# edavalosanaya/FastPoseCNN

Measured on AMD Instinct MI355X. Metric: img/s end-to-end 640x480 inference; hough-vote kernel HBM GB/s vs roofline, higher is better.
Workload: dtype f32

## Files before the change

fastposecnn_amd/_native.py:

```python
import ctypes
import os

import torch

_HERE = os.path.dirname(os.path.abspath(__file__))
LIB_PATH = os.path.join(_HERE, "libfpc_hip.so")

_lib = None

_vp = ctypes.c_void_p
_i = ctypes.c_int
_i64 = ctypes.c_int64
_u64 = ctypes.c_uint64
_f = ctypes.c_float
_d = ctypes.c_double
_sz = ctypes.c_size_t

_SIGNATURES = {
    "fpc_abi_version": (ctypes.c_int, []),
    "fpc_error_string": (ctypes.c_char_p, [_i]),
    "fpc_last_hip_error": (ctypes.c_char_p, []),
    "fpc_generate_hypothesis": (_i, [_vp, _vp, _vp, _vp, _i, _i, _i, _vp]),
    "fpc_voting_for_hypothesis": (_i, [_vp, _vp, _vp, _vp, _i, _i, _i, _f, _vp]),
    "fpc_ransac_workspace_bytes": (_sz, [_i, _i, _i, _i]),
    "fpc_ransac_voting_v3": (_i, [_vp, _vp, _i64, _i64, _i64, _i64, _i, _vp, _i, _i, _i, _vp, _vp, _u64, _f, _i, _i,
                                  _vp, _vp, _vp, _vp, _vp, _vp, _vp, _vp, _vp, _sz, _vp]),
    "fpc_ransac_voting_v3_bits": (_i, [_vp, _vp, _vp, _i64, _i64, _i64, _i64, _i, _vp, _i, _i, _i, _vp, _vp, _u64, _f, _i, _i, _vp, _vp, _vp, _vp, _vp, _vp, _vp, _vp, _vp, _sz, _vp]),
    "fpc_ransac_voting_v3_pose": (_i, [_vp, _vp, _vp, _i64, _i64, _i64, _i64, _i, _vp, _i, _i, _i, _vp, _vp, _u64, _f, _i, _i, _vp, _vp, _vp, _vp, _vp, _vp, _vp, _vp,
                                       _vp, _vp, _vp, _vp, _vp, _vp, _vp, _sz, _vp]),
    "fpc_vote_set_prune": (_i, [_i, _i, ctypes.POINTER(ctypes.c_int32)]),
    "fpc_vote_prune_info": (_i, [_vp, _sz, _i, _i, _i, _i, _vp, _vp]),
    "fpc_class_compress": (_i, [_vp, _vp, _vp, _vp, _vp, _vp, _i, _i, _i, _vp, _vp, _vp, _vp, _vp, _vp]),
    "fpc_class_compress_bits": (_i, [_vp, _vp, _vp, _vp, _vp, _vp, _i, _i, _i, _vp, _vp, _vp, _vp, _vp, _vp, _vp]),
    "fpc_cc_workspace_bytes": (_sz, [_i, _i, _i]),
    "fpc_cc_bits_supported": (_i, [_i, _i, _i]),
    "fpc_fg_bits": (_i, [_vp, _i, _i, _i, _vp, _vp]),
    "fpc_cc_label_bits": (_i, [_vp, _i, _i, _i, _vp, _vp, _vp, _i, _vp, _sz, _vp]),
    "fpc_cc_label": (_i, [_vp, _i, _i, _i, _vp, _vp, _vp, _i, _vp, _sz, _vp]),
    "fpc_aggregate_workspace_bytes": (_sz, [_i]),
    "fpc_aggregate": (_i, [_vp, _vp, _vp, _vp, _vp, _vp, _i, _i, _i, _i, _vp, _vp, _vp, _vp, _vp, _vp, _vp, _vp, _vp, _vp, _sz,
                           _vp]),
    "fpc_aggregate_bits": (_i, [_vp, _vp, _vp, _vp, _vp, _vp, _i, _i, _i, _i, _vp, _vp, _vp, _vp, _vp, _vp, _vp, _vp, _vp, _vp, _vp, _vp, _sz, _vp]),
    "fpc_mask_bits_words": (_sz, [_i, _i]),
    "fpc_pose_errors": (_i, [_vp, _vp, _vp, _vp, _i, _vp, _vp, _vp, _vp, _vp, _vp, _i, _vp, _vp, _vp, _vp]),
    "fpc_pose_metrics_state_words": (_sz, [_i, _i, _i, _i, _i]),
    "fpc_pose_metrics_update": (_i, [_vp, _vp, _vp, _i, _i] + [_vp] * 11 + [_i, _vp, _i, _vp, _i, _vp, _i, _vp, _i, _vp, _i] + [_vp] * 5 + [_i, _vp]),
    "fpc_confusion_update": (_i, [_vp, _vp, _i64, _i, _vp, _vp]),
    "fpc_post_network_backward": (_i, [_vp, _vp, _i, _i, _i, _i, _vp, _vp, _f, _i, _u64, _vp, _vp, _vp, _vp, _vp, _vp]),
    "fpc_vote_refine_backward": (_i, [_vp, _vp, _i64, _i64, _i64, _i64, _i, _i, _i, _vp, _f, _i, _u64, _vp, _vp, _vp]),
    "fpc_class_compress_backward": (_i, [_vp, _vp, _vp, _vp, _vp, _vp, _vp, _i, _i, _i, _vp, _vp, _vp, _vp, _vp]),
    "fpc_mask_losses": (_i, [_vp, _vp, _i, _i, _i, _i64, _i64, _f, _f, _vp, _vp, _vp, _vp]),
    "fpc_match_assign": (_i, [_vp, _vp, _vp, _i, _i, _vp, _vp, _vp, _vp]),
    "fpc_matched_losses": (_i, [_vp, _vp, _vp, _i, _i] + [_vp] * 10 + [_i, _d, _i, _i, _i, ctypes.POINTER(_d)] + [_vp] * 5),
    "fpc_matched_losses_backward": (_i, [_vp, _vp, _vp, _i, _i] + [_vp] * 10 + [_i, _d, _i, _i, _i, ctypes.POINTER(_d)] + [_vp] * 8),
    "fpc_grad_sumsq": (_i, [_vp, _sz, _vp, _vp]),
    "fpc_lookahead_radam_step": (_i, [_vp, _vp, _vp, _vp, _vp, _sz, _f, _f, _f, _f, _f, _i64, _i, _f, _vp, _vp]),
    "fpc_pose_rt": (_i, [_vp, _vp, _vp, _vp, _i, _vp, _vp, _vp, _vp]),
    "fpc_pack_pose_records": (_i, [_vp] * 9 + [_i, _i, _i, _vp, _vp]),
    "fpc_mask_iou_workspace_bytes": (_sz, [_i, _i, _i64]),
    "fpc_mask_iou": (_i, [_vp, _i, _vp, _i, _i64, _i, _vp, _vp, _vp, _vp, _sz, _vp]),
    "fpc_preprocess_workspace_bytes": (_sz, [_i]),
    "fpc_preprocess_u8": (_i, [_vp, _i, _i, _i, ctypes.POINTER(ctypes.c_double), ctypes.POINTER(ctypes.c_double), _i, _vp, _vp,
                               _sz, _vp]),
    "fpc_png_info": (_i, [_vp, _sz, ctypes.POINTER(ctypes.c_int32)]),
    "fpc_png_decode": (_i, [_vp, _sz, _vp, _sz, _i]),
    "fpc_png_decode_batch": (_i, [ctypes.POINTER(_vp), ctypes.POINTER(_sz), _i, _vp, _i, _i, _i]),
    "fpc_inflate_host": (_i, [_vp, _sz, _vp, _sz, ctypes.POINTER(_sz)]),
    "fpc_png_pack_bytes": (_sz, [_i, _i, _i]),
    "fpc_png_pack_batch": (_i, [ctypes.POINTER(_vp), ctypes.POINTER(_sz), _i, _i, _i, _i, _vp, _sz, _vp, ctypes.POINTER(_sz)]),
    "fpc_png_decode_device_workspace_bytes": (_sz, [_i, _i, _i, _i]),
    "fpc_png_decode_device": (_i, [_vp, _sz, _vp, _i, _i, _i, _i, _i, _vp, _sz, _vp, _vp, _sz, _vp]),
    "fpc_gt_build": (_i, [_vp, _i64, _i64, _i, _i, _i, _vp, _vp, _vp, _i, _vp, _vp, _i, _vp, _vp]),
    "fpc_depth_decode": (_i, [_vp, _i, _i, _i, _i, _i, _vp, _vp]),
    "fpc_net_create": (_i, [ctypes.c_char_p, _i, _i, _i, _i, ctypes.POINTER(_vp)]),
    "fpc_net_create_encoder": (_i, [_i, ctypes.POINTER(_i), _i, _i, _i, _i, ctypes.POINTER(_vp)]),
    "fpc_net_create_encoder_ex": (_i, [_i, ctypes.POINTER(_i), _i, _i, _i, _i, _i, _i, ctypes.POINTER(_vp)]),
    "fpc_net_create_encoder_se": (_i, [ctypes.POINTER(_i), _i, _i, _i, _i, _i, ctypes.POINTER(_vp)]),
    "fpc_net_destroy": (None, [_vp]),
    "fpc_net_set_graph": (_i, [_vp, _i]),
    "fpc_net_set_split_precision": (_i, [_vp, _i]),
    "fpc_net_param_count": (_i, [_vp]),
    "fpc_net_param_name": (ctypes.c_char_p, [_vp, _i]),
    "fpc_net_param_numel": (_i64, [_vp, _i]),
    "fpc_net_workspace_bytes": (_sz, [_vp]),
    "fpc_net_load_params": (_i, [_vp, _vp, _i, _vp, _sz, _vp]),
    "fpc_net_forward": (_i, [_vp, _vp, _vp, _vp, _vp, _vp, _vp, _vp, _vp, _vp, _vp, _vp, _vp]),
    "fpc_net_forward_bits": (_i, [_vp, _vp, _vp, _vp, _vp, _vp, _vp, _vp, _vp, _vp, _vp, _vp, _vp, _vp]),
    "fpc_net_autotune_next": (_i, [_vp, _i]),
    "fpc_net_conv_count": (_i, [_vp]),
    "fpc_net_conv_plan": (_i, [_vp, _i, ctypes.POINTER(_i)]),
    "fpc_net_copy_plans": (_i, [_vp, _vp]),
    "fpc_net_force_winograd": (_i, [_vp, _i]),
    "fpc_net_force_pointwise": (_i, [_vp, _i]),
    "fpc_net_force_fold": (_i, [_vp, _i]),
    "fpc_net_force_direct_h3": (_i, [_vp, _i]),
    "fpc_net_force_stem_pool": (_i, [_vp, _i]),
    "fpc_act_range": (_i, [_vp, ctypes.c_longlong, _vp, _vp]),
    "fpc_net_survey_next": (_i, [_vp, _vp, _i]),
    "fpc_net_guard_ranges": (_i, [_vp, ctypes.POINTER(ctypes.c_uint32), _i, _f, _f]),
    "fpc_net_guarded": (_i, [_vp, _i]),
    "fpc_stem_pool_tasks": (_i, [_i, _i, ctypes.POINTER(_i64)]),
    "fpc_wino_pack_geometry": (_i, [_i, _i, _i, _i, _i, ctypes.POINTER(_i64)]),
    "fpc_net_set_wino_pack": (_i, [_vp, _i]),
    "fpc_net_set_wino_orient": (_i, [_vp, _i]),
    "fpc_wino_orient_geometry": (_i, [_i, _i, _i, _i, _i, _i, ctypes.POINTER(_i64)]),
    "fpc_wino_recip": (_i, [ctypes.c_uint32, ctypes.POINTER(_i64)]),
    "fpc_wino_decode": (_i, [_i, _i, _i, _i, _i, _i, _i, ctypes.POINTER(_i64)]),
    "fpc_net_wino_blocks": (_i64, [_vp]),
    "fpc_net_graph_recorded": (_i, [_vp]),
    "fpc_net_flops": (_i, [_vp, ctypes.POINTER(ctypes.c_double)]),
    "fpc_net_tensor": (_i, [_vp, ctypes.c_char_p, ctypes.POINTER(_vp), ctypes.POINTER(_i), ctypes.POINTER(_i),
                            ctypes.POINTER(_i)]),
    "fpc_conv2d_workspace_bytes": (_sz, [_i, _i, _i, _i, _i, _i, _i]),
    "fpc_conv2d_workspace_bytes_for": (_sz, [_i, _i, _i, _i, _i, _i, _i, _i, _i, _i]),
    "fpc_conv2d_plan": (_i, [_i, _i, _i, _i, _i, _i, _i, _i, _i, _i, ctypes.POINTER(_i)]),
    "fpc_conv2d": (_i, [_vp, _i64, _i64, _i64, _i64, _vp, _vp, _vp, _vp, _vp, _vp, _vp, _i, _i, _i, _i, _i, _i, _i, _i,
                        _i, _i, _i, _i, _i, _vp, _sz, _vp]),
    "fpc_conv2d_grouped_workspace_bytes": (_sz, [_i, _i]),
    "fpc_conv2d_grouped": (_i, [_vp, _i64, _i64, _i64, _i64, _vp, _vp, _vp, _vp, _i, _i, _i, _i, _i, _i, _i, _i, _vp, _sz, _vp]),
    "fpc_conv2d_grouped_dgrad_workspace_bytes": (_sz, [_i, _i]),
    "fpc_conv2d_grouped_dgrad": (_i, [_vp, _vp, _vp, _i, _i, _i, _i, _i, _i, _vp, _sz, _vp]),
    "fpc_conv2d_grouped_wgrad_workspace_bytes": (_sz, [_i, _i, _i, _i, _i]),
    "fpc_conv2d_grouped_wgrad": (_i, [_vp, _i64, _i64, _i64, _vp, _vp, _i, _i, _i, _i, _i, _i, _vp, _sz, _vp]),
    "fpc_image_nhwc4": (_i, [_vp, _vp, _i, _i, _i, _vp]),
    "fpc_stem_wgrad_workspace_bytes": (_sz, [_i, _i, _i]),
    "fpc_stem_wgrad_slices": (_i, [_i, _i, _i]),
    "fpc_stem_wgrad": (_i, [_vp, _vp, _vp, _i, _i, _i, _vp, _sz, _vp]),
    "fpc_maxpool3x3s2_fwd": (_i, [_vp, _vp, _i, _i, _i, _i, _vp]),
    "fpc_maxpool3x3s2_bwd": (_i, [_vp, _vp, _vp, _i, _i, _i, _i, _vp]),
    "fpc_se_pool_slabs": (_i, [_i, _i, _i]),
    "fpc_se_scratch_floats": (_sz, [_i, _i, _i, _i]),
    "fpc_se_gate": (_i, [_vp, _vp, _vp, _vp, _vp, _vp, _vp, _i, _i, _i, _i, _i, _vp]),
    "fpc_se_scale_add_relu": (_i, [_vp, _vp, _vp, _vp, _i, _i, _i, _i, _vp]),
    "fpc_maxpool3x3s2_ceil_fwd": (_i, [_vp, _vp, _i, _i, _i, _i, _vp]),
    "fpc_conv2d_wgrad_workspace_bytes": (_sz, [_i, _i, _i, _i, _i, _i, _i]),
    "fpc_upsample_bilinear_fwd": (_i, [_vp, _i64, _i64, _i64, _i64, _vp, _i, _i, _i, _i, _i, _i, _vp]),
    "fpc_upsample_bilinear_bwd_scratch_floats": (_sz, [_i, _i, _i, _i, _i]),
    "fpc_upsample_bilinear_bwd": (_i, [_vp, _i64, _i64, _i64, _i64, _vp, _vp, _i, _i, _i, _i, _i, _i, _vp]),
    "fpc_groupnorm4_relu_scratch_floats": (_sz, [_i, _i, _i]),
    "fpc_groupnorm4_relu_fwd": (_i, [_vp, _vp, _vp, _vp, _vp, _vp, _i, _i, _i, _i, ctypes.c_float, _vp]),
    "fpc_groupnorm4_relu_bwd": (_i, [_vp, _vp, _vp, _vp, _vp, _vp, _vp, _i, _i, _i, _i, _vp]),
    "fpc_batchnorm_scratch_floats": (_sz, [_i, _i]),
    "fpc_batchnorm_fwd": (_i, [_vp, _vp, _vp, _vp, _vp, _vp, _vp, _vp, _vp, _i, _i, _f, _f, _i, _vp]),
    "fpc_batchnorm_bwd": (_i, [_vp, _vp, _vp, _vp, _vp, _vp, _vp, _vp, _vp, _vp, _i, _i, _i, _vp]),
    "fpc_conv2d_wgrad": (_i, [_vp, _i64, _i64, _i64, _vp, _vp, _i, _i, _i, _i, _i, _i, _i, _i, _i, _vp, _sz, _vp]),
    "fpc_conv2d_wgrad_split": (_i, [_vp, _i64, _i64, _i64, _vp, _vp, _i, _i, _i, _i, _i, _i, _i, _i, _i, _vp, _sz, _vp]),
}

EXPORTED = tuple(_SIGNATURES)


def lib():
    global _lib
    if _lib is None:
        if not os.path.exists(LIB_PATH):
            raise RuntimeError(
                f"fastposecnn_amd: {LIB_PATH} is missing — build it with `python -m fastposecnn_amd.build` "
                "(hipcc --offload-arch=gfx950). There is no CPU fallback for the HIP hot path.")
        L = ctypes.CDLL(LIB_PATH)
        for name, (res, args) in _SIGNATURES.items():
            fn = getattr(L, name)
            fn.restype = res
            fn.argtypes = args
        if L.fpc_abi_version() != 11:
            raise RuntimeError("fastposecnn_amd: libfpc_hip.so ABI version mismatch")
        _lib = L
    return _lib


def check(rc, what):
    if rc != 0:
        L = lib()
        msg = L.fpc_error_string(rc).decode()
        hip = L.fpc_last_hip_error().decode() if rc == -3 else ""
        raise RuntimeError(f"fastposecnn_amd: {what} failed: {msg} (code {rc}){' — HIP: ' + hip if hip else ''}")


def ptr(t):
    return None if t is None else t.data_ptr()


_raw_stream = getattr(torch._C, "_cuda_getCurrentRawStream", None)
_cur_device = getattr(torch._C, "_cuda_getDevice", None)


def stream():
    if _raw_stream is not None and _cur_device is not None:
        return _raw_stream(_cur_device())
    return torch.cuda.current_stream().cuda_stream


def require_gpu(*tensors, what="this op"):
    for t in tensors:
        if t is not None and not t.is_cuda:
            raise RuntimeError(f"fastposecnn_amd: {what} runs only on GPU tensors (HIP kernels, no CPU fallback)")


_workspaces = {}


def workspace(tag, device, nbytes):
    key = (tag, device.index, stream())
    ws = _workspaces.get(key)
    if ws is None or ws.numel() < nbytes:
        ws = torch.empty(max(int(nbytes), 256), dtype=torch.uint8, device=device)
        assert ws.data_ptr() % 256 == 0
        _workspaces[key] = ws
    return ws
```

fastposecnn_amd/csrc/net.hip:

```cpp
#include <math.h>
#include <stdio.h>
#include <stdlib.h>
#include <string.h>

#include <initializer_list>
#include <string>
#include <utility>
#include <vector>

#include "net_kernels.hpp"

namespace fpc {

struct PackedConv {
    int Cin = 0, Cinp = 0, Cout = 0, Kh = 1, Kw = 1, stride = 1, pad = 0;
    int Kwp = 1;
    int K = 0, Kpad = 0, Npad = 0;
    int p_w = -1;
    int p_bn = -1;
    int p_bias = -1;
    size_t w_off = 0, scale_off = 0, shift_off = 0;
    size_t wino_off = 0;
    bool wino_ok = false;
    size_t h3_off = 0;
// ... 94 lines not shown
    return out;
}

static size_t splitk_floats_for(const ConvPlan& p, int groups, int B, int Npad) {
    return p.nsplit > 1 ? (size_t)groups * p.nsplit * B * p.mtiles * p.bm * Npad : 0;
}

enum WinoImage { kImgF32, kImgBf3, kImgC128, kImgH2, kImgH3, kWinoImageCount };
struct WinoImageDesc { int units, tail; int (*pack)(const float* w_oihw, float* packed, int Cout, int Cin, hipStream_t s); };
static int pack_h3_plain(const float* w_oihw, float* packed, int Cout, int Cin, hipStream_t s) { return launch_wino_pack_h3(w_oihw, packed, Cout, Cin, false, s); }
constexpr WinoImageDesc kWinoImages[kWinoImageCount] = {
    {16, 0, launch_wino_pack},
    {24, 0, launch_wino_pack_bf3},
    {24, 0, launch_wino_pack_c128},
    {16, 8, launch_wino_pack_h2},
    {16, 8, pack_h3_plain},
};
constexpr size_t kWinoSlack = 128;

constexpr int kWinoFormCount = 10;
constexpr int kWinoBf3 = 5, kWinoW4 = 7;
constexpr int kWinoH2 = 8, kWinoH3 = 9;
struct WinoForm {
    int waves;
    int bn, ck;
    int variant;
    WinoImage image;
    int wg_per_cu;
    int min_split;
    bool zeros;
    bool range_limited;
    int (*launch)(const WinoArgs& a, int groups, hipStream_t s);
};
constexpr WinoForm kWinoForms[kWinoFormCount] = {
    {},
    {4, 64, 8, 0, kImgF32, 2, 0, false, false, launch_conv_wino},
    {8, 64, 8, 0, kImgF32, 1, 0, false, false, launch_conv_wino},
    {4, 64, 8, 1, kImgF32, 2, 0, false, false, launch_conv_wino},
    {8, 64, 8, 2, kImgF32, 1, 0, true, false, launch_conv_wino},
    {8, 64, 8, 3, kImgBf3, 1, 1, true, false, launch_conv_wino},
    {4, 128, 8, 0, kImgC128, 1, 1, false, false, launch_conv_wino_c128},
    {8, 64, 8, 0, kImgBf3, 1, 1, false, false, launch_conv_wino_w4},
    {8, 64, 8, 0, kImgH2, 1, 2, false, true, launch_conv_wino_h2},
    {8, 64, 16, 0, kImgH3, 1, 3, false, true, launch_conv_wino_h3},
};
static bool wino_form_ok(int form, int Cin, int Cout) {
    return form >= 1 && form < kWinoFormCount && Cout % kWinoForms[form].bn == 0 && Cin % kWinoForms[form].ck == 0;
}
struct WinoSpan { size_t units, tails; };
static WinoSpan wino_span(int end, bool c128) {
    WinoSpan sp{0, 0};
    for (int i = 0; i < end; ++i)
        if (i != kImgC128 || c128) { sp.units += kWinoImages[i].units; sp.tails += kWinoImages[i].tail; }
    return sp;
}
static_assert(kWinoImages[kImgH2].tail + kWinoImages[kImgH3].tail <= 64, "kWinoSlack keeps one 64-float line for all tails");
static size_t wino_image_offset(WinoImage img, int Cout, int Cin) {
    const WinoSpan sp = wino_span(img, Cout % 128 == 0);
    return sp.units * Cout * Cin + sp.tails;
}
static size_t wino_region_floats(WinoImage last, int Cout, int Cin, bool c128) { return (wino_span(last, c128).units + kWinoImages[last].units) * Cout * Cin + kWinoSlack; }
static bool plan_range_limited(const ConvPlan& p) {
    return p.h3 || p.fold || p.pool || (p.wino && kWinoForms[p.wino].range_limited);
}
struct WinoGrid { int tbx, tby; int patches() const { return tbx * tby; } };
static WinoGrid wino_grid(int form, int H, int W) { return {cdiv(cdiv(W, 2), 8), cdiv(cdiv(H, 2), kWinoForms[form].waves)}; }

struct Conv2dRequest { int nsplit; bool bf3, two_launch; int wino, lat; bool stem; int pw; bool h3, pool, pack, orient; int grp; };
static Conv2dRequest decode_plan(int code) {
    Conv2dRequest r{code, false, false, 0, 0, false, 0, false, false, false, false, 0};
    if (code >= FPC_PLAN_GROUPED && code < FPC_PLAN_GROUPED + 1000) { r.grp = code - FPC_PLAN_GROUPED + 1; r.nsplit = 1; return r; }
    if (code == FPC_PLAN_WINO_ORIENT) { r.orient = true; r.nsplit = -kWinoH3; }
    if (code == FPC_PLAN_WINO_PACKED) { r.pack = true; r.nsplit = -kWinoH3; }
    if (r.nsplit >= FPC_PLAN_LATERAL_H3 && r.nsplit < FPC_PLAN_LATERAL_H3 + 1000) { r.lat = r.nsplit - FPC_PLAN_LATERAL_H3; r.h3 = true; r.nsplit = 1; return r; }
    if (r.nsplit >= FPC_PLAN_H3 && r.nsplit < FPC_PLAN_H3 + 200) { r.h3 = true; r.nsplit -= FPC_PLAN_H3; }
    if (r.nsplit >= FPC_PLAN_POINTWISE) { r.pw = r.nsplit - FPC_PLAN_POINTWISE + 1; r.bf3 = true; r.nsplit = 1; return r; }
    if (r.nsplit == FPC_PLAN_STEM_POOL) { r.stem = true; r.pool = true; r.h3 = true; r.nsplit = 1; return r; }
    if (r.nsplit == FPC_PLAN_STEM) { r.stem = true; r.bf3 = true; r.nsplit = 1; return r; }
    if (r.nsplit >= FPC_PLAN_LATERAL) { r.lat = r.nsplit - FPC_PLAN_LATERAL; r.bf3 = true; r.nsplit = 1; return r; }
    if (r.nsplit >= FPC_PLAN_BF3) { r.bf3 = true; r.nsplit -= FPC_PLAN_BF3; }
    if (r.nsplit >= FPC_PLAN_TWO_LAUNCH) { r.two_launch = true; r.nsplit -= FPC_PLAN_TWO_LAUNCH; }
    if (r.nsplit <= -1 && r.nsplit > -kWinoFormCount) r.wino = -r.nsplit;
    return r;
}
static int encode_plan(const ConvPlan& p, bool folded_away) {
    if (folded_away) return FPC_PLAN_FOLDED;
    if (p.grp) return FPC_PLAN_GROUPED + p.grp - 1;
    if (p.h3) return p.lat ? FPC_PLAN_LATERAL_H3 + p.lat : FPC_PLAN_H3 + p.nsplit;
    if (p.pw) return FPC_PLAN_POINTWISE + p.pw - 1;
    if (p.stem) return p.pool ? FPC_PLAN_STEM_POOL : FPC_PLAN_STEM;
    if (p.lat) return FPC_PLAN_LATERAL + p.lat;
    return p.wino ? -p.wino : p.nsplit;
}

}

using namespace fpc;

struct fpc_net {
    int layers[4];
    int classes, B, H, W;
    int expansion = 1;
    int groups = 1, width = 64;
    int se = 0;
    std::vector<std::string> pnames;
    std::vector<int64_t> pnumel;
    std::vector<const float*> pptr;
    std::vector<PackedConv> convs;
    size_t packed_floats = 0;
    size_t total_floats = 0;
    float* ws = nullptr;
    bool loaded = false;
    bool tuning = false;
    bool tuned = false;
    int tune_mode = 0;

    int c_stem = -1;
    struct Block { int conv1, conv2, ds, conv3 = -1; int p_se = -1; };
    std::vector<Block> blocks[4];
    struct Dec {
        int lat[4];
        int seg[7];
        int p_gn[7];
        int p_head_w, p_head_b;
        int head_ch, head_chp;
    } dec[4];

    Act a_img4, a_stem, a_pool;
    std::vector<Act> a_blk_t[4], a_blk_y[4], a_blk_d[4];
    std::vector<Act> a_blk_t2[4];
    Act a_p[4][4];
    Act a_seg[4][7];
    Act a_up[4][3];
    size_t gn_part_off[4][7], gn_aff_off[4][7];
    int gn_P[7];
    Act a_low[4];
    Act a_lsum[4];
    int merge_split = -1;
    size_t splitk_off = 0, splitk_floats = 0;
    size_t se_gate_off = 0, se_part_off = 0;
    int use_graph = 0;
    long long wino_blocks = 0;
    int wino_pack = 1;
    int wino_orient = 1;
    std::vector<char> c_tr;
    int split_precision = 0;
    hipGraphExec_t graph_exec = nullptr;
    size_t zeros_off = 0;
    size_t tickets_off = 0;

    bool h3_packed = false;
    hipStream_t load_stream = nullptr;
    size_t stem_h3_off = 0;
    bool fold_ok = false;
    size_t fold_wc_off[4] = {}, fold_img1_off[4] = {}, fold_img2_off[4] = {}, fold_tab_off[4] = {};

    std::vector<ConvPlan> cplan;
    std::vector<float> tune_score;
    unsigned* survey = nullptr;
    std::vector<ConvPlan> free_plan;
    std::vector<char> has_free;
    std::vector<char> guarded;
    std::vector<int> c_howo, c_groups;

    size_t bump = 0;
    size_t alloc(size_t n) { size_t o = bump; bump += (n + 63) / 64 * 64; return o; }
    Act alloc_act(int h, int w, int c) { Act a; a.H = h; a.W = w; a.C = c; a.off = alloc((size_t)B * h * w * c); return a; }
    int add_param(const std::string& n, int64_t numel) { pnames.push_back(n); pnumel.push_back(numel); return (int)pnames.size() - 1; }

    int add_conv(const std::string& wname, int Cin, int Cout, int k, int stride, int pad, const char* bn_prefix,
                 const char* bias_name, int Cinp = 0, int Kwp = 0) {
        PackedConv c;
        c.Cin = Cin; c.Cinp = Cinp ? Cinp : Cin; c.Cout = Cout; c.Kh = c.Kw = k; c.stride = stride; c.pad = pad;
        c.Kwp = Kwp ? Kwp : k;
        c.K = c.Cinp * k * c.Kwp; c.Kpad = cdiv(c.K, kConvBK) * kConvBK; c.Npad = cdiv(Cout, kConvNAlign) * kConvNAlign;
        c.p_w = add_param(wname, (int64_t)Cout * Cin * k * k);
        if (bn_prefix) {
            std::string p(bn_prefix);
            c.p_bn = add_param(p + ".weight", Cout);
            add_param(p + ".bias", Cout);
            add_param(p + ".running_mean", Cout);
            add_param(p + ".running_var", Cout);
        }
        if (bias_name) c.p_bias = add_param(bias_name, Cout);
        c.w_off = alloc(conv_packed_floats(c.Npad, c.Kpad));
        if (bn_prefix) { c.scale_off = alloc(Cout); c.shift_off = alloc(Cout); }
        c.wino_ok = (k == 3 && stride == 1 && pad == 1 && c.Cinp == Cin && Cin % 8 == 0 && Cout % 64 == 0);
        if (c.wino_ok) c.wino_off = alloc(wino_region_floats(kImgH3, Cout, Cin, Cout % 128 == 0));
        convs.push_back(c);
        return (int)convs.size() - 1;
    }
    int add_grouped_conv(const std::string& wname, int C, int cg, int stride, const char* bn_prefix) {
        PackedConv c;
        c.Cin = c.Cinp = c.Cout = C; c.Kh = c.Kw = c.Kwp = 3; c.stride = stride; c.pad = 1; c.cg = cg;
        c.K = cg * 9; c.Kpad = cdiv(c.K, kConvBK) * kConvBK; c.Npad = cdiv(C, kConvNAlign) * kConvNAlign;
        c.p_w = add_param(wname, (int64_t)C * cg * 9);
        std::string p(bn_prefix);
        c.p_bn = add_param(p + ".weight", C);
        add_param(p + ".bias", C);
        add_param(p + ".running_mean", C);
        add_param(p + ".running_var", C);
        c.grp_off = alloc((size_t)C * cg * 9);
        c.scale_off = alloc(C); c.shift_off = alloc(C);
        convs.push_back(c);
        return (int)convs.size() - 1;
    }
};

static void drop_graph(fpc_net* n) {
    if (n->graph_exec) { (void)hipGraphExecDestroy(n->graph_exec); n->graph_exec = nullptr; }
}

static const char* kDecNames[4] = {"mask_decoder", "rotation_decoder", "translation_decoder", "scales_decoder"};
static const char* kHeadNames[4] = {"segmentation_head", "rotation_head", "translation_head", "scales_head"};

static int conv_out(int x, int k, int s, int p) { return (x + 2 * p - k) / s + 1; }

static int net_build(fpc_net* n, int classes, int B, int H, int W, fpc_net_t** out);

extern "C" int fpc_net_create(const char* encoder, int classes, int B, int H, int W, fpc_net_t** out) {
    const int r18[4] = {2, 2, 2, 2}, r34[4] = {3, 4, 6, 3}, r101[4] = {3, 4, 23, 3};
    if (!encoder) return FPC_EINVAL;
    if (!strcmp(encoder, "resnext50_32x4d")) return fpc_net_create_encoder_ex(4, r34, 32, 4, classes, B, H, W, out);
    if (!strcmp(encoder, "resnext101_32x4d")) return fpc_net_create_encoder_ex(4, r101, 32, 4, classes, B, H, W, out);
    if (!strcmp(encoder, "resnext101_32x8d")) return fpc_net_create_encoder_ex(4, r101, 32, 8, classes, B, H, W, out);
    const int r152[4] = {3, 8, 36, 3};
    if (!strcmp(encoder, "se_resnet50")) return fpc_net_create_encoder_se(r34, 16, classes, B, H, W, out);
    if (!strcmp(encoder, "se_resnet101")) return fpc_net_create_encoder_se(r101, 16, classes, B, H, W, out);
    if (!strcmp(encoder, "se_resnet152")) return fpc_net_create_encoder_se(r152, 16, classes, B, H, W, out);
    if (strcmp(encoder, "resnet18") && strcmp(encoder, "resnet34")) return FPC_EINVAL;
    return fpc_net_create_encoder(1, strcmp(encoder, "resnet18") ? r34 : r18, classes, B, H, W, out);
}

extern "C" int fpc_net_create_encoder(int block, const int* layers4, int classes, int B, int H, int W, fpc_net_t** out) {
    return fpc_net_create_encoder_ex(block, layers4, 1, 64, classes, B, H, W, out);
}

extern "C" int fpc_net_create_encoder_ex(int block, const int* layers4, int groups, int width_per_group, int classes, int B, int H,
                                         int W, fpc_net_t** out) {
    if (!layers4 || !out || (block != 1 && block != 4) || classes < 2 || classes > 8 || B < 1 || H < 32 || W < 32 || H % 32 ||
        W % 32)
        return FPC_EINVAL;
    for (int L = 0; L < 4; ++L)
        if (layers4[L] < 1 || layers4[L] > 64) return FPC_EINVAL;
    if (groups < 1 || width_per_group < 1 || (groups == 1 && width_per_group != 64) || (groups > 1 && block != 4)) return FPC_EINVAL;
    if (groups > 1)
        for (int planes = 64; planes <= 512; planes *= 2) {
            const int cg = planes * width_per_group / 64;
            if (!grouped_cg_ok(cg) || (long long)cg * groups > 8192 || (cg * groups) % 64) return FPC_EINVAL;
        }
    fpc_net* n = new fpc_net();
    memcpy(n->layers, layers4, sizeof(n->layers));
    n->expansion = block;
    n->groups = groups; n->width = width_per_group;
    return net_build(n, classes, B, H, W, out);
}

extern "C" int fpc_net_create_encoder_se(const int* layers4, int reduction, int classes, int B, int H, int W, fpc_net_t** out) {
    if (!layers4 || !out || classes < 2 || classes > 8 || B < 1 || H < 32 || W < 32 || H % 32 || W % 32) return FPC_EINVAL;
    for (int L = 0; L < 4; ++L)
        if (layers4[L] < 1 || layers4[L] > 64) return FPC_EINVAL;
    if (reduction < 1 || 256 % reduction) return FPC_EINVAL;
    fpc_net* n = new fpc_net();
    memcpy(n->layers, layers4, sizeof(n->layers));
    n->expansion = 4;
    n->se = reduction;
    return net_build(n, classes, B, H, W, out);
}

static int net_build(fpc_net* n, int classes, int B, int H, int W, fpc_net_t** out) {
    n->classes = classes; n->B = B; n->H = H; n->W = W;
    {
        const char* e = getenv("FPC_MERGE_SPLIT");
        n->merge_split = e ? (atoi(e) != 0) : 1;
    }
    char buf[256];

    n->c_stem = n->se ? n->add_conv("encoder.layer0.conv1.weight", 3, 64, 7, 2, 3, "encoder.layer0.bn1", nullptr, 4, 8)
                      : n->add_conv("encoder.conv1.weight", 3, 64, 7, 2, 3, "encoder.bn1", nullptr, 4, 8);
    const int planes[4] = {64, 128, 256, 512};
    const int e = n->expansion;
    int inpl = 64;
    for (int L = 0; L < 4; ++L)
        for (int bi = 0; bi < n->layers[L]; ++bi) {
            int stride = (bi == 0 && L > 0) ? 2 : 1;
            fpc_net::Block blk;
            snprintf(buf, sizeof(buf), "encoder.layer%d.%d", L + 1, bi);
            std::string p(buf);
            if (n->se) {
                const int C = 4 * planes[L], Cr = C / n->se;
                blk.conv1 = n->add_conv(p + ".conv1.weight", inpl, planes[L], 1, stride, 0, (p + ".bn1").c_str(), nullptr);
                blk.conv2 = n->add_conv(p + ".conv2.weight", planes[L], planes[L], 3, 1, 1, (p + ".bn2").c_str(), nullptr);
                blk.conv3 = n->add_conv(p + ".conv3.weight", planes[L], C, 1, 1, 0, (p + ".bn3").c_str(), nullptr);
                blk.p_se = n->add_param(p + ".se_module.fc1.weight", (int64_t)Cr * C);
                n->add_param(p + ".se_module.fc1.bias", Cr);
                n->add_param(p + ".se_module.fc2.weight", (int64_t)C * Cr);
                n->add_param(p + ".se_module.fc2.bias", C);
                blk.ds = -1;
                if (stride != 1 || inpl != C)
                    blk.ds = n->add_conv(p + ".downsample.0.weight", inpl, C, 1, stride, 0, (p + ".downsample.1").c_str(), nullptr);
                inpl = C;
                n->blocks[L].push_back(blk);
                continue;
            }
            if (e == 4) {
                const int C = 4 * planes[L];
// ... 36 lines not shown
                snprintf(buf, sizeof(buf), "%s.seg_blocks.%d.block.%d.block", kDecNames[d], sb, j);
                std::string p(buf);
                dc.seg[si] = n->add_conv(p + ".0.weight", j == 0 ? 256 : 128, 128, 3, 1, 1, nullptr, nullptr);
                dc.p_gn[si] = n->add_param(p + ".1.weight", 128);
                n->add_param(p + ".1.bias", 128);
                ++si;
            }
    }
    for (int d = 0; d < 4; ++d) {
        fpc_net::Dec& dc = n->dec[d];
        dc.head_ch = head_ch[d];
        dc.head_chp = (head_ch[d] + 3) / 4 * 4;
        dc.p_head_w = n->add_param(std::string(kHeadNames[d]) + ".0.weight", (int64_t)head_ch[d] * 128);
        dc.p_head_b = n->add_param(std::string(kHeadNames[d]) + ".0.bias", head_ch[d]);
    }
    n->fold_ok = e == 1;
    if (n->fold_ok)
        for (int d = 0; d < 4; ++d) {
            n->fold_wc_off[d] = n->alloc((size_t)128 * 64 * 9);
            n->fold_img1_off[d] = n->alloc((size_t)16 * 128 * 64 + 2);
            n->fold_img2_off[d] = n->alloc((size_t)16 * 128 * 256 + 2);
            n->fold_tab_off[d] = n->alloc((size_t)16 * 128);
        }
    if (e == 1) {
        std::vector<int> sites;
        for (int L = 1; L < 4; ++L) { sites.push_back(n->blocks[L][0].conv1); if (n->blocks[L][0].ds >= 0) sites.push_back(n->blocks[L][0].ds); }
        for (int d = 0; d < 4; ++d)
            for (int i = 0; i < 3; ++i) sites.push_back(n->dec[d].lat[i]);
        for (int ci : sites) {
            PackedConv& c = n->convs[ci];
            if (c.wino_ok || c.Cin % kConvBK != 0 || c.Cinp != c.Cin || c.Kh * c.Kw > 32) continue;
            c.h3_ok = true;
            c.h3_off = n->alloc(h3_packed_floats(c.Npad, c.Kpad));
        }
    }
    n->stem_h3_off = n->alloc(h3_packed_floats(n->convs[n->c_stem].Npad, n->convs[n->c_stem].Kpad));
    n->zeros_off = n->alloc(64);
    n->tickets_off = n->alloc(kConvTickets);
    n->packed_floats = n->bump;

    int h1 = conv_out(H, 7, 2, 3), w1 = conv_out(W, 7, 2, 3);
    n->a_img4 = n->alloc_act(H, W, 4);
    n->a_stem = n->alloc_act(h1, w1, 64);
    int hp = n->se ? h1 / 2 : conv_out(h1, 3, 2, 1), wp = n->se ? w1 / 2 : conv_out(w1, 3, 2, 1);
    n->a_pool = n->alloc_act(hp, wp, 64);
    int fh[4], fw[4];
    {
        int h = hp, w = wp;
        for (int L = 0; L < 4; ++L) {
            const int hin = h, win = w;
            if (L > 0) { h = conv_out(h, 3, 2, 1); w = conv_out(w, 3, 2, 1); }
            fh[L] = h; fw[L] = w;
            if (e == 4) {
                const int C = 4 * planes[L];
                const int mid = planes[L] * n->width / 64 * n->groups;
                const Act t1 = n->se ? n->alloc_act(h, w, mid) : n->alloc_act(hin, win, mid), t2 = n->alloc_act(h, w, mid);
                const Act y[2] = {n->alloc_act(h, w, C), n->alloc_act(h, w, C)};
                const Act dd = n->alloc_act(h, w, C);
                for (int bi = 0; bi < n->layers[L]; ++bi) {
                    Act t = t1;
                    if (bi > 0) { t.H = h; t.W = w; }
                    n->a_blk_t[L].push_back(t);
                    n->a_blk_t2[L].push_back(t2);
                    n->a_blk_y[L].push_back(y[bi & 1]);
                    n->a_blk_d[L].push_back(n->blocks[L][bi].ds >= 0 ? dd : Act());
                }
                continue;
            }
            for (int bi = 0; bi < n->layers[L]; ++bi) {
                n->a_blk_t[L].push_back(n->alloc_act(h, w, planes[L]));
                n->a_blk_y[L].push_back(n->alloc_act(h, w, planes[L]));
                n->a_blk_d[L].push_back(n->blocks[L][bi].ds >= 0 ? n->alloc_act(h, w, planes[L]) : Act());
            }
        }
    }
    if (n->se) {
        size_t part = 0;
        for (int L = 0; L < 4; ++L) part = std::max(part, (size_t)se_pool_slabs(fh[L], fw[L], 4 * planes[L]) * 4 * planes[L]);
        n->se_gate_off = n->alloc((size_t)B * 4 * planes[3]);
        n->se_part_off = n->alloc((size_t)B * part);
    }
    for (int L = 1; L < 4; ++L)
        if (fh[L - 1] != 2 * fh[L] || fw[L - 1] != 2 * fw[L]) { delete n; return FPC_EINVAL; }
    const int seg_level[7] = {3, 2, 1, 2, 1, 1, 0};
    for (int d = 0; d < 4; ++d) {
        for (int i = 0; i < 4; ++i) n->a_p[d][i] = n->alloc_act(fh[3 - i], fw[3 - i], 256);
        for (int i = 0; i < 7; ++i) n->a_seg[d][i] = n->alloc_act(fh[seg_level[i]], fw[seg_level[i]], 128);
        n->a_up[d][0] = n->alloc_act(fh[2], fw[2], 128);
        n->a_up[d][1] = n->alloc_act(fh[1], fw[1], 128);
        n->a_up[d][2] = n->alloc_act(fh[1], fw[1], 128);
        n->a_low[d] = n->alloc_act(fh[0], fw[0], n->dec[d].head_chp);
        n->a_lsum[d] = n->alloc_act(fh[1], fw[1], n->dec[d].head_chp);
    }

    n->cplan.resize(n->convs.size());
    n->tune_score.assign(n->convs.size(), 0.f);
    n->free_plan.assign(n->convs.size(), ConvPlan());
    n->has_free.assign(n->convs.size(), 0);
    n->guarded.assign(n->convs.size(), 0);
    n->c_howo.assign(n->convs.size(), 0);
    n->c_groups.assign(n->convs.size(), 0);
    n->c_tr.assign(n->convs.size(), 0);
    auto oriented = [&](int ci, int h, int w) { if (ci >= 0 && n->convs[ci].wino_ok) n->c_tr[ci] = wino_orient_rule(h, w) ? 1 : 0; };
    for (int L = 0; L < 4; ++L)
        for (const fpc_net::Block& blk : n->blocks[L]) { oriented(blk.conv1, fh[L], fw[L]); oriented(blk.conv2, fh[L], fw[L]); }
    auto plan = [&](int ci, int HoWo, int groups) {
        const PackedConv& c = n->convs[ci];
        n->c_howo[ci] = HoWo; n->c_groups[ci] = groups;
        if (c.cg) { ConvPlan q; q.grp = 1; n->cplan[ci] = q; return; }
        n->cplan[ci] = plan_conv(HoWo, B, c.Cout, c.Kpad / kConvBK, groups);
        size_t need = splitk_floats_for(n->cplan[ci], groups, B, c.Npad);
        for (const ConvPlan& q : conv_candidates(HoWo, B, c.Cout, c.Kpad / kConvBK, groups)) {
            size_t f = splitk_floats_for(q, groups, B, c.Npad);
            if (f * sizeof(float) <= ((size_t)256 << 20) && f > need) need = f;
        }
        if (need > n->splitk_floats) n->splitk_floats = need;
    };
    plan(n->c_stem, h1 * w1, 1);
    for (int L = 0; L < 4; ++L)
        for (size_t bi = 0; bi < n->blocks[L].size(); ++bi) {
            const fpc_net::Block& blk = n->blocks[L][bi];
            plan(blk.conv1, n->a_blk_t[L][bi].H * n->a_blk_t[L][bi].W, 1);
            plan(blk.conv2, fh[L] * fw[L], 1);
            if (blk.conv3 >= 0) plan(blk.conv3, fh[L] * fw[L], 1);
            if (blk.ds >= 0) plan(blk.ds, fh[L] * fw[L], 1);
        }
    for (int i = 0; i < 4; ++i) plan(n->dec[0].lat[i], fh[3 - i] * fw[3 - i], 4);
    for (int i = 0; i < 7; ++i) {
        int HoWo = fh[seg_level[i]] * fw[seg_level[i]];
        plan(n->dec[0].seg[i], HoWo, 4);
        n->gn_P[i] = cdiv(HoWo, 128) * 4;
        n->gn_P[i] = std::max(n->gn_P[i], wino_pack_geometry(fh[seg_level[i]], fw[seg_level[i]], B, n->convs[n->dec[0].seg[i]].Cin, true).gn_rows);
        bool tr;
        if (wino_launch_geometry(fh[seg_level[i]], fw[seg_level[i]], B, n->convs[n->dec[0].seg[i]].Cin, true, true, &tr).gn_rows > n->gn_P[i]) { delete n; return FPC_EINVAL; }
        for (int d = 0; d < 4; ++d) oriented(n->dec[d].seg[i], fh[seg_level[i]], fw[seg_level[i]]);
        for (int d = 0; d < 4; ++d) {
            n->gn_part_off[d][i] = n->alloc((size_t)B * n->gn_P[i] * 128 * 2);
            n->gn_aff_off[d][i] = n->alloc((size_t)B * 128 * 2);
        }
    }
    n->splitk_off = n->alloc(n->splitk_floats);
    n->total_floats = n->bump;
    n->pptr.assign(n->pnames.size(), nullptr);
    *out = n;
    return FPC_OK;
}

extern "C" void fpc_net_destroy(fpc_net_t* n) {
    if (!n) return;
    if (n->graph_exec) (void)hipGraphExecDestroy(n->graph_exec);
    delete n;
}

static int pack_h3_images(fpc_net* n, hipStream_t s) {
    for (const PackedConv& c : n->convs)
        if (c.h3_ok) {
            int rc = launch_pack_weight_h3(n->pptr[c.p_w], n->ws + c.h3_off, c.Cout, c.Cin, c.Cinp, c.Kh, c.Kw, c.Kwp, c.Npad, c.Kpad, s);
            if (rc) return rc;
        }
    const PackedConv& st = n->convs[n->c_stem];
    int rc = launch_pack_weight_h3(n->pptr[st.p_w], n->ws + n->stem_h3_off, st.Cout, st.Cin, st.Cinp, st.Kh, st.Kw, st.Kwp, st.Npad, st.Kpad, s);
    if (rc) return rc;
    n->h3_packed = true;
    return FPC_OK;
}

extern "C" int fpc_net_set_split_precision(fpc_net_t* n, int on) {
    if (!n) return FPC_EINVAL;
    n->split_precision = on < 0 ? 0 : (on > 3 ? 3 : on);
    if (n->split_precision >= 3 && n->loaded && !n->h3_packed) return pack_h3_images(n, n->load_stream);
    return FPC_OK;
}

extern "C" int fpc_net_graph_recorded(const fpc_net_t* n) { return n && n->use_graph && n->graph_exec ? 1 : 0; }

extern "C" int fpc_net_set_wino_pack(fpc_net_t* n, int on) {
    if (!n || on < 0 || on > 1) return FPC_EINVAL;
    if (n->wino_pack != on) drop_graph(n);
    n->wino_pack = on;
    return FPC_OK;
}

static int pack_wino_h3_image(const fpc_net* n, int ci, hipStream_t s) {
    const PackedConv& c = n->convs[ci];
    return launch_wino_pack_h3(n->pptr[c.p_w], n->ws + c.wino_off + wino_image_offset(kImgH3, c.Cout, c.Cin), c.Cout, c.Cin,
                               n->wino_orient && n->c_tr[ci], s);
}
static int pack_fold_images(const fpc_net* n, int d, hipStream_t s) {
    const PackedConv &sc = n->convs[n->dec[d].seg[6]], &lc = n->convs[n->dec[d].lat[3]];
    const bool tr = n->wino_orient && n->c_tr[n->dec[d].seg[6]];
    int rc = launch_fold_compose(n->pptr[sc.p_w], n->pptr[lc.p_w], n->pptr[lc.p_bias], n->ws + n->fold_wc_off[d],
                                 n->ws + n->fold_tab_off[d], sc.Cout, sc.Cin, lc.Cin, tr, s);
    if (!rc) rc = launch_wino_pack_h3_pair(n->ws + n->fold_wc_off[d], n->ws + n->fold_img1_off[d], lc.Cin, n->pptr[sc.p_w],
                                           n->ws + n->fold_img2_off[d], sc.Cin, sc.Cout, tr, s);
    return rc;
}

extern "C" int fpc_net_set_wino_orient(fpc_net_t* n, int on) {
    if (!n || on < 0 || on > 1) return FPC_EINVAL;
    if (n->wino_orient == on) return FPC_OK;
    drop_graph(n);
    n->wino_orient = on;
    if (!n->loaded) return FPC_OK;
    if (hipDeviceSynchronize() != hipSuccess) return FPC_ELAUNCH;
    for (size_t ci = 0; ci < n->convs.size(); ++ci)
        if (n->c_tr[ci] && wino_form_ok(kWinoH3, n->convs[ci].Cin, n->convs[ci].Cout)) { const int rc = pack_wino_h3_image(n, (int)ci, n->load_stream); if (rc) return rc; }
    if (n->fold_ok && n->c_tr[n->dec[0].seg[6]])
        for (int d = 0; d < 4; ++d) { const int rc = pack_fold_images(n, d, n->load_stream); if (rc) return rc; }
    return hipStreamSynchronize(n->load_stream) == hipSuccess ? FPC_OK : FPC_ELAUNCH;
}

extern "C" int64_t fpc_net_wino_blocks(const fpc_net_t* n) { return n ? (int64_t)n->wino_blocks : -1; }

extern "C" int fpc_net_set_graph(fpc_net_t* n, int on) {
    if (!n) return FPC_EINVAL;
    n->use_graph = on ? 1 : 0;
    if (!on) drop_graph(n);
    return FPC_OK;
}
extern "C" int fpc_net_param_count(const fpc_net_t* n) { return n ? (int)n->pnames.size() : 0; }
extern "C" const char* fpc_net_param_name(const fpc_net_t* n, int i) {
    return (n && i >= 0 && i < (int)n->pnames.size()) ? n->pnames[i].c_str() : nullptr;
}
extern "C" int64_t fpc_net_param_numel(const fpc_net_t* n, int i) {
    return (n && i >= 0 && i < (int)n->pnumel.size()) ? n->pnumel[i] : -1;
}
extern "C" size_t fpc_net_workspace_bytes(const fpc_net_t* n) { return n ? n->total_floats * sizeof(float) : 0; }

extern "C" int fpc_net_load_params(fpc_net_t* n, const float* const* params, int count, void* ws, size_t ws_bytes,
                                   fpc_stream_t stream) {
    if (!n || !params || count != (int)n->pnames.size() || !ws) return FPC_EINVAL;
    if (((uintptr_t)ws & 255) != 0 || ws_bytes < n->total_floats * sizeof(float)) return FPC_EWORKSPACE;
    drop_graph(n);
    for (int i = 0; i < count; ++i)
        if (!params[i] || ((uintptr_t)params[i] & 15)) return FPC_EINVAL;
    hipStream_t s = (hipStream_t)stream;
    n->ws = (float*)ws;
    n->pptr.assign(params, params + count);
    n->load_stream = s;
    n->h3_packed = false;
    if (n->split_precision >= 3) { int rc = pack_h3_images(n, s); if (rc) return rc; }
    if (hipMemsetAsync(n->ws + n->zeros_off, 0, 64 * sizeof(float), s) != hipSuccess) return FPC_ELAUNCH;
    if (hipMemsetAsync(n->ws + n->tickets_off, 0, kConvTickets * sizeof(int), s) != hipSuccess) return FPC_ELAUNCH;
    for (size_t ci = 0; ci < n->convs.size(); ++ci) {
        const PackedConv& c = n->convs[ci];
        if (c.cg) {
            int rg = launch_pack_grouped(n->pptr[c.p_w], n->ws + c.grp_off, c.Cout, c.cg, s);
            if (!rg) rg = launch_fold_bn(n->pptr[c.p_bn], n->pptr[c.p_bn + 1], n->pptr[c.p_bn + 2], n->pptr[c.p_bn + 3], 1e-5f, c.Cout,
                                         n->ws + c.scale_off, n->ws + c.shift_off, s);
            if (rg) return rg;
            continue;
        }
        int rc = launch_pack_weight(n->pptr[c.p_w], n->ws + c.w_off, c.Cout, c.Cin, c.Cinp, c.Kh, c.Kw, c.Kwp, c.Npad, c.Kpad, s);
        if (rc) return rc;
        rc = launch_pack_weight_bf3(n->pptr[c.p_w], n->ws + c.w_off, c.Cout, c.Cin, c.Cinp, c.Kh, c.Kw, c.Kwp, c.Npad, c.Kpad, s);
        if (rc) return rc;
        if (c.wino_ok) {
            for (int f = 1, done = 0; f < kWinoFormCount; ++f) {
                const WinoImage img = kWinoForms[f].image;
                if (!wino_form_ok(f, c.Cin, c.Cout) || (done >> img & 1)) continue;
                done |= 1 << img;
                rc = img == kImgH3 ? pack_wino_h3_image(n, (int)ci, s)
                                   : kWinoImages[img].pack(n->pptr[c.p_w], n->ws + c.wino_off + wino_image_offset(img, c.Cout, c.Cin), c.Cout, c.Cin, s);
                if (rc) return rc;
            }
        }
        if (c.p_bn >= 0) {
            rc = launch_fold_bn(n->pptr[c.p_bn], n->pptr[c.p_bn + 1], n->pptr[c.p_bn + 2], n->pptr[c.p_bn + 3], 1e-5f,
                                c.Cout, n->ws + c.scale_off, n->ws + c.shift_off, s);
            if (rc) return rc;
        }
    }
    if (n->fold_ok)
        for (int d = 0; d < 4; ++d) {
            const int rc = pack_fold_images(n, d, s);
            if (rc) return rc;
        }
    n->loaded = true;
    return FPC_OK;
}

namespace {

struct ConvIO {
    const float* in; long long sb, sh, sw, sc; int Hi, Wi;
    float* out; int Ho, Wo;
    const float* res; const float* up; float* gn_part;
};

void fill_conv_args(const fpc_net* n, ConvArgs& a, const PackedConv& c, const ConvPlan& p, int Hi, int Wi, int Ho,
                    int Wo, long long sb, long long sh, long long sw, long long sc, bool relu, int mode) {
    memset(&a, 0, sizeof(a));
    a.B = n->B; a.Hi = Hi; a.Wi = Wi; a.Cin = c.Cin; a.Ho = Ho; a.Wo = Wo; a.Cout = c.Cout; a.Npad = c.Npad;
    a.Kh = c.Kh; a.Kw = c.Kw; a.stride = c.stride; a.pad = c.pad; a.K = c.K; a.Kpad = c.Kpad;
    a.in_sb = sb; a.in_sh = sh; a.in_sw = sw; a.in_sc = sc;
    a.relu = relu ? 1 : 0; a.nsplit = p.nsplit; a.mtiles = p.mtiles; a.ntiles = p.ntiles; a.ksteps = c.Kpad / kConvBK;
    a.bm = p.bm; a.bn = p.bn; a.generic = mode;
    a.splitk_ws = n->ws + n->splitk_off;
    a.zeros = n->ws + n->zeros_off;
    a.tickets = (int*)(n->ws + n->tickets_off);
    a.fused = p.fused;
    a.wino_pack = n->wino_pack;
    a.wino_orient = n->wino_orient;
}

int launch_conv_plan(ConvArgs& a, const ConvPlan& p, int groups, hipStream_t s) {
    if (p.grp || a.cg) {
        if (!p.grp || p.grp > kGroupedForms || !a.cg || !a.grp_w || groups != 1 || a.in_sc != 1 || a.Kh != 3 || a.pad != 1 ||
            a.Cin != a.Cout || a.p[0].res || a.p[0].up || a.p[0].gn_part)
            return FPC_EINVAL;
        GroupedArgs g;
        memset(&g, 0, sizeof(g));
        g.in = a.p[0].in; g.w = a.grp_w; g.out = a.p[0].out; g.scale = a.p[0].scale; g.shift = a.p[0].shift;
        g.in_sb = a.in_sb; g.in_sh = a.in_sh; g.in_sw = a.in_sw;
        g.B = a.B; g.Hi = a.Hi; g.Wi = a.Wi; g.Ho = a.Ho; g.Wo = a.Wo; g.C = a.Cout; g.CG = a.cg; g.stride = a.stride; g.relu = a.relu;
        g.form = p.grp - 1;
        return launch_conv3x3_grouped(g, s);
// ... 95 lines not shown
    int rc = launch_conv(l, groups, s);
    if (!rc && l.nsplit > 1 && !l.fused) rc = launch_conv_splitk_epilogue(l, groups, s);
    return rc;
}

int plan_gn_rows(const ConvPlan& p, int Ho, int Wo, int B, int Cin, int pack, int orient) {
    bool tr;
    if (p.wino == kWinoH3) return wino_launch_geometry(Ho, Wo, B, Cin, orient, pack && !p.fold, &tr).gn_rows;
    return p.wino ? wino_grid(p.wino, Ho, Wo).patches() : p.mtiles * p.bm / 32;
}

template <class F> float min_ms(hipStream_t s, int reps, F run) {
    hipEvent_t e0 = nullptr, e1 = nullptr;
    float ms = 1e30f;
    if (hipEventCreate(&e0) == hipSuccess && hipEventCreate(&e1) == hipSuccess)
        for (int rep = 0; rep < reps; ++rep) {
            float t = 0.f;
            bool timed = hipEventRecord(e0, s) == hipSuccess && run() == FPC_OK && hipEventRecord(e1, s) == hipSuccess &&
                         hipEventSynchronize(e1) == hipSuccess && hipEventElapsedTime(&t, e0, e1) == hipSuccess;
            if (timed && t < ms) ms = t;
        }
    if (e0) (void)hipEventDestroy(e0);
    if (e1) (void)hipEventDestroy(e1);
    return ms;
}

std::vector<ConvPlan> tune_candidates(const ConvArgs& a, int groups, int split, int expansion) {
    if (a.cg) {
        std::vector<ConvPlan> gc;
        for (int f = 0; f < kGroupedForms; ++f) { ConvPlan q; q.grp = f + 1; gc.push_back(q); }
        return gc;
    }
    std::vector<ConvPlan> cands = conv_candidates(a.Ho * a.Wo, a.B, a.Cout, a.ksteps, groups);
    const size_t nf = cands.size();
    if (split && a.generic == 0) {
        for (size_t i = 0; i < nf; ++i) { ConvPlan q = cands[i]; q.bf3 = 1; cands.push_back(q); }
    }
    if (split >= 3 && a.generic == 0 && a.h3_w[0]) {
        for (size_t i = 0; i < nf; ++i) { ConvPlan q = cands[i]; q.h3 = 1; cands.push_back(q); }
    }
    if (split && groups == 1 && stem_ok(a)) {
        ConvPlan sq; sq.stem = 256; cands.push_back(sq);
    }
    if (split && lateral_ok(a, groups)) {
        const int tiles = groups * (a.Cout / 32);
        for (int parts = 1; parts <= tiles; parts *= 2)
            if (tiles % parts == 0) {
                ConvPlan lq; lq.lat = parts; cands.push_back(lq);
                if (split >= 3 && a.h3_w[0]) { lq.h3 = 1; cands.push_back(lq); }
            }
    }
    if (split && expansion == 4 && pw_ok(a, groups)) {
        ConvPlan pq;
        pq.pw = 1; cands.push_back(pq);
        pq.pw = 2; cands.push_back(pq);
    }
    if (a.wino_w[0] && !a.p[0].up) {
        auto offered = [&](int f) { return split >= kWinoForms[f].min_split && wino_form_ok(f, a.Cin, a.Cout) && (a.zeros || !kWinoForms[f].zeros); };
        for (int f = 1; f < kWinoFormCount; ++f) {
            if (!offered(f) || (f == kWinoH2 && offered(kWinoH3))) continue;
            ConvPlan wq; wq.wino = f; cands.push_back(wq);
        }
    }
    return cands;
}

struct PlanFootprint { double nblk, share; };
PlanFootprint plan_footprint(const ConvPlan& q, const ConvArgs& a, int groups) {
    bool tr;
    double nblk = q.grp ? (double)cdiv(a.Ho, 8) * cdiv(a.Wo, grouped_tile_cols(a.stride)) * (a.Cout / 32) * a.B
                  : q.stem ? 512.0
                  : q.lat ? (double)cdiv(a.Ho * a.Wo, 128) * a.B * q.lat
                  : q.pw ? (double)cdiv(a.B * a.Ho * a.Wo, pw_tile_pixels(q.pw - 1)) * (a.Cout / 64) * groups * q.pw
                  : q.wino == kWinoH3 ? (double)wino_launch_geometry(a.Ho, a.Wo, a.B, a.Cin, a.wino_orient, a.wino_pack && !q.fold, &tr).patches * (a.Cout / 64) * groups
                  : q.wino ? (double)wino_grid(q.wino, a.Ho, a.Wo).patches() * a.B * (a.Cout / kWinoForms[q.wino].bn) * groups
                         : (double)q.mtiles * q.ntiles * q.nsplit * a.B * groups;
    double share = nblk / (256.0 * (q.wino ? kWinoForms[q.wino].wg_per_cu : 2));
    if (share > 1.0) share = 1.0;
    if (share < 0.125) share = 0.125;
    return {nblk, share};
}

int survey_site(const fpc_net* n, const ConvArgs& a, const ConvPlan& p, int groups, int ci, hipStream_t s) {
    unsigned* rec = n->survey + 4 * (size_t)ci;
    if (p.fold) {
        unsigned* rec_up = n->survey + 4 * (size_t)n->dec[0].lat[3];
        int rc = launch_act_range(a.fold_in, (long long)a.B * a.Ho * a.Wo * a.fold_cin, rec, s);
        for (int g = 0; g < groups && !rc; ++g) rc = launch_act_range(a.fold_up[g], (long long)a.B * (a.Ho / 2) * (a.Wo / 2) * a.Cin, rec_up, s);
        return rc;
    }
    for (int g = 0; g < groups; ++g) {
        bool seen = false;
        for (int h = 0; h < g; ++h) seen = seen || a.p[h].in == a.p[g].in;
        if (seen) continue;
        const int rc = launch_act_range(a.p[g].in, (long long)a.B * a.in_sb, rec, s);
        if (rc) return rc;
    }
    return FPC_OK;
}

int run_conv(fpc_net* n, ConvArgs& a, int groups, int ci, hipStream_t s) {
    if (n && n->tuning) {
        float best_ms = 1e30f, free_ms = 1e30f;
        ConvPlan best = n->cplan[ci];
        n->has_free[ci] = 0;
        for (const ConvPlan& q : tune_candidates(a, groups, n->split_precision, n->expansion)) {
            if (splitk_floats_for(q, groups, a.B, a.Npad) > n->splitk_floats) continue;
            if (n->guarded[ci] && plan_range_limited(q)) continue;
            int rc = launch_conv_plan(a, q, groups, s);
            if (rc == FPC_EINVAL) continue;
            if (rc) return rc;
            const float ms = min_ms(s, 3, [&] { return launch_conv_plan(a, q, groups, s); });
            float score = ms;
            if (n->tune_mode >= 1) {
                const double share = plan_footprint(q, a, groups).share;
                score = ms * (float)(n->tune_mode == 2 ? share : sqrt(share));
            }
            if (score < best_ms) { best_ms = score; best = q; }
            if (score < free_ms && !plan_range_limited(q)) { free_ms = score; n->free_plan[ci] = q; n->has_free[ci] = 1; }
        }
        n->tune_score[ci] = best_ms;
        if (n->split_precision >= 3 && a.fold_in && a.fold_lat_ms > 0.f && !n->guarded[ci]) {
            ConvPlan fq;
            fq.wino = kWinoH3; fq.fold = 1;
            int rc = launch_conv_plan(a, fq, groups, s);
            if (rc && rc != FPC_EINVAL) return rc;
            const float ms = rc ? 1e30f : min_ms(s, 3, [&] { return launch_conv_plan(a, fq, groups, s); });
            if (ms < best_ms + a.fold_lat_ms) best = fq;
        }
        n->cplan[ci] = best;
    }
    ConvPlan p = n ? n->cplan[ci] : ConvPlan{a.bm, a.bn, a.nsplit, a.mtiles, a.ntiles, 0, a.bf3, a.fused};
    if (n && n->survey) { const int rs = survey_site(n, a, p, groups, ci, s); if (rs) return rs; }
    const int rc = launch_conv_plan(a, p, groups, s);
    if (n && !rc && p.wino == kWinoH3) n->wino_blocks += a.wino_blocks;
    return rc;
}

}

#define FPC_TRY(x) do { int rc__ = (x); if (rc__) return rc__; } while (0)

static int launch_stem_pool(const ConvArgs& a, const float* h3_image, float* pool, int Hp, int Wp, hipStream_t s) {
    if (!h3_image || !stem_ok(a)) return FPC_EINVAL;
    StemPoolArgs t;
    memset(&t, 0, sizeof(t));
    t.in = a.p[0].in; t.wpl = reinterpret_cast<const unsigned short*>(h3_image); t.out = pool;
    t.scale = a.p[0].scale; t.shift = a.p[0].shift;
    t.B = a.B; t.Hi = a.Hi; t.Wi = a.Wi; t.Ho = a.Ho; t.Wo = a.Wo; t.Hp = Hp; t.Wp = Wp; t.Npad = a.Npad; t.Kpad = a.Kpad; t.relu = a.relu;
    t.band = kStemPoolBand; t.grid = 256;
    return launch_stem_pool_h3(t, s);
}

static int forward_middle(fpc_net* n, hipStream_t s) {
    float* ws = n->ws;
    n->wino_blocks = 0;
    const int B = n->B, H = n->H, W = n->W;
    ConvArgs a;
    auto nhwc = [&](const Act& t, long long& sb, long long& sh, long long& sw, long long& sc) {
        sc = 1; sw = t.C; sh = (long long)t.W * t.C; sb = (long long)t.H * sh;
    };
    {
        const PackedConv& c = n->convs[n->c_stem];
        fill_conv_args(n, a, c, n->cplan[n->c_stem], H, W, n->a_stem.H, n->a_stem.W, (long long)4 * H * W, (long long)4 * W, 4,
                       1, true, 0);
        a.Cin = 8 * c.Cinp; a.Kw = 1; a.K = c.K; a.lanepx = 1;
        a.p[0] = ConvPtrs{ws + n->a_img4.off, ws + c.w_off, ws + n->a_stem.off, ws + c.scale_off, ws + c.shift_off, nullptr, nullptr, nullptr};
        const float* h3img = n->h3_packed ? ws + n->stem_h3_off : nullptr;
        auto pool_launch = [&]() {
            return launch_maxpool3x3s2(ws + n->a_stem.off, ws + n->a_pool.off, B, n->a_stem.H, n->a_stem.W, 64, n->a_pool.H, n->a_pool.W, s);
        };
        if (n->se) {
            n->cplan[n->c_stem].pool = 0;
            FPC_TRY(run_conv(n, a, 1, n->c_stem, s));
            FPC_TRY(launch_maxpool3x3s2_ceil(ws + n->a_stem.off, ws + n->a_pool.off, B, n->a_stem.H, n->a_stem.W, 64, s));
        } else if (n->cplan[n->c_stem].pool && !n->tuning) {
            if (n->survey) FPC_TRY(survey_site(n, a, n->cplan[n->c_stem], 1, n->c_stem, s));
            FPC_TRY(launch_stem_pool(a, h3img, ws + n->a_pool.off, n->a_pool.H, n->a_pool.W, s));
        } else {
            n->cplan[n->c_stem].pool = 0;
            FPC_TRY(run_conv(n, a, 1, n->c_stem, s));
            FPC_TRY(pool_launch());
            if (n->tuning && n->split_precision >= 3 && !n->guarded[n->c_stem] && launch_stem_pool(a, h3img, ws + n->a_pool.off, n->a_pool.H, n->a_pool.W, s) == FPC_OK) {
                const ConvPlan cur = n->cplan[n->c_stem];
                float ms_pair = 1e30f, ms_fused = 1e30f;
                for (int rep = 0; rep < 3; ++rep) {
                    ms_pair = std::min(ms_pair, min_ms(s, 1, [&] { int rc = launch_conv_plan(a, cur, 1, s); return rc ? rc : pool_launch(); }));
                    ms_fused = std::min(ms_fused, min_ms(s, 1, [&] { return launch_stem_pool(a, h3img, ws + n->a_pool.off, n->a_pool.H, n->a_pool.W, s); }));
                }
                if (ms_fused < ms_pair) { ConvPlan q; q.stem = 256; q.pool = 1; n->cplan[n->c_stem] = q; }
            }
        }
    }
    auto enc_conv = [&](int ci, const Act& in, const Act& out, bool relu, const float* res) -> int {
        long long sb, sh, sw, sc;
        nhwc(in, sb, sh, sw, sc);
        const PackedConv& c = n->convs[ci];
        fill_conv_args(n, a, c, n->cplan[ci], in.H, in.W, out.H, out.W, sb, sh, sw, sc, relu, 0);
        a.p[0] = ConvPtrs{ws + in.off, ws + c.w_off, ws + out.off, ws + c.scale_off, ws + c.shift_off, res, nullptr, nullptr};
        if (c.wino_ok) a.wino_w[0] = ws + c.wino_off;
        if (c.h3_ok && n->h3_packed) a.h3_w[0] = ws + c.h3_off;
        if (c.cg) { a.cg = c.cg; a.grp_w = ws + c.grp_off; }
        return run_conv(n, a, 1, ci, s);
    };
    Act cur = n->a_pool;
    Act feat[4];
    for (int L = 0; L < 4; ++L) {
        for (size_t bi = 0; bi < n->blocks[L].size(); ++bi) {
            const fpc_net::Block& blk = n->blocks[L][bi];
            const Act& T = n->a_blk_t[L][bi];
            const Act& Y = n->a_blk_y[L][bi];
            const float* res = ws + cur.off;
            if (n->se) {
                const Act& T2 = n->a_blk_t2[L][bi];
                FPC_TRY(enc_conv(blk.conv1, cur, T, true, nullptr));
                FPC_TRY(enc_conv(blk.conv2, T, T2, true, nullptr));
                if (blk.ds >= 0) {
                    FPC_TRY(enc_conv(blk.ds, cur, n->a_blk_d[L][bi], false, nullptr));
                    res = ws + n->a_blk_d[L][bi].off;
                }
                FPC_TRY(enc_conv(blk.conv3, T2, Y, false, nullptr));
                FPC_TRY(launch_se_pool(ws + Y.off, ws + n->se_part_off, B, Y.H, Y.W, Y.C, s));
                FPC_TRY(launch_se_excite(ws + n->se_part_off, n->pptr[blk.p_se], n->pptr[blk.p_se + 1], n->pptr[blk.p_se + 2],
                                         n->pptr[blk.p_se + 3], ws + n->se_gate_off, B, Y.H, Y.W, Y.C, n->se, s));
                FPC_TRY(launch_se_scale_add_relu(ws + Y.off, ws + n->se_gate_off, res, ws + Y.off, B, Y.H, Y.W, Y.C, s));
                cur = Y;
                continue;
            }
            if (n->expansion == 4) {
                const Act& T2 = n->a_blk_t2[L][bi];
                FPC_TRY(enc_conv(blk.conv1, cur, T, true, nullptr));
                FPC_TRY(enc_conv(blk.conv2, T, T2, true, nullptr));
                if (blk.ds >= 0) {
                    FPC_TRY(enc_conv(blk.ds, cur, n->a_blk_d[L][bi], false, nullptr));
                    res = ws + n->a_blk_d[L][bi].off;
                }
                FPC_TRY(enc_conv(blk.conv3, T2, Y, true, res));
                cur = Y;
                continue;
            }
            FPC_TRY(enc_conv(blk.conv1, cur, T, true, nullptr));
            if (blk.ds >= 0) {
                FPC_TRY(enc_conv(blk.ds, cur, n->a_blk_d[L][bi], false, nullptr));
                res = ws + n->a_blk_d[L][bi].off;
            }
            FPC_TRY(enc_conv(blk.conv2, T, Y, true, res));
            cur = Y;
        }
        feat[L] = cur;
    }

    const bool fold = n->cplan[n->dec[0].seg[6]].fold && !n->tuning;
    for (int i = 0; i < 4; ++i) {
        if (i == 3 && fold) continue;
        const Act& src = feat[3 - i];
        long long sb, sh, sw, sc;
        nhwc(src, sb, sh, sw, sc);
        int ci0 = n->dec[0].lat[i];
        fill_conv_args(n, a, n->convs[ci0], n->cplan[ci0], src.H, src.W, src.H, src.W, sb, sh, sw, sc, false, 0);
        for (int d = 0; d < 4; ++d) {
            const PackedConv& c = n->convs[n->dec[d].lat[i]];
            a.p[d] = ConvPtrs{ws + src.off, ws + c.w_off, ws + n->a_p[d][i].off, nullptr, n->pptr[c.p_bias], nullptr,
                              i > 0 ? ws + n->a_p[d][i - 1].off : nullptr, nullptr};
            if (c.h3_ok && n->h3_packed) a.h3_w[d] = ws + c.h3_off;
        }
        FPC_TRY(run_conv(n, a, 4, ci0, s));
    }
    auto seg_conv = [&](int si, int which) -> int {
        int ci0 = n->dec[0].seg[si];
        const Act& in0 = which < 0 ? n->a_p[0][-which - 1] : n->a_up[0][which];
        long long sb, sh, sw, sc;
        nhwc(in0, sb, sh, sw, sc);
        const Act& o0 = n->a_seg[0][si];
        fill_conv_args(n, a, n->convs[ci0], n->cplan[ci0], in0.H, in0.W, o0.H, o0.W, sb, sh, sw, sc, false, 0);
        for (int d = 0; d < 4; ++d) {
            const PackedConv& c = n->convs[n->dec[d].seg[si]];
            const Act& in = which < 0 ? n->a_p[d][-which - 1] : n->a_up[d][which];
            a.p[d] = ConvPtrs{ws + in.off, ws + c.w_off, ws + n->a_seg[d][si].off, nullptr, nullptr, nullptr, nullptr,
                              ws + n->gn_part_off[d][si]};
            if (c.wino_ok) a.wino_w[d] = ws + c.wino_off;
        }
        if (si == 6 && n->fold_ok) {
            a.fold_in = ws + feat[0].off;
            a.fold_cin = feat[0].C;
            for (int d = 0; d < 4; ++d) {
                a.fold_w[d] = ws + n->fold_img1_off[d];
                a.fold_w2[d] = ws + n->fold_img2_off[d];
                a.fold_up[d] = ws + n->a_p[d][2].off;
                a.fold_tab[d] = ws + n->fold_tab_off[d];
            }
            a.fold_lat_ms = n->tune_score[n->dec[0].lat[3]];
        }
        return run_conv(n, a, 4, ci0, s);
    };
    auto gn_finish = [&](std::initializer_list<int> sites) -> int {
        GnFinArgs g;
        memset(&g, 0, sizeof(g));
        int k = 0;
        for (int si : sites) {
            const Act& o0 = n->a_seg[0][si];
            for (int d = 0; d < 4; ++d) {
                g.gn_part[k * kMaxGroup + d] = ws + n->gn_part_off[d][si];
                g.gamma[k * kMaxGroup + d] = n->pptr[n->dec[d].p_gn[si]];
                g.beta[k * kMaxGroup + d] = n->pptr[n->dec[d].p_gn[si] + 1];
                g.affine[k * kMaxGroup + d] = ws + n->gn_aff_off[d][si];
            }
            g.P[k] = plan_gn_rows(n->cplan[n->dec[0].seg[si]], o0.H, o0.W, B, n->convs[n->dec[0].seg[si]].Cin, n->wino_pack, n->wino_orient);
            g.count[k] = (long long)o0.H * o0.W * 4;
            ++k;
        }
        g.B = B; g.C = 128; g.groups = 32; g.sites = k; g.eps = 1e-5f;
        return launch_gn_finalize(g, 4, s);
    };
    auto gn_up = [&](std::initializer_list<std::pair<int, int>> jobs) -> int {
        GnUpArgs u;
        memset(&u, 0, sizeof(u));
        int k = 0;
        for (const auto& job : jobs) {
            const int si = job.first, ui = job.second;
            for (int d = 0; d < 4; ++d) {
                u.in[k * kMaxGroup + d] = ws + n->a_seg[d][si].off;
                u.affine[k * kMaxGroup + d] = ws + n->gn_aff_off[d][si];
                u.out[k * kMaxGroup + d] = ws + n->a_up[d][ui].off;
            }
            u.h[k] = n->a_seg[0][si].H; u.w[k] = n->a_seg[0][si].W;
            ++k;
        }
        u.B = B; u.C = 128; u.jobs = k;
        return launch_gn_relu_up2(u, 4, s);
    };
    FPC_TRY(seg_conv(0, -1));
    FPC_TRY(seg_conv(3, -2));
    FPC_TRY(seg_conv(5, -3));
    FPC_TRY(seg_conv(6, -4));
    FPC_TRY(gn_finish({0, 3, 5, 6}));
    FPC_TRY(gn_up({{0, 0}, {3, 2}}));
    FPC_TRY(seg_conv(1, 0));
    FPC_TRY(seg_conv(4, 2));
    FPC_TRY(gn_finish({1, 4}));
    FPC_TRY(gn_up({{1, 1}}));
    FPC_TRY(seg_conv(2, 1));
    FPC_TRY(gn_finish({2}));

    const int lo[3] = {2, 4, 5};
    const int split = n->merge_split;
    if (split) {
        HeadPartArgs hl, hh;
        memset(&hl, 0, sizeof(hl));
        memset(&hh, 0, sizeof(hh));
        for (int d = 0; d < 4; ++d) {
            for (int k = 0; k < 3; ++k) {
                hl.t[d][k] = ws + n->a_seg[d][lo[k]].off;
                hl.aff[d][k] = ws + n->gn_aff_off[d][lo[k]];
            }
            hh.t[d][0] = ws + n->a_seg[d][6].off;
            hh.aff[d][0] = ws + n->gn_aff_off[d][6];
            hl.hw[d] = hh.hw[d] = n->pptr[n->dec[d].p_head_w];
            hl.hb[d] = hh.hb[d] = n->pptr[n->dec[d].p_head_b];
            hl.out[d] = ws + n->a_lsum[d].off;
            hh.lsum[d] = ws + n->a_lsum[d].off;
            hh.out[d] = ws + n->a_low[d].off;
            hl.ch[d] = hh.ch[d] = n->dec[d].head_ch;
            hl.chp[d] = hh.chp[d] = n->dec[d].head_chp;
        }
        hl.B = hh.B = B; hl.C = hh.C = 128;
        hl.H = n->a_seg[0][2].H; hl.W = n->a_seg[0][2].W; hl.hl = hl.H; hl.wl = hl.W;
        hh.H = n->a_seg[0][6].H; hh.W = n->a_seg[0][6].W; hh.hl = hl.H; hh.wl = hl.W;
        FPC_TRY(launch_head_part(hl, false, 4, s));
        FPC_TRY(launch_head_part(hh, true, 4, s));
    } else {
        MergeHeadArgs m;
        memset(&m, 0, sizeof(m));
        for (int d = 0; d < 4; ++d) {
            for (int k = 0; k < 3; ++k) {
                m.t_lo[d][k] = ws + n->a_seg[d][lo[k]].off;
                m.a_lo[d][k] = ws + n->gn_aff_off[d][lo[k]];
            }
            m.t_hi[d] = ws + n->a_seg[d][6].off;
            m.a_hi[d] = ws + n->gn_aff_off[d][6];
            m.hw[d] = n->pptr[n->dec[d].p_head_w];
            m.hb[d] = n->pptr[n->dec[d].p_head_b];
            m.out[d] = ws + n->a_low[d].off;
            m.ch[d] = n->dec[d].head_ch;
            m.chp[d] = n->dec[d].head_chp;
        }
        m.B = B; m.h = n->a_seg[0][2].H; m.w = n->a_seg[0][2].W; m.C = 128;
        FPC_TRY(launch_merge_head(m, 4, s));
    }
    return FPC_OK;
}

extern "C" int fpc_net_forward(fpc_net_t* n, const float* x, float* logits_mask, float* logits_quat,
                               float* logits_scales, float* logits_xy, float* logits_z, int64_t* cat_mask, float* cq,
                               float* cs, float* cxy, float* cz, fpc_stream_t stream) {
    return fpc_net_forward_bits(n, x, logits_mask, logits_quat, logits_scales, logits_xy, logits_z, cat_mask, cq, cs, cxy, cz, nullptr, stream);
}

static int forward_bits(fpc_net_t* n, const float* x, float* logits_mask, float* logits_quat, float* logits_scales,
                        float* logits_xy, float* logits_z, int64_t* cat_mask, float* cq, float* cs, float* cxy, float* cz,
                        uint64_t* fg_bits, fpc_stream_t stream);

extern "C" int fpc_net_forward_bits(fpc_net_t* n, const float* x, float* logits_mask, float* logits_quat,
                                    float* logits_scales, float* logits_xy, float* logits_z, int64_t* cat_mask, float* cq,
                                    float* cs, float* cxy, float* cz, uint64_t* fg_bits, fpc_stream_t stream) {
    const int rc = forward_bits(n, x, logits_mask, logits_quat, logits_scales, logits_xy, logits_z, cat_mask, cq, cs, cxy, cz, fg_bits, stream);
    if (n) n->survey = nullptr;
    return rc;
}

static int forward_bits(fpc_net_t* n, const float* x, float* logits_mask, float* logits_quat, float* logits_scales,
                        float* logits_xy, float* logits_z, int64_t* cat_mask, float* cq, float* cs, float* cxy, float* cz,
                        uint64_t* fg_bits, fpc_stream_t stream) {
    if (!n || !n->loaded || !x || !cat_mask || !cq || !cs || !cxy || !cz) return FPC_EINVAL;
    if (fg_bits && (n->W % 64 != 0 || ((uintptr_t)fg_bits & 7))) return FPC_EINVAL;
    bool any = logits_mask || logits_quat || logits_scales || logits_xy || logits_z;
    bool all = logits_mask && logits_quat && logits_scales && logits_xy && logits_z;
    if (any && !all) return FPC_EINVAL;
    hipStream_t s = (hipStream_t)stream;
    float* ws = n->ws;
    const int B = n->B, H = n->H, W = n->W;

    FPC_TRY(launch_nchw3_to_nhwc4(x, ws + n->a_img4.off, B, H * W, s));
    const bool plain = n->tuning || n->survey;
    if (n->use_graph && !plain && s != nullptr && !n->graph_exec) {
        hipGraph_t g = nullptr;
        if (hipStreamBeginCapture(s, hipStreamCaptureModeThreadLocal) == hipSuccess) {
            int rc = forward_middle(n, s);
            hipError_t e = hipStreamEndCapture(s, &g);
            if (rc) { if (g) (void)hipGraphDestroy(g); return rc; }
            if (e == hipSuccess && g) e = hipGraphInstantiate(&n->graph_exec, g, nullptr, nullptr, 0);
            if (g) (void)hipGraphDestroy(g);
            if (e != hipSuccess) n->graph_exec = nullptr;
        }
        if (!n->graph_exec) { (void)hipGetLastError(); n->use_graph = 0; }
    }
    if (n->use_graph && !plain && s != nullptr && n->graph_exec) {
        if (hipGraphLaunch(n->graph_exec, s) != hipSuccess) return FPC_ELAUNCH;
    } else {
        FPC_TRY(forward_middle(n, s));
    }
    {
        Up4Args u;
        memset(&u, 0, sizeof(u));
        u.lm = ws + n->a_low[0].off; u.lq = ws + n->a_low[1].off; u.lt = ws + n->a_low[2].off; u.ls = ws + n->a_low[3].off;
        u.pm = n->dec[0].head_chp; u.pq = n->dec[1].head_chp; u.pt = n->dec[2].head_chp; u.ps = n->dec[3].head_chp;
        u.o_mask = logits_mask; u.o_quat = logits_quat; u.o_scales = logits_scales; u.o_xy = logits_xy; u.o_z = logits_z;
        u.cat_mask = (long long*)cat_mask; u.cq = cq; u.cs = cs; u.cxy = cxy; u.cz = cz;
        u.B = B; u.hl = n->a_low[0].H; u.wl = n->a_low[0].W; u.H = H; u.W = W; u.C = n->classes;
        u.fg_bits = reinterpret_cast<unsigned long long*>(fg_bits); u.fg_stride = (size_t)((H * W + 4095) / 4096) * 64;
        if (u.hl * 4 != H || u.wl * 4 != W) return FPC_EINVAL;
        FPC_TRY(launch_up4_compress(u, s));
    }
    if (n->tuning) { n->tuning = false; n->tuned = true; }
    return FPC_OK;
}

extern "C" int fpc_net_autotune_next(fpc_net_t* n, int mode) {
    if (!n || !n->loaded || mode < 0 || mode > 2) return FPC_EINVAL;
    n->tuning = true;
    n->tune_mode = mode;
    drop_graph(n);
    return FPC_OK;
}

extern "C" int fpc_net_survey_next(fpc_net_t* n, unsigned* records_dev, int sites) {
    if (n && !records_dev) { n->survey = nullptr; return FPC_OK; }
    if (!n || !n->loaded || ((uintptr_t)records_dev & 3) || sites != (int)n->convs.size()) return FPC_EINVAL;
    n->survey = records_dev;
    return FPC_OK;
}

static ConvPlan range_free_plan(const fpc_net* n, int i) {
    if (n->has_free[i]) return n->free_plan[i];
    const PackedConv& c = n->convs[i];
    ConvPlan q = n->cplan[i];
    if (q.pool) { ConvPlan st; st.stem = 256; return st; }
    if (q.wino) {
        q.wino = wino_form_ok(kWinoW4, c.Cin, c.Cout) ? kWinoW4 : kWinoBf3;
        q.fold = 0;
        return q;
    }
    q.h3 = 0; q.bf3 = 1;
    return q;
}

extern "C" int fpc_net_guard_ranges(fpc_net_t* n, const unsigned* records_host, int sites, float lo, float hi) {
    if (!n || !records_host || sites != (int)n->convs.size() || !(lo >= 0.f) || !(hi > lo)) return FPC_EINVAL;
    auto outside = [&](int site) {
        const unsigned* rec = records_host + 4 * (size_t)site;
        float mx;
        memcpy(&mx, &rec[0], sizeof(mx));
        return rec[2] != 0 && (rec[1] > 0 || mx >= hi || (mx > 0.f && mx < lo));
    };
    int demoted = 0;
    for (int i = 0; i < sites; ++i) {
        if (!n->c_groups[i] || !plan_range_limited(n->cplan[i]) || records_host[4 * (size_t)i + 2] == 0) continue;
        if (!(outside(i) || (n->cplan[i].fold && outside(n->dec[0].lat[3])))) continue;
        n->cplan[i] = range_free_plan(n, i);
        n->guarded[i] = 1;
        ++demoted;
    }
    if (demoted) drop_graph(n);
    return demoted;
}

extern "C" int fpc_net_guarded(const fpc_net_t* n, int i) {
    return n && i >= 0 && i < (int)n->guarded.size() && n->guarded[i] ? 1 : 0;
}

extern "C" int fpc_net_conv_count(const fpc_net_t* n) { return n ? (int)n->convs.size() : 0; }
extern "C" int fpc_net_conv_plan(const fpc_net_t* n, int i, int* out5) {
    if (!n || !out5 || i < 0 || i >= (int)n->convs.size()) return FPC_EINVAL;
    const ConvPlan& p = n->cplan[i];
    out5[0] = p.bm; out5[1] = p.bn;
    if (p.lat) { out5[0] = 128; out5[1] = 32; }
    if (p.stem) { out5[0] = 64; out5[1] = 64; }
    if (p.pw) { out5[0] = pw_tile_pixels(p.pw - 1); out5[1] = 64; }
    if (p.grp) { out5[0] = 8 * grouped_tile_cols(n->convs[i].stride); out5[1] = 32; }
    out5[2] = encode_plan(p, n->fold_ok && i == n->dec[0].lat[3] && n->cplan[n->dec[0].seg[6]].fold);
    out5[3] = n->convs[i].Cout; out5[4] = n->convs[i].K;
    return FPC_OK;
}

extern "C" int fpc_net_force_winograd(fpc_net_t* n, int form) {
    if (!n || form < 1 || form >= kWinoFormCount) return FPC_EINVAL;
    int changed = 0;
    for (size_t i = 0; i < n->convs.size(); ++i) {
        const PackedConv& c = n->convs[i];
        if (!c.wino_ok || !n->c_groups[i] || !wino_form_ok(form, c.Cin, c.Cout)) continue;
        ConvPlan q = n->cplan[i];
        q.wino = form; q.lat = 0; q.stem = 0;
        if (form != kWinoH3) q.fold = 0;
        n->cplan[i] = q;
        n->guarded[i] = 0;
        ++changed;
    }
    drop_graph(n);
    return changed;
}

extern "C" int fpc_net_force_fold(fpc_net_t* n, int on) {
    if (!n || on < 0 || on > 1 || (on && !n->fold_ok)) return FPC_EINVAL;
    ConvPlan& p = n->cplan[n->dec[0].seg[6]];
    if (p.fold == on) return 0;
    ConvPlan q;
    q.wino = kWinoH3; q.fold = on;
    p = q;
    n->guarded[n->dec[0].seg[6]] = 0;
    drop_graph(n);
    return 1;
}

extern "C" int fpc_net_force_pointwise(fpc_net_t* n, int on) {
    if (!n || on < 0 || on > 1) return FPC_EINVAL;
    int changed = 0;
    for (size_t i = 0; i < n->convs.size(); ++i) {
        const PackedConv& c = n->convs[i];
        if (!n->c_groups[i] || c.Kh != 1 || c.pad != 0 || c.Cinp != c.Cin || c.Cin % 64 || c.Kpad != c.Cin || c.Cout % 64) continue;
        if (on) {
            if (n->cplan[i].pw) continue;
            ConvPlan q;
            q.pw = 1;
            n->cplan[i] = q;
        } else {
            if (!n->cplan[i].pw) continue;
            n->cplan[i] = plan_conv(n->c_howo[i], n->B, c.Cout, c.Kpad / kConvBK, n->c_groups[i]);
        }
        ++changed;
    }
    drop_graph(n);
    return changed;
}

extern "C" int fpc_net_force_direct_h3(fpc_net_t* n, int on) {
    if (!n || on < 0 || on > 1 || (on && !n->h3_packed)) return FPC_EINVAL;
    int changed = 0;
    for (size_t i = 0; i < n->convs.size(); ++i) {
        const PackedConv& c = n->convs[i];
        if (!c.h3_ok || !n->c_groups[i] || on == n->cplan[i].h3) continue;
        const ConvPlan& p = n->cplan[i];
        ConvPlan q = plan_conv(n->c_howo[i], n->B, c.Cout, c.Kpad / kConvBK, n->c_groups[i]);
        if (on && !p.wino && !p.stem && !p.pw) q = p;
        q.bf3 = 0;
        q.h3 = on;
        n->cplan[i] = q;
        n->guarded[i] = 0;
        ++changed;
    }
    drop_graph(n);
    return changed;
}

extern "C" int fpc_net_force_stem_pool(fpc_net_t* n, int on) {
    if (!n || on < 0 || on > 1 || (on && !n->h3_packed)) return FPC_EINVAL;
    if (on && n->se) return FPC_EINVAL;
    if (on && ((n->a_stem.H & 1) || (n->a_stem.W & 63) || (long long)n->H * n->W * 16 >= (1LL << 31))) return FPC_EINVAL;
    ConvPlan& p = n->cplan[n->c_stem];
    if (p.pool == on) return 0;
    ConvPlan q;
    q.stem = 256; q.pool = on;
    p = q;
    n->guarded[n->c_stem] = 0;
    drop_graph(n);
    return 1;
}

extern "C" int fpc_net_copy_plans(fpc_net_t* dst, const fpc_net_t* src) {
    if (!dst || !src || dst->convs.size() != src->convs.size() || dst->H != src->H || dst->W != src->W) return FPC_EINVAL;
    for (size_t i = 0; i < dst->convs.size(); ++i) {
        const PackedConv &a = dst->convs[i], &b = src->convs[i];
        if (a.Cin != b.Cin || a.Cout != b.Cout || a.Kh != b.Kh || a.Kw != b.Kw || a.stride != b.stride || a.Npad != b.Npad ||
            a.Kpad != b.Kpad || a.cg != b.cg || dst->c_groups[i] != src->c_groups[i])
            return FPC_EINVAL;
    }
    for (size_t i = 0; i < dst->convs.size(); ++i) {
        const ConvPlan& q = src->cplan[i];
        if (splitk_floats_for(q, dst->c_groups[i] ? dst->c_groups[i] : 1, dst->B, dst->convs[i].Npad) > dst->splitk_floats) continue;
        if (q.nsplit > 1 && q.fused && !can_fuse(q, dst->c_groups[i] ? dst->c_groups[i] : 1, dst->B)) continue;
        if ((q.h3 || q.pool) && !dst->h3_packed) continue;
        dst->cplan[i] = q;
    }
    for (size_t i = 0; i < dst->convs.size(); ++i) {
        const ConvPlan& q = src->free_plan[i];
        const int groups = dst->c_groups[i] ? dst->c_groups[i] : 1;
        dst->has_free[i] = src->has_free[i] && splitk_floats_for(q, groups, dst->B, dst->convs[i].Npad) <= dst->splitk_floats &&
                           !(q.nsplit > 1 && q.fused && !can_fuse(q, groups, dst->B));
        if (dst->has_free[i]) dst->free_plan[i] = q;
        dst->guarded[i] = dst->guarded[i] || src->guarded[i];
        if (dst->guarded[i] && plan_range_limited(dst->cplan[i])) dst->cplan[i] = range_free_plan(dst, (int)i);
    }
    dst->tuned = true;
    drop_graph(dst);
    return FPC_OK;
}

extern "C" int fpc_net_flops(const fpc_net_t* n, double* out3) {
    if (!n || !out3) return FPC_EINVAL;
    double direct = 0.0, executed = 0.0, wino = 0.0;
    for (size_t i = 0; i < n->convs.size(); ++i) {
        if (!n->c_groups[i]) continue;
        const PackedConv& c = n->convs[i];
        const double f = 2.0 * n->B * (double)n->c_howo[i] * c.Cout * (c.cg ? c.cg : c.Cin) * c.Kh * c.Kw * n->c_groups[i];
        direct += f;
        if (n->cplan[i].wino) { executed += f / 2.25; wino += f; } else executed += f;
    }
    for (int d = 0; d < 4; ++d)
        direct += 2.0 * n->B * (double)n->a_low[d].H * n->a_low[d].W * 128.0 * n->dec[d].head_ch,
        executed += 2.0 * n->B * (double)n->a_low[d].H * n->a_low[d].W * 128.0 * n->dec[d].head_ch;
    out3[0] = direct; out3[1] = executed; out3[2] = direct > 0.0 ? wino / direct : 0.0;
    return FPC_OK;
}

extern "C" int fpc_net_tensor(const fpc_net_t* n, const char* name, const float** ptr, int* H, int* W, int* C) {
    if (!n || !n->ws || !name || !ptr || !H || !W || !C) return FPC_EINVAL;
    Act t;
    bool ok = false;
    if (!strcmp(name, "stem")) {
        if (n->cplan[n->c_stem].pool) return FPC_EINVAL;
        t = n->a_stem; ok = true;
    }
    else if (!strcmp(name, "pool")) { t = n->a_pool; ok = true; }
    else if (name[0] == 'c' && name[1] >= '2' && name[1] <= '5' && !name[2]) { t = n->a_blk_y[name[1] - '2'].back(); ok = true; }
    else if (name[0] == 'd' && name[1] >= '0' && name[1] <= '3' && name[2] == '.') {
        int d = name[1] - '0';
        const char* r = name + 3;
        if (r[0] == 'p' && r[1] >= '2' && r[1] <= '5' && !r[2]) {
            if (r[1] == '2' && n->cplan[n->dec[0].seg[6]].fold) return FPC_EINVAL;
            t = n->a_p[d]['5' - r[1]]; ok = true;
        }
        else if (!strncmp(r, "seg", 3) && r[3] >= '0' && r[3] <= '6' && !r[4]) { t = n->a_seg[d][r[3] - '0']; ok = true; }
        else if (!strcmp(r, "low")) { t = n->a_low[d]; ok = true; }
    }
    if (!ok) return FPC_EINVAL;
    *ptr = n->ws + t.off; *H = t.H; *W = t.W; *C = t.C;
    return FPC_OK;
}

extern "C" int fpc_stem_pool_tasks(int Ho, int Wo, int64_t* out4) {
    if (!out4 || Ho < 2 || (Ho & 1) || Wo < 64 || (Wo & 63)) return FPC_EINVAL;
    long long o[4];
    stem_pool_tasks(Ho, Wo, kStemPoolBand, o);
    for (int i = 0; i < 4; ++i) out4[i] = o[i];
    return FPC_OK;
}

extern "C" int fpc_wino_pack_geometry(int H, int W, int B, int Cin, int fold, int64_t* out8) {
    if (!out8 || H < 1 || W < 1 || B < 1 || Cin < 1) return FPC_EINVAL;
    const WinoPackGeom q = wino_pack_geometry(H, W, B, Cin, !fold);
    out8[0] = q.G; out8[1] = q.tbx; out8[2] = q.tby; out8[3] = q.patches; out8[4] = q.slots; out8[5] = q.tiles; out8[6] = q.gn_rows;
    out8[7] = q.rx;
    return FPC_OK;
}

extern "C" int fpc_wino_orient_geometry(int H, int W, int B, int Cin, int fold, int pack, int64_t* out9) {
    if (!out9 || H < 1 || W < 1 || B < 1 || Cin < 1) return FPC_EINVAL;
    bool tr;
    const WinoPackGeom q = wino_launch_geometry(H, W, B, Cin, true, pack && !fold, &tr);
    out9[0] = tr ? 1 : 0;
    out9[1] = q.G; out9[2] = q.tbx; out9[3] = q.tby; out9[4] = q.patches; out9[5] = q.slots; out9[6] = q.tiles; out9[7] = q.gn_rows;
    out9[8] = q.rx;
    return FPC_OK;
}

extern "C" int fpc_wino_recip(uint32_t d, int64_t* out2) {
    if (!out2 || d < 1 || d > (1u << 31)) return FPC_EINVAL;
    const WinoRecip r = wino_recip(d);
    out2[0] = r.m; out2[1] = r.sh;
    return FPC_OK;
}
extern "C" int fpc_wino_decode(int Cout, int groups, int tbx, int tby, int W, int B, int pack, int64_t* out14) {
    if (!out14 || Cout < 64 || groups < 1 || tbx < 1 || tby < 1 || W < 1 || B < 1 || pack < 0) return FPC_EINVAL;
    const WinoDecode d = wino_decode(Cout, groups, tbx, tby, W, B, pack);
    const WinoRecip r[7] = {d.nnb, d.groups, d.tbx, d.tby, d.per, d.tbxl, d.tcw};
    for (int i = 0; i < 7; ++i) { out14[2 * i] = r[i].m; out14[2 * i + 1] = r[i].sh; }
    return FPC_OK;
}

extern "C" size_t fpc_conv2d_workspace_bytes(int B, int Ho, int Wo, int Cin, int Cout, int Kh, int Kw) {
    int K = Cin * Kh * Kw, Kpad = cdiv(K, kConvBK) * kConvBK, Npad = cdiv(Cout, kConvNAlign) * kConvNAlign;
    size_t packed = conv_packed_floats(Npad, Kpad);
    size_t splitk = (size_t)32 * B * (cdiv(Ho * Wo, 128) * 128) * Npad;
    size_t wino = wino_region_floats(kImgH3, Cout, Cin, true);
    return (packed + splitk + wino + kConvTickets) * sizeof(float);
}

namespace {
struct Conv2dLayout { size_t packed, splitk, wino, tickets, total; };
Conv2dLayout conv2d_layout(int B, int Cin, int Cout, int Kh, int Kw, const ConvPlan& p, const Conv2dRequest& r) {
    const int K = Cin * Kh * Kw, Kpad = cdiv(K, kConvBK) * kConvBK, Npad = cdiv(Cout, kConvNAlign) * kConvNAlign;
    Conv2dLayout L;
    L.packed = r.wino ? 0 : conv_packed_floats(Npad, Kpad);
    L.splitk = r.wino ? 0 : (splitk_floats_for(p, 1, B, Npad) + 63) / 64 * 64;
    L.wino = r.wino ? wino_region_floats(kWinoForms[r.wino].image, Cout, Cin, Cout % 128 == 0) : 0;
    L.tickets = (!r.wino && p.fused && p.nsplit > 1) ? kConvTickets : 0;
    L.total = L.packed + L.splitk + L.wino + L.tickets;
    return L;
}
ConvPlan conv2d_plan_for(int B, int Ho, int Wo, int Cin, int Cout, int Kh, int Kw, int bm, int bn, const Conv2dRequest& r) {
    const int Kpad = cdiv(Cin * Kh * Kw, kConvBK) * kConvBK;
    ConvPlan p = plan_conv(Ho * Wo, B, Cout, Kpad / kConvBK, 1, r.wino ? 0 : bm, bn, r.wino ? 1 : r.nsplit);
    p.bf3 = r.bf3 ? 1 : 0;
    p.h3 = r.h3 ? 1 : 0;
    if (r.two_launch) p.fused = 0;
    p.lat = r.lat;
    p.stem = r.stem ? 256 : 0;
    p.pool = r.pool ? 1 : 0;
    p.pw = r.pw;
    p.wino = r.wino;
    return p;
}
}

extern "C" int fpc_conv2d_plan(int B, int Ho, int Wo, int Cin, int Cout, int Kh, int Kw, int bm, int bn, int nsplit,
                               int* out4) {
    if (!out4) return FPC_EINVAL;
    const int Kpad = cdiv(Cin * Kh * Kw, kConvBK) * kConvBK;
    const Conv2dRequest r = decode_plan(nsplit);
    ConvPlan p = plan_conv(Ho * Wo, B, Cout, Kpad / kConvBK, 1, bm, bn, r.nsplit);
    p.wino = r.wino;
    out4[0] = p.bm; out4[1] = p.bn; out4[2] = r.wino ? nsplit : p.nsplit; out4[3] = plan_gn_rows(p, Ho, Wo, B, Cin, r.pack, r.orient);
    return FPC_OK;
}

extern "C" size_t fpc_conv2d_workspace_bytes_for(int B, int Ho, int Wo, int Cin, int Cout, int Kh, int Kw, int bm, int bn,
                                                 int nsplit) {
    if (B < 1 || Ho < 1 || Wo < 1 || Cin < 1 || Cout < 1 || Kh < 1 || Kw < 1) return 0;
    const Conv2dRequest r = decode_plan(nsplit);
    const ConvPlan p = conv2d_plan_for(B, Ho, Wo, Cin, Cout, Kh, Kw, bm, bn, r);
    return std::max<size_t>(conv2d_layout(B, Cin, Cout, Kh, Kw, p, r).total * sizeof(float), 256);
}

extern "C" int fpc_conv2d(const float* in, int64_t sb, int64_t sh, int64_t sw, int64_t sc, const float* w_oihw,
                          const float* scale, const float* shift, const float* res, const float* up, float* out,
                          float* gn_part, int B, int Hi, int Wi, int Cin, int Cout, int Kh, int Kw, int stride, int pad,
                          int relu, int bm, int bn, int nsplit, void* ws, size_t ws_bytes, fpc_stream_t stream) {
    if (!in || !w_oihw || !out || !ws || B < 1 || Kh != Kw) return FPC_EINVAL;
    int Ho = conv_out(Hi, Kh, stride, pad), Wo = conv_out(Wi, Kw, stride, pad);
    if (Ho < 1 || Wo < 1) return FPC_EINVAL;
    const Conv2dRequest rq = decode_plan(nsplit);
    if (rq.grp) return FPC_EINVAL;
    const int wino = rq.wino;
    ConvPlan p = conv2d_plan_for(B, Ho, Wo, Cin, Cout, Kh, Kw, bm, bn, rq);
    const Conv2dLayout lay = conv2d_layout(B, Cin, Cout, Kh, Kw, p, rq);
    if (ws_bytes < lay.total * sizeof(float) || ((uintptr_t)ws & 255)) return FPC_EWORKSPACE;
    PackedConv c;
    c.Cin = c.Cinp = Cin; c.Cout = Cout; c.Kh = Kh; c.Kw = Kw; c.stride = stride; c.pad = pad;
    c.K = Cin * Kh * Kw; c.Kpad = cdiv(c.K, kConvBK) * kConvBK; c.Npad = cdiv(Cout, kConvNAlign) * kConvNAlign;
    hipStream_t s = (hipStream_t)stream;
    float* packed = (float*)ws;
    if (rq.stem) {
        if (Cin != 4 || Kh != 7 || stride != 2 || pad != 3 || Cout != 64 || sc != 1 || sw != 4 || sh != (int64_t)4 * Wi ||
            sb != (int64_t)4 * Hi * Wi || res || up || gn_part)
            return FPC_EINVAL;
        c.Kwp = 8; c.K = 4 * 7 * 8; c.Kpad = 224;
        FPC_TRY((rq.pool ? launch_pack_weight_h3 : launch_pack_weight_bf3)(w_oihw, packed, Cout, Cin, Cin, Kh, Kw, c.Kwp, c.Npad, c.Kpad, s));
        fpc_net tmp0;
        tmp0.B = B; tmp0.ws = packed; tmp0.splitk_off = lay.packed;
        ConvArgs a0;
        fill_conv_args(&tmp0, a0, c, p, Hi, Wi, Ho, Wo, sb, sh, sw, sc, relu != 0, 0);
        a0.Cin = 8 * c.Cinp; a0.Kw = 1; a0.K = c.K; a0.lanepx = 1;
        a0.p[0] = ConvPtrs{in, packed, out, scale, shift, nullptr, nullptr, nullptr};
        return rq.pool ? launch_stem_pool(a0, packed, out, Ho / 2, Wo / 2, s) : launch_conv_plan(a0, p, 1, s);
    }
    static_assert(FPC_IGEMM_DMA_B, "the split-precision direct form stages its B rows from the bf16 planes by LDS-DMA; a build that loads "
                                   "them from the f32 image must pack that image here as well");
    if (!wino) FPC_TRY((p.h3 ? launch_pack_weight_h3 : p.bf3 ? launch_pack_weight_bf3 : launch_pack_weight)(w_oihw, packed, Cout, Cin, Cin, Kh, Kw, Kw, c.Npad, c.Kpad, s));
    int mode = (sc == 1 && Cin % kConvBK == 0 && Kh * Kw <= 32 && ((int64_t)Hi + 2 * pad) * sh * 4 < ((int64_t)1 << 31)) ? 0
               : (sc == 1 && Cin % 4 == 0 && sw % 4 == 0 && sh % 4 == 0 && sb % 4 == 0 && ((uintptr_t)in & 15) == 0) ? 2 : 1;
    fpc_net tmp;
    tmp.B = B;
    tmp.wino_pack = rq.pack ? 1 : 0;
    tmp.wino_orient = rq.orient ? 1 : 0;
    tmp.ws = packed;
    tmp.splitk_off = lay.packed;
    ConvArgs a;
    fill_conv_args(&tmp, a, c, p, Hi, Wi, Ho, Wo, sb, sh, sw, sc, relu != 0, mode);
    a.p[0] = ConvPtrs{in, packed, out, scale, shift, res, up, gn_part};
    a.zeros = nullptr;
    a.tickets = nullptr;
    if (lay.tickets) {
        float* tk = packed + lay.packed + lay.splitk + lay.wino;
        a.tickets = (int*)tk;
        if (hipMemsetAsync(tk, 0, kConvTickets * sizeof(int), s) != hipSuccess) return FPC_ELAUNCH;
    }
#ifdef FPC_STAMP_WINO
    if (wino && relu == 77) { a.dbg = gn_part; a.p[0].gn_part = nullptr; a.relu = 0; }
#endif
#ifdef FPC_STAMP_IGEMM
    if (!wino && relu == 77) { a.dbg = gn_part; a.p[0].gn_part = nullptr; a.relu = 0; }
#endif
    if (wino) {
        if (Kh != 3 || stride != 1 || pad != 1 || Cin % 8 || Cout % 64 || sc != 1 || up || sw != Cin ||
            sh != (int64_t)Wi * Cin || sb != (int64_t)Hi * Wi * Cin)
            return FPC_EINVAL;
        float* wp = packed + lay.packed + lay.splitk;
        if (!wino_form_ok(wino, Cin, Cout)) return FPC_EINVAL;
        const WinoImage img = kWinoForms[wino].image;
        if (rq.orient && wino_orient_rule(Ho, Wo)) FPC_TRY(launch_wino_pack_h3(w_oihw, wp + wino_image_offset(img, Cout, Cin), Cout, Cin, true, s));
        else FPC_TRY(kWinoImages[img].pack(w_oihw, wp + wino_image_offset(img, Cout, Cin), Cout, Cin, s));
        a.wino_w[0] = wp;
        a.zeros = zero_page();
        if (!a.zeros) {
            float* zp = wp + lay.wino - 64;
            if (hipMemsetAsync(zp, 0, 64 * sizeof(float), s) != hipSuccess) return FPC_ELAUNCH;
            a.zeros = zp;
        }
        return launch_conv_plan(a, p, 1, s);
    }
    if (p.h3) {
        if (mode != 0) return FPC_EINVAL;
        a.h3_w[0] = packed;
        return launch_conv_plan(a, p, 1, s);
    }
    a.bf3 = (p.bf3 && mode == 0) ? 1 : 0;
    if (p.bf3 && mode != 0) return FPC_EINVAL;
    if (p.lat || p.pw) return launch_conv_plan(a, p, 1, s);
    return run_conv(nullptr, a, 1, 0, s);
}

extern "C" size_t fpc_conv2d_grouped_workspace_bytes(int C, int groups) {
    if (C < 32 || C % 32 || groups < 1 || C % groups || !grouped_cg_ok(C / groups)) return 0;
    return std::max<size_t>(align_up((size_t)C * (C / groups) * 9 * sizeof(float), 256), 256);
}

extern "C" int fpc_conv2d_grouped(const float* in, int64_t sb, int64_t sh, int64_t sw, int64_t sc, const float* w_oihw,
                                  const float* scale, const float* shift, float* out, int B, int Hi, int Wi, int C, int groups,
                                  int stride, int relu, int form, void* ws, size_t ws_bytes, fpc_stream_t stream) {
    if (!in || !w_oihw || !out || !ws || B < 1 || Hi < 1 || Wi < 1 || C < 32 || C % 32 || groups < 1 || C % groups ||
        !grouped_cg_ok(C / groups) || (stride != 1 && stride != 2) || sc != 1 || form < 0 || form >= 1000)
        return FPC_EINVAL;
    const Conv2dRequest rq = decode_plan(FPC_PLAN_GROUPED + form);
    if (!rq.grp || rq.grp > kGroupedForms) return FPC_EINVAL;
    if (ws_bytes < fpc_conv2d_grouped_workspace_bytes(C, groups) || ((uintptr_t)ws & 255)) return FPC_EWORKSPACE;
    hipStream_t s = (hipStream_t)stream;
    GroupedArgs g;
    memset(&g, 0, sizeof(g));
    g.in = in; g.w = (const float*)ws; g.out = out; g.scale = scale; g.shift = shift;
    g.in_sb = sb; g.in_sh = sh; g.in_sw = sw;
    g.B = B; g.Hi = Hi; g.Wi = Wi; g.Ho = conv_out(Hi, 3, stride, 1); g.Wo = conv_out(Wi, 3, stride, 1);
    g.C = C; g.CG = C / groups; g.stride = stride; g.relu = relu ? 1 : 0; g.form = rq.grp - 1;
    if (((uintptr_t)in | (uintptr_t)out | (uintptr_t)scale | (uintptr_t)shift | (uintptr_t)w_oihw) & 15) return FPC_EINVAL;
    if ((sb | sh | sw) % 4 || sw < C) return FPC_EINVAL;
    FPC_TRY(launch_pack_grouped(w_oihw, (float*)ws, C, g.CG, s));
    return launch_conv3x3_grouped(g, s);
}
```

fastposecnn_amd/csrc/net_kernels.hpp:

```cpp
#pragma once
#include "common.hpp"

namespace fpc {

#ifndef FPC_IGEMM_DMA_B
#define FPC_IGEMM_DMA_B 1
#endif

constexpr int kMaxGroup = 4;
constexpr int kConvBK = 32;
constexpr int kConvNAlign = 128;
constexpr int kConvTickets = 16384;

struct ConvPtrs {
    const float* in;
    const float* w;
    float* out;
    const float* scale;
    const float* shift;
    const float* res;
    const float* up;
    float* gn_part;
};

struct ConvArgs {
    ConvPtrs p[kMaxGroup];
    float* splitk_ws;
    int* tickets;
    int fused;
    int B, Hi, Wi, Cin, Ho, Wo, Cout, Npad, Kh, Kw, stride, pad, K, Kpad;
    long long in_sb, in_sh, in_sw, in_sc;
    int relu, nsplit, mtiles, ntiles, ksteps, bm, bn, generic, groups;
    int bf3;
    int h3;
    int lanepx;
    const float* wino_w[kMaxGroup];
    const float* h3_w[kMaxGroup];
    const float* zeros;
    const float* fold_in;
    const float* fold_w[kMaxGroup];
    const float* fold_w2[kMaxGroup];
    const float* fold_up[kMaxGroup];
    const float* fold_tab[kMaxGroup];
    int fold_cin;
    float fold_lat_ms;
    void* dbg;
    long long wino_blocks;
    int wino_pack;
    int wino_orient;
    int cg;
    const float* grp_w;
};

struct LatArgs {
    const float* in;
    const unsigned short* wpl[kMaxGroup];
    float* out[kMaxGroup];
    const float* shift[kMaxGroup];
    const float* up[kMaxGroup];
    int B, Ho, Wo, Cout, Npad, Kpad, groups, relu;
    unsigned bias_mask;
    int parts;
    int h3;
};
int launch_lateral1x1(const LatArgs& a, hipStream_t s);

struct PwArgs {
    const float* in;
    const unsigned short* wpl[kMaxGroup];
    float* out[kMaxGroup];
    const float* scale[kMaxGroup];
    const float* shift[kMaxGroup];
    const float* res[kMaxGroup];
    const float* up[kMaxGroup];
    long long in_sb, in_sh, in_sw;
    int B, Ho, Wo, Cin, Cout, Npad, Kpad, stride, groups, relu;
    int has_scale, has_shift, has_res, has_up;
    int variant;
};
int launch_conv1x1(const PwArgs& a, hipStream_t s);
inline int pw_tile_pixels(int variant) { return variant == 0 ? 64 : 128; }

struct GroupedArgs {
    const float* in;
    const float* w;
    float* out;
    const float* scale;
    const float* shift;
    long long in_sb, in_sh, in_sw;
    int B, Hi, Wi, Ho, Wo, C, CG, stride, relu;
    int form;
    int tx, ty;
};
constexpr int kGroupedForms = 1;
bool grouped_cg_ok(int cg);
int launch_pack_grouped(const float* w_oihw, float* packed, int C, int CG, hipStream_t s, int mode = 0);
int launch_conv3x3_grouped(const GroupedArgs& a, hipStream_t s);
inline int grouped_tile_cols(int stride) { return stride == 1 ? 16 : 8; }

struct StemArgs {
    const float* in;
    const unsigned short* wpl;
    float* out;
    const float* scale;
    const float* shift;
    int B, Hi, Wi, Ho, Wo, Cout, Npad, Kpad, relu;
    int grid;
};
int launch_stem7x7(const StemArgs& a, hipStream_t s);

struct StemPoolArgs {
    const float* in;
    const unsigned short* wpl;
    float* out;
    const float* scale;
    const float* shift;
    int B, Hi, Wi, Ho, Wo, Hp, Wp, Npad, Kpad, relu;
    int band;
    int grid;
};
constexpr int kStemPoolBand = 10;
int launch_stem_pool_h3(const StemPoolArgs& a, hipStream_t s);
void stem_pool_tasks(int Ho, int Wo, int band, long long out4[4]);

constexpr int kMaxGnSites = 4;
struct GnFinArgs {
    const float* gn_part[kMaxGnSites * kMaxGroup];
    const float* gamma[kMaxGnSites * kMaxGroup];
    const float* beta[kMaxGnSites * kMaxGroup];
    float* affine[kMaxGnSites * kMaxGroup];
    int P[kMaxGnSites];
    long long count[kMaxGnSites];
    int B, C, groups, sites;
    float eps;
};

constexpr int kMaxUpJobs = 2;
struct GnUpArgs {
    const float* in[kMaxUpJobs * kMaxGroup];
    const float* affine[kMaxUpJobs * kMaxGroup];
    float* out[kMaxUpJobs * kMaxGroup];
    int h[kMaxUpJobs], w[kMaxUpJobs];
    int B, C, jobs;
};

struct MergeHeadArgs {
    const float* t_lo[kMaxGroup][3];
    const float* a_lo[kMaxGroup][3];
    const float* t_hi[kMaxGroup];
    const float* a_hi[kMaxGroup];
    const float* hw[kMaxGroup];
    const float* hb[kMaxGroup];
    float* out[kMaxGroup];
    int ch[kMaxGroup];
    int chp[kMaxGroup];
    int B, h, w, C;
};

struct HeadPartArgs {
    const float* t[kMaxGroup][3];
    const float* aff[kMaxGroup][3];
    const float* hw[kMaxGroup];
    const float* hb[kMaxGroup];
    const float* lsum[kMaxGroup];
    float* out[kMaxGroup];
    int ch[kMaxGroup], chp[kMaxGroup];
    int B, H, W, C, hl, wl;
};
int launch_head_part(const HeadPartArgs& a, bool hi, int groups, hipStream_t s);

struct Up4Args {
    const float* lm; const float* lq; const float* lt; const float* ls;
    int pm, pq, pt, ps;
    float* o_mask; float* o_quat; float* o_scales; float* o_xy; float* o_z;
    long long* cat_mask; float* cq; float* cs; float* cxy; float* cz;
    int B, hl, wl, H, W, C;
    unsigned long long* fg_bits; size_t fg_stride;
};

#ifdef FPC_STAMP_WINO
constexpr bool kWinoStamp = true;
#else
constexpr bool kWinoStamp = false;
#endif
constexpr int kWinoSerialStamps = 16;

struct WinoRecip { unsigned m; int sh; };
inline WinoRecip wino_recip(unsigned d) {
    int l = 0;
    while ((1ull << l) < d) ++l;
    const int sh = 31 + l;
    return WinoRecip{(unsigned)(((1ull << sh) + d - 1) / d), sh};
}
struct WinoDecode { WinoRecip nnb, groups, tbx, tby, per, tbxl, tcw; };
inline WinoDecode wino_decode(int Cout, int groups, int tbx, int tby, int W, int B, int pack) {
    const int tcw = (W + 1) / 2, last = pack > 0 ? ((B % pack) * tcw + 7) / 8 : 0;
    return WinoDecode{wino_recip(Cout / 64), wino_recip(groups), wino_recip(tbx), wino_recip(tby), wino_recip(tbx * tby),
                      wino_recip(last ? last : tbx), wino_recip(tcw)};
}

struct WinoArgs {
    ConvPtrs p[kMaxGroup];
    long long* dbg;
    const float* zeros;
    int variant;
    int groups;
    int waves;
    int B, H, W, Cin, Cout, relu, tbx, tby;
    const float* in2[kMaxGroup];
    const float* w2[kMaxGroup];
    const float* btab[kMaxGroup];
    int fold, Cin2;
    int pack, pack_rx;
    int orient;
    WinoDecode dec;
};
int launch_conv_wino(const WinoArgs& a, int groups, hipStream_t s);
const float* zero_page();
int launch_wino_pack(const float* w_oihw, float* packed, int Cout, int Cin, hipStream_t s);
int launch_wino_pack_bf3(const float* w_oihw, float* packed, int Cout, int Cin, hipStream_t s);
int launch_conv_wino_c128(const WinoArgs& a, int groups, hipStream_t s);
int launch_wino_pack_c128(const float* w_oihw, float* packed, int Cout, int Cin, hipStream_t s);
int launch_conv_wino_w4(const WinoArgs& a, int groups, hipStream_t s);
int launch_conv_wino_h2(const WinoArgs& a, int groups, hipStream_t s);
int launch_wino_pack_h2(const float* w_oihw, float* packed, int Cout, int Cin, hipStream_t s);
int launch_absmax_bits(const float* w, long long n, unsigned* out_bits, hipStream_t s);
int launch_act_range(const float* x, long long n, unsigned* rec4, hipStream_t s);
int launch_conv_wino_h3(const WinoArgs& a, int groups, hipStream_t s);
struct WinoPackGeom { int G, tbx, tby, rx; long long patches, slots, tiles; int gn_rows; };
WinoPackGeom wino_pack_geometry(int H, int W, int B, int Cin, bool allow);
bool wino_orient_rule(int H, int W);
WinoPackGeom wino_launch_geometry(int H, int W, int B, int Cin, bool orient, bool pack_allow, bool* transposed);
int launch_wino_pack_h3(const float* w_oihw, float* packed, int Cout, int Cin, bool transpose, hipStream_t s);
int launch_wino_pack_h3_pair(const float* w1, float* packed1, int Cin1, const float* w2, float* packed2, int Cin2, int Cout, bool transpose,
                             hipStream_t s);
int launch_fold_compose(const float* W, const float* L, const float* bias, float* wc, float* btab, int Cout, int Cmid, int Cin,
                        bool transpose, hipStream_t s);
int launch_conv(const ConvArgs& a, int groups, hipStream_t s);
int launch_conv_splitk_epilogue(const ConvArgs& a, int groups, hipStream_t s);
int launch_maxpool3x3s2(const float* in, float* out, int B, int Hi, int Wi, int C, int Ho, int Wo, hipStream_t s);
int launch_maxpool3x3s2_ceil(const float* in, float* out, int B, int Hi, int Wi, int C, hipStream_t s);
int se_pool_slabs(int H, int W, int C);
int launch_se_pool(const float* x, float* partial, int B, int H, int W, int C, hipStream_t s);
int launch_se_excite(const float* partial, const float* w1, const float* b1, const float* w2, const float* b2, float* gate, int B, int H,
                     int W, int C, int R, hipStream_t s);
int launch_se_scale_add_relu(const float* x, const float* gate, const float* res, float* y, int B, int H, int W, int C, hipStream_t s);
int launch_gn_finalize(const GnFinArgs& a, int groups, hipStream_t s);
int launch_gn_relu_up2(const GnUpArgs& a, int groups, hipStream_t s);
int launch_merge_head(const MergeHeadArgs& a, int groups, hipStream_t s);
int launch_up4_compress(const Up4Args& a, hipStream_t s);
void launch_up4_compress7x4(const Up4Args& a, hipStream_t s);

struct Lerp { int i0, i1; float l0, l1; };
__device__ __forceinline__ Lerp lerp_coord(int dst, int in, int out) {
    float scale = out > 1 ? (float)(in - 1) / (float)(out - 1) : 0.f;
    float src = scale * (float)dst;
    Lerp L;
    L.i0 = (int)src;
    L.i1 = L.i0 + (L.i0 < in - 1 ? 1 : 0);
    L.l1 = src - (float)L.i0;
    L.l0 = 1.f - L.l1;
    return L;
}

__device__ __forceinline__ Lerp lerp_scaled(int dst, int in, float scale) {
    float src = scale * (float)dst;
    Lerp L;
    L.i0 = (int)src;
    L.i1 = L.i0 + (L.i0 < in - 1 ? 1 : 0);
    L.l1 = src - (float)L.i0;
    L.l0 = 1.f - L.l1;
    return L;
}

int launch_pack_weight(const float* w_oihw, float* packed, int Cout, int Cin, int Cinp, int Kh, int Kw, int Kwp, int Npad,
// ... 13 lines not shown
```

fastposecnn_amd/csrc/stem.hip:

```cpp
#include <algorithm>
#include <type_traits>

#include "net_kernels.hpp"

namespace fpc {

typedef float f32x16 __attribute__((ext_vector_type(16)));
typedef unsigned u32x4 __attribute__((ext_vector_type(4)));
typedef float f32x3 __attribute__((ext_vector_type(3)));
typedef __bf16 bf16x8 __attribute__((ext_vector_type(8)));
typedef _Float16 f16x8 __attribute__((ext_vector_type(8)));

constexpr int kStemKG = 14;
constexpr int kStemLds = kStemKG * 3 * 2 * 1024;

__global__ __launch_bounds__(512, 1) void k_stem7x7(const StemArgs a) {
    __shared__ __attribute__((aligned(16))) unsigned char s_w[kStemLds];
    const int tid = threadIdx.x, lane = tid & 63, wv = tid >> 6, col = lane & 31, h = lane >> 5;
    for (int c = tid; c < kStemKG * 3 * 2 * 64; c += 512) {
        const int l = c & 63, nt = (c >> 6) & 1, pk = c >> 7, plane = pk % 3, kg = pk / 3;
        const unsigned short* src = a.wpl + ((size_t)plane * a.Npad + nt * 32 + (l & 31)) * a.Kpad + 16 * kg + 8 * (l >> 5);
        *reinterpret_cast<u32x4*>(&s_w[(size_t)c * 16]) = *reinterpret_cast<const u32x4*>(src);
    }
    float sc[2], sh[2];
    sc[0] = a.scale ? a.scale[col] : 1.f; sc[1] = a.scale ? a.scale[32 + col] : 1.f;
    sh[0] = a.shift ? a.shift[col] : 0.f; sh[1] = a.shift ? a.shift[32 + col] : 0.f;
    __syncthreads();

    const int segs = a.Wo >> 6;
    const int ntile = a.B * a.Ho * segs;
    int t_first = blockIdx.x * 8 + wv, t_end = ntile, t_step = gridDim.x * 8;
    if ((gridDim.x & 7) == 0) {
        const int per = (ntile + 7) >> 3, lo = (blockIdx.x & 7) * per;
        t_first = lo + (blockIdx.x >> 3) * 8 + wv; t_end = min(lo + per, ntile); t_step = (gridDim.x >> 3) * 8;
    }
    for (int tile = t_first; tile < t_end; tile += t_step) {
        const int t2 = tile / segs, seg = tile - t2 * segs;
        const int b = t2 / a.Ho, oy = t2 - b * a.Ho;
        const int ox0 = seg * 64;
        const float* img = a.in + (size_t)b * a.Hi * a.Wi * 4;
        f32x16 acc[2][2];
#pragma unroll
        for (int s = 0; s < 2; ++s)
#pragma unroll
            for (int nt = 0; nt < 2; ++nt)
#pragma unroll
                for (int i = 0; i < 16; ++i) acc[s][nt][i] = 0.f;
        const int ixb = 2 * (ox0 + col) - 3 + 2 * h;
        constexpr int kPre = 4;
        f32x4 ring[kPre][4];
        unsigned keep[kPre][4];
        auto issue = [&](int j, f32x4 (&r)[4], unsigned (&m)[4]) {
            const int kh = j >> 1, g2 = j & 1;
            const int iy = 2 * oy - 3 + kh;
            const bool rowok = iy >= 0 && iy < a.Hi;
            const float* rowp = img + (size_t)min(max(iy, 0), a.Hi - 1) * a.Wi * 4;
#pragma unroll
            for (int q = 0; q < 4; ++q) {
                const int ix = ixb + 64 * (q >> 1) + 4 * g2 + (q & 1);
                m[q] = (rowok && ix >= 0 && ix < a.Wi) ? 0xFFFFFFFFu : 0u;
                r[q] = *reinterpret_cast<const f32x4*>(rowp + (size_t)min(max(ix, 0), a.Wi - 1) * 4);
            }
        };
        auto masked = [](f32x4 v, unsigned m) {
            f32x4 o;
#pragma unroll
            for (int e = 0; e < 4; ++e) { const float x = v[e]; o[e] = __builtin_bit_cast(float, __builtin_bit_cast(unsigned, x) & m); }
            return o;
        };
#pragma unroll
        for (int j = 0; j < kPre; ++j) issue(j, ring[j], keep[j]);
#pragma unroll
        for (int j = 0; j < kStemKG; ++j) {
            u32x4 A1[2], A2[2], A3[2];
#pragma unroll
            for (int s = 0; s < 2; ++s) {
                u32x2 p1, p2, p3, q1, q2, q3;
                split_bf3(masked(ring[j % kPre][2 * s], keep[j % kPre][2 * s]), p1, p2, p3);
                split_bf3(masked(ring[j % kPre][2 * s + 1], keep[j % kPre][2 * s + 1]), q1, q2, q3);
                A1[s] = u32x4{p1[0], p1[1], q1[0], q1[1]};
                A2[s] = u32x4{p2[0], p2[1], q2[0], q2[1]};
                A3[s] = u32x4{p3[0], p3[1], q3[0], q3[1]};
            }
            if (j + kPre < kStemKG) issue(j + kPre, ring[j % kPre], keep[j % kPre]);
            const unsigned char* wb = &s_w[(size_t)(j * 3 * 2) * 1024 + lane * 16];
#pragma unroll
            for (int nt = 0; nt < 2; ++nt) {
                const bf16x8 b1 = __builtin_bit_cast(bf16x8, *reinterpret_cast<const u32x4*>(wb + (0 * 2 + nt) * 1024));
                const bf16x8 b2 = __builtin_bit_cast(bf16x8, *reinterpret_cast<const u32x4*>(wb + (1 * 2 + nt) * 1024));
                const bf16x8 b3 = __builtin_bit_cast(bf16x8, *reinterpret_cast<const u32x4*>(wb + (2 * 2 + nt) * 1024));
#pragma unroll
                for (int s = 0; s < 2; ++s) {
                    f32x16 c = acc[s][nt];
                    c = __builtin_amdgcn_mfma_f32_32x32x16_bf16(__builtin_bit_cast(bf16x8, A3[s]), b1, c, 0, 0, 0);
                    c = __builtin_amdgcn_mfma_f32_32x32x16_bf16(__builtin_bit_cast(bf16x8, A1[s]), b3, c, 0, 0, 0);
                    c = __builtin_amdgcn_mfma_f32_32x32x16_bf16(__builtin_bit_cast(bf16x8, A2[s]), b2, c, 0, 0, 0);
                    c = __builtin_amdgcn_mfma_f32_32x32x16_bf16(__builtin_bit_cast(bf16x8, A2[s]), b1, c, 0, 0, 0);
                    c = __builtin_amdgcn_mfma_f32_32x32x16_bf16(__builtin_bit_cast(bf16x8, A1[s]), b2, c, 0, 0, 0);
                    c = __builtin_amdgcn_mfma_f32_32x32x16_bf16(__builtin_bit_cast(bf16x8, A1[s]), b1, c, 0, 0, 0);
                    acc[s][nt] = c;
                }
            }
            __builtin_amdgcn_sched_barrier(0);
        }
        float* orow = a.out + (((size_t)b * a.Ho + oy) * a.Wo + ox0 + 4 * h) * a.Cout + col;
#pragma unroll
        for (int s = 0; s < 2; ++s)
#pragma unroll
            for (int nt = 0; nt < 2; ++nt)
#pragma unroll
                for (int i = 0; i < 16; ++i) {
                    float v = acc[s][nt][i] * sc[nt] + sh[nt];
                    if (a.relu) v = fmaxf(v, 0.f);
                    orow[(size_t)(32 * s + 8 * (i >> 2) + (i & 3)) * a.Cout + 32 * nt] = v;
                }
    }
}

constexpr int kSpLdsW = kStemKG * 2 * 2 * 1024;
constexpr int kSpHaloRows = 32;

__device__ __attribute__((noinline)) void stem_pool_halo(const char* img, const unsigned char* s_w, float* halo, int y0, int ox0, int Hi,
                                                         unsigned rowB, float sc0, float sc1, float sh0, float sh1) {
    const int lane = threadIdx.x & 63, col = lane & 31, h = lane >> 5;
    const float sc[2] = {sc0, sc1}, sh[2] = {sh0, sh1};
    float m1 = -1.f;
    asm volatile("" : "+s"(m1));
    auto masked = [](f32x3 v, unsigned m) {
        f32x4 o;
#pragma unroll
        for (int e = 0; e < 3; ++e) { const float x = v[e]; o[e] = __builtin_bit_cast(float, __builtin_bit_cast(unsigned, x) & m); }
        o[3] = 0.f;
        return o;
    };
                const int iyb = 2 * (y0 + col) - 3;
                const int ixh = 2 * (ox0 - 1) - 3 + 2 * h;
                f32x16 hacc[2];
    #pragma unroll
                for (int nt = 0; nt < 2; ++nt)
    #pragma unroll
                    for (int i = 0; i < 16; ++i) hacc[nt][i] = 0.f;
                constexpr int kPreH = 4;
                f32x3 hr[kPreH][2];
                unsigned hk[kPreH];
                auto hissue = [&](int j, f32x3 (&r)[2], unsigned& m) {
                    const int kh = j >> 1, g2 = j & 1, iy = iyb + kh;
                    m = (iy >= 0 && iy < Hi) ? 0xFFFFFFFFu : 0u;
                    const unsigned off = (unsigned)min(max(iy, 0), Hi - 1) * rowB + (unsigned)(ixh + 4 * g2) * 16u;
                    r[0] = *reinterpret_cast<const f32x3*>(img + off);
                    r[1] = *reinterpret_cast<const f32x3*>(img + off + 16u);
                };
    #pragma unroll
                for (int j = 0; j < kPreH; ++j) hissue(j, hr[j], hk[j]);
    #pragma unroll
                for (int j = 0; j < kStemKG; ++j) {
                    u32x2 p1, p2, q1, q2;
                    split_h2(masked(hr[j % kPreH][0], hk[j % kPreH]), m1, p1, p2);
                    split_h2(masked(hr[j % kPreH][1], hk[j % kPreH]), m1, q1, q2);
                    const u32x4 A1 = u32x4{p1[0], p1[1], q1[0], q1[1]}, A2 = u32x4{p2[0], p2[1], q2[0], q2[1]};
                    if (j + kPreH < kStemKG) hissue(j + kPreH, hr[j % kPreH], hk[j % kPreH]);
                    const unsigned char* wb = &s_w[(size_t)(j * 2 * 2) * 1024 + lane * 16];
    #pragma unroll
                    for (int nt = 0; nt < 2; ++nt) {
                        const f16x8 b1 = __builtin_bit_cast(f16x8, *reinterpret_cast<const u32x4*>(wb + (0 * 2 + nt) * 1024));
                        const f16x8 b2 = __builtin_bit_cast(f16x8, *reinterpret_cast<const u32x4*>(wb + (1 * 2 + nt) * 1024));
                        f32x16 c = hacc[nt];
                        c = __builtin_amdgcn_mfma_f32_32x32x16_f16(__builtin_bit_cast(f16x8, A2), b1, c, 0, 0, 0);
                        c = __builtin_amdgcn_mfma_f32_32x32x16_f16(__builtin_bit_cast(f16x8, A1), b2, c, 0, 0, 0);
                        c = __builtin_amdgcn_mfma_f32_32x32x16_f16(__builtin_bit_cast(f16x8, A1), b1, c, 0, 0, 0);
                        hacc[nt] = c;
                    }
                    __builtin_amdgcn_sched_barrier(0);
                }
    #pragma unroll
                for (int nt = 0; nt < 2; ++nt)
    #pragma unroll
                    for (int i = 0; i < 16; ++i)
                        halo[(8 * (i >> 2) + (i & 3) + 4 * h) * 64 + 32 * nt + col] = fmaxf(hacc[nt][i] * sc[nt] + sh[nt], 0.f);
                __builtin_amdgcn_fence(__ATOMIC_RELEASE, "wavefront");
                __builtin_amdgcn_wave_barrier();
                __builtin_amdgcn_fence(__ATOMIC_ACQUIRE, "wavefront");
}

__global__ __launch_bounds__(512, 1) void k_stem_pool_h3(const StemPoolArgs a) {
    __shared__ __attribute__((aligned(16))) unsigned char s_w[kSpLdsW];
    __shared__ float s_halo[8][kSpHaloRows][64];
    const int tid = threadIdx.x, lane = tid & 63, col = lane & 31, h = lane >> 5;
    const int wv = __builtin_amdgcn_readfirstlane(tid >> 6);
    for (int c = tid; c < kStemKG * 2 * 2 * 64; c += 512) {
        const int l = c & 63, nt = (c >> 6) & 1, pk = c >> 7, plane = pk & 1, kg = pk >> 1;
        const unsigned short* src = a.wpl + ((size_t)plane * a.Npad + nt * 32 + (l & 31)) * a.Kpad + 16 * kg + 8 * (l >> 5);
        *reinterpret_cast<u32x4*>(&s_w[(size_t)c * 16]) = *reinterpret_cast<const u32x4*>(src);
    }
    const float isc = reinterpret_cast<const float*>(a.wpl)[(size_t)a.Npad * a.Kpad];
    float sc[2], sh[2];
    sc[0] = (a.scale ? a.scale[col] : 1.f) * isc; sc[1] = (a.scale ? a.scale[32 + col] : 1.f) * isc;
    sh[0] = a.shift ? a.shift[col] : 0.f; sh[1] = a.shift ? a.shift[32 + col] : 0.f;
    float m1 = -1.f;
    asm volatile("" : "+s"(m1));
    __syncthreads();

    const int strips = a.Wo >> 6, bands = (a.Hp + a.band - 1) / a.band;
    const int ntask = a.B * bands * strips;
    int t_first = blockIdx.x * 8 + wv, t_end = ntask, t_step = gridDim.x * 8;
    if ((gridDim.x & 7) == 0) {
        const int per = (ntask + 7) >> 3, lo = (blockIdx.x & 7) * per;
        t_first = lo + (blockIdx.x >> 3) * 8 + wv; t_end = min(lo + per, ntask); t_step = (gridDim.x >> 3) * 8;
    }
    const unsigned rowB = (unsigned)a.Wi * 16u;
    auto masked = [](f32x3 v, unsigned m) {
        f32x4 o;
#pragma unroll
        for (int e = 0; e < 3; ++e) { const float x = v[e]; o[e] = __builtin_bit_cast(float, __builtin_bit_cast(unsigned, x) & m); }
        o[3] = 0.f;
        return o;
    };
    float* halo = &s_halo[wv][0][0];
    for (int task = t_first; task < t_end; task += t_step) {
        const int t2 = task / strips, strip = task - t2 * strips;
        const int b = t2 / bands, band = t2 - b * bands;
        const int r0 = band * a.band, nr = min(a.band, a.Hp - r0);
        const int y0 = 2 * r0 - 1;
        const int ox0 = strip * 64;
        const char* img = reinterpret_cast<const char*>(a.in + (size_t)b * a.Hi * a.Wi * 4);
        if (strip > 0) stem_pool_halo(img, s_w, halo, y0, ox0, a.Hi, rowB, sc[0], sc[1], sh[0], sh[1]);
        else {
#pragma unroll
            for (int i = 0; i < kSpHaloRows * 64 / 256; ++i) *reinterpret_cast<f32x4*>(&halo[(i * 64 + lane) * 4]) = f32x4{0.f, 0.f, 0.f, 0.f};
        }
        __builtin_amdgcn_fence(__ATOMIC_RELEASE, "wavefront");
        __builtin_amdgcn_wave_barrier();
        __builtin_amdgcn_fence(__ATOMIC_ACQUIRE, "wavefront");
        unsigned xoff[8], xm[8];
#pragma unroll
        for (int k = 0; k < 8; ++k) {
            const int ix = 2 * (ox0 + col) - 3 + 2 * h + 64 * (k >> 2) + 4 * ((k >> 1) & 1) + (k & 1);
            xm[k] = (ix >= 0 && ix < a.Wi) ? 0xFFFFFFFFu : 0u;
            xoff[k] = (unsigned)min(max(ix, 0), a.Wi - 1) * 16u;
        }
        constexpr int kPre = 4;
        f32x3 ring[kPre][4];
        auto issue = [&](int y, int j, f32x3 (&r)[4]) {
            const int kh = j >> 1, g2 = j & 1;
            const unsigned ro = (unsigned)min(max(2 * y - 3 + kh, 0), a.Hi - 1) * rowB;
#pragma unroll
            for (int q = 0; q < 4; ++q) r[q] = *reinterpret_cast<const f32x3*>(img + (ro + xoff[4 * (q >> 1) + 2 * g2 + (q & 1)]));
        };
        const unsigned olane = (unsigned)(2 * h * 64 + col) * 4u;
        float run[2][16];
#pragma unroll
        for (int nt = 0; nt < 2; ++nt)
#pragma unroll
            for (int i = 0; i < 16; ++i) run[nt][i] = 0.f;
        auto conv_row = [&](auto Mc, int y, int yn, int prow) {
            constexpr int MODE = decltype(Mc)::value;
            constexpr int SL = MODE == 1 ? 2 : 0;
            float hlv[2];
#pragma unroll
            for (int nt = 0; nt < 2; ++nt) hlv[nt] = halo[(y - y0) * 64 + 32 * nt + col];
            __builtin_amdgcn_sched_barrier(0);
            f32x16 acc[2][2];
#pragma unroll
            for (int s = 0; s < 2; ++s)
#pragma unroll
                for (int nt = 0; nt < 2; ++nt)
#pragma unroll
                    for (int i = 0; i < 16; ++i) acc[s][nt][i] = 0.f;
#pragma unroll
            for (int j = 0; j < kStemKG; ++j) {
                const int slot = (j + SL) % kPre;
                const int kh = j >> 1, g2 = j & 1;
                const int iy = 2 * y - 3 + kh;
                const unsigned rm = (iy >= 0 && iy < a.Hi) ? 0xFFFFFFFFu : 0u;
                const unsigned char* wb = &s_w[(size_t)(j * 2 * 2) * 1024 + lane * 16];
                f16x8 bw[2][2];
#pragma unroll
                for (int nt = 0; nt < 2; ++nt) {
                    bw[0][nt] = __builtin_bit_cast(f16x8, *reinterpret_cast<const u32x4*>(wb + (0 * 2 + nt) * 1024));
                    bw[1][nt] = __builtin_bit_cast(f16x8, *reinterpret_cast<const u32x4*>(wb + (1 * 2 + nt) * 1024));
                }
#pragma unroll
                for (int s = 0; s < 2; ++s) {
                    u32x2 p1, p2, q1, q2;
                    split_h2(masked(ring[slot][2 * s], xm[4 * s + 2 * g2] & rm), m1, p1, p2);
                    split_h2(masked(ring[slot][2 * s + 1], xm[4 * s + 2 * g2 + 1] & rm), m1, q1, q2);
                    const u32x4 A1 = u32x4{p1[0], p1[1], q1[0], q1[1]}, A2 = u32x4{p2[0], p2[1], q2[0], q2[1]};
#pragma unroll
                    for (int nt = 0; nt < 2; ++nt) {
                        f32x16 c = acc[s][nt];
                        c = __builtin_amdgcn_mfma_f32_32x32x16_f16(__builtin_bit_cast(f16x8, A2), bw[0][nt], c, 0, 0, 0);
                        c = __builtin_amdgcn_mfma_f32_32x32x16_f16(__builtin_bit_cast(f16x8, A1), bw[1][nt], c, 0, 0, 0);
                        c = __builtin_amdgcn_mfma_f32_32x32x16_f16(__builtin_bit_cast(f16x8, A1), bw[0][nt], c, 0, 0, 0);
                        acc[s][nt] = c;
                    }
                }
                if (j + kPre < kStemKG) issue(y, j + kPre, ring[slot]);
                else issue(yn, j + kPre - kStemKG, ring[slot]);
                __builtin_amdgcn_sched_barrier(0);
            }
#pragma unroll
            for (int nt = 0; nt < 2; ++nt) {
                float recv[8];
#pragma unroll
                for (int G = 0; G < 8; ++G)
                    recv[G] = __shfl_xor(fmaxf(acc[G >> 2][nt][4 * (G & 3) + 3] * sc[nt] + sh[nt], 0.f), 32, 64);
                const float hl = hlv[nt];
#pragma unroll
                for (int G = 0; G < 8; ++G) {
                    float v[4];
#pragma unroll
                    for (int e = 0; e < 4; ++e) v[e] = fmaxf(acc[G >> 2][nt][4 * (G & 3) + e] * sc[nt] + sh[nt], 0.f);
                    const float left = h ? recv[G] : (G ? recv[G ? G - 1 : 0] : hl);
                    const float hm0 = fmaxf(fmaxf(v[0], v[1]), left), hm1 = fmaxf(fmaxf(v[1], v[2]), v[3]);
                    if (MODE == 2) {
                        char* ob = reinterpret_cast<char*>(a.out + (((size_t)b * a.Hp + prow) * a.Wp + 32 * strip) * 64) + olane;
                        float* o = reinterpret_cast<float*>(ob) + (4 * G) * 64 + 32 * nt;
                        o[0] = fmaxf(run[nt][2 * G], hm0);
                        o[64] = fmaxf(run[nt][2 * G + 1], hm1);
                    }
                    if (MODE == 0) {
                        run[nt][2 * G] = y >= 0 ? hm0 : 0.f;
                        run[nt][2 * G + 1] = y >= 0 ? hm1 : 0.f;
                    } else if (MODE == 2) {
                        run[nt][2 * G] = hm0;
                        run[nt][2 * G + 1] = hm1;
                    } else {
                        run[nt][2 * G] = fmaxf(run[nt][2 * G], hm0);
                        run[nt][2 * G + 1] = fmaxf(run[nt][2 * G + 1], hm1);
                    }
                    __builtin_amdgcn_sched_barrier(0);
                }
            }
        };
#pragma unroll
        for (int j = 0; j < kPre; ++j) issue(y0, j, ring[j]);
        conv_row(std::integral_constant<int, 0>{}, y0, y0 + 1, 0);
        for (int p = 0; p < nr; ++p) {
            conv_row(std::integral_constant<int, 1>{}, y0 + 2 * p + 1, y0 + 2 * p + 2, 0);
            conv_row(std::integral_constant<int, 2>{}, y0 + 2 * p + 2, y0 + 2 * p + 3, r0 + p);
        }
    }
}

void stem_pool_tasks(int Ho, int Wo, int band, long long out4[4]) {
    const int Hp = Ho / 2, strips = Wo / 64, bands = (Hp + band - 1) / band;
    long long rows = 0;
    for (int bd = 0; bd < bands; ++bd) {
        const int r0 = bd * band, nr = std::min(band, Hp - r0);
        rows += 2 * nr + 1 - (r0 == 0 ? 1 : 0);
    }
    out4[0] = bands; out4[1] = strips;
    out4[2] = rows * Wo + (long long)bands * (strips - 1) * 32;
    out4[3] = (long long)Ho * Wo;
}

int launch_stem_pool_h3(const StemPoolArgs& a, hipStream_t s) {
    if (!a.in || !a.wpl || !a.out || a.B < 1 || !a.relu || a.Npad < 64 || a.Kpad != 224 || (a.Wo & 63) != 0 || a.Ho < 2 || (a.Ho & 1) ||
        a.Ho != (a.Hi + 6 - 7) / 2 + 1 || a.Wo != (a.Wi + 6 - 7) / 2 + 1 || a.Hp != a.Ho / 2 || a.Wp != a.Wo / 2 ||
        a.band < 1 || 2 * a.band + 1 > kSpHaloRows || (long long)a.Hi * a.Wi * 16 >= (1LL << 31))
        return FPC_EINVAL;
    const long long tasks = (long long)a.B * ((a.Hp + a.band - 1) / a.band) * (a.Wo >> 6);
    if (tasks >= (1LL << 31) - 8 * 4096) return FPC_EINVAL;
    const int grid = (int)std::min<long long>(a.grid > 0 ? a.grid : 256, (tasks + 7) / 8);
    hipLaunchKernelGGL(k_stem_pool_h3, dim3(grid), dim3(512), 0, s, a);
    return check_launch();
}

int launch_stem7x7(const StemArgs& a, hipStream_t s) {
    if (!a.in || !a.wpl || !a.out || a.B < 1 || a.Cout != 64 || a.Npad < 64 || a.Kpad != 224 || (a.Wo & 63) != 0 || a.Ho < 1 ||
        a.Ho != (a.Hi + 6 - 7) / 2 + 1 || a.Wo != (a.Wi + 6 - 7) / 2 + 1 || (long long)a.Hi * a.Wi * 4 >= (1LL << 31))
        return FPC_EINVAL;
    const long long waves = (long long)a.B * a.Ho * (a.Wo >> 6);
    if (waves >= (1LL << 31) - 8 * 4096) return FPC_EINVAL;
    const int grid = (int)std::min<long long>(a.grid > 0 ? a.grid : 256, (waves + 7) / 8);
    hipLaunchKernelGGL(k_stem7x7, dim3(grid), dim3(512), 0, s, a);
    return check_launch();
}

}
```

fastposecnn_amd/engine.py:

```python
import ctypes
import operator

import torch

from fastposecnn_amd import _native as nat


_DATA_PTR = torch.Tensor.data_ptr
_VERSION = operator.attrgetter('_version')

class NetEngine:

    def __init__(self, model, B, H, W, device, autotune=True, tune_mode=0, graph=False, split_precision=False):
        L = nat.lib()
        self._lib = L
        self.B, self.H, self.W, self.device = B, H, W, device
        self.classes = model.classes
        h = ctypes.c_void_p()
        from fastposecnn_amd.lib import backbone
        block, layers = backbone.encoder_layout(model.encoder.name)
        groups, width = backbone.encoder_groups(model.encoder.name)
        reduction = backbone.encoder_reduction(model.encoder.name)
        if reduction:
            nat.check(L.fpc_net_create_encoder_se((ctypes.c_int * 4)(*layers), reduction, self.classes, B, H, W, ctypes.byref(h)),
                      "fpc_net_create_encoder_se")
        elif groups > 1:
            nat.check(L.fpc_net_create_encoder_ex(block, (ctypes.c_int * 4)(*layers), groups, width, self.classes, B, H, W,
                                                  ctypes.byref(h)), "fpc_net_create_encoder_ex")
        elif block == 1:
            nat.check(L.fpc_net_create(model.encoder.name.encode(), self.classes, B, H, W, ctypes.byref(h)), "fpc_net_create")
        else:
            nat.check(L.fpc_net_create_encoder(block, (ctypes.c_int * 4)(*layers), self.classes, B, H, W, ctypes.byref(h)),
                      "fpc_net_create_encoder")
        self._h = h
        self._names = [L.fpc_net_param_name(h, i).decode() for i in range(L.fpc_net_param_count(h))]
        nbytes = L.fpc_net_workspace_bytes(h)
        with torch.cuda.device(device):
            self._ws = torch.empty(nbytes, dtype=torch.uint8, device=device)
            assert self._ws.data_ptr() % 256 == 0
        self.reloads = 0
        self.generation = 0
        self.guard_forwards = 0
        self.bind(model)
        if split_precision:
            nat.check(L.fpc_net_set_split_precision(h, int(split_precision)), "fpc_net_set_split_precision")
        if autotune:
            nat.check(L.fpc_net_autotune_next(h, int(tune_mode)), "fpc_net_autotune_next")
            self.forward(torch.zeros((B, 3, H, W), dtype=torch.float32, device=device), want_logits=False)
        if graph:
            nat.check(L.fpc_net_set_graph(h, 1), "fpc_net_set_graph")

    def bind(self, model):
        L, h, device = self._lib, self._h, self.device
        tensors = dict(model.named_parameters())
        tensors.update(dict(model.named_buffers()))
        params = []
        for i, name in enumerate(self._names):
            if name not in tensors:
                raise RuntimeError(f"fastposecnn_amd: the model has no parameter {name!r} (smp naming expected)")
            t = tensors[name]
            if t.device != device or t.dtype != torch.float32 or not t.is_contiguous():
                raise RuntimeError(f"fastposecnn_amd: parameter {name!r} must be a contiguous f32 tensor on {device}")
            if t.numel() != L.fpc_net_param_numel(h, i):
                raise RuntimeError(f"fastposecnn_amd: parameter {name!r} has {t.numel()} elements, expected "
                                   f"{L.fpc_net_param_numel(h, i)}")
            params.append(t)
        self._params = params
        n = len(params)
        ptrs = (ctypes.c_void_p * n)(*[t.data_ptr() for t in params])
        with torch.cuda.device(device):
            nat.check(L.fpc_net_load_params(h, ptrs, n, self._ws.data_ptr(), self._ws.numel(), nat.stream()),
                      "fpc_net_load_params")
        self._stamp = self._fingerprint()
        self.reloads += 1

    def _fingerprint(self):
        return (tuple(map(_DATA_PTR, self._params)), tuple(map(_VERSION, self._params)))

    def stale(self):
        return self._fingerprint() != self._stamp

    def conv_plans(self):
        out = []
        buf = (ctypes.c_int * 5)()
        for i in range(self._lib.fpc_net_conv_count(self._h)):
            self._lib.fpc_net_conv_plan(self._h, i, buf)
            out.append(tuple(buf))
        return out

    def copy_plans_from(self, other):
        nat.check(self._lib.fpc_net_copy_plans(self._h, other._h), "fpc_net_copy_plans")

    def force_winograd(self, form):
        rc = self._lib.fpc_net_force_winograd(self._h, int(form))
        if rc < 0:
            nat.check(rc, "fpc_net_force_winograd")
        return rc

    def force_fold(self, on):
        rc = self._lib.fpc_net_force_fold(self._h, int(on))
        if rc < 0:
            nat.check(rc, "fpc_net_force_fold")
        return rc

    def force_direct_h3(self, on):
        rc = self._lib.fpc_net_force_direct_h3(self._h, int(on))
        if rc < 0:
            nat.check(rc, "fpc_net_force_direct_h3")
        return rc

    def force_stem_pool(self, on):
        rc = self._lib.fpc_net_force_stem_pool(self._h, int(on))
        if rc < 0:
            nat.check(rc, "fpc_net_force_stem_pool")
        return rc

    def survey(self, x, want_logits=True):
        if tuple(x.shape) != (self.B, 3, self.H, self.W) or x.device != self.device:
            raise RuntimeError("NetEngine.survey: input shape / device does not match the plan")
        sites = self._lib.fpc_net_conv_count(self._h)
        with torch.cuda.device(self.device):
            rec = torch.zeros((sites, 4), dtype=torch.int32, device=self.device)
            nat.check(self._lib.fpc_net_survey_next(self._h, rec.data_ptr(), sites), "fpc_net_survey_next")
        try:
            logits, cat = self.forward(x, want_logits=want_logits)
        finally:
            self._lib.fpc_net_survey_next(self._h, None, sites)
        return logits, cat, rec.cpu().to(torch.int64) & 0xFFFFFFFF

    @staticmethod
    def record_max(records):
        return (records[:, 0] & 0xFFFFFFFF).to(torch.int32).view(torch.float32) if records.dtype == torch.int64 \
            else records[:, 0].contiguous().view(torch.float32)

    def guard_ranges(self, records, lo=2.0 ** -2, hi=2.0 ** 14):
        sites = self._lib.fpc_net_conv_count(self._h)
        flat = [int(v) & 0xFFFFFFFF for v in records.reshape(-1).tolist()]
        if len(flat) != 4 * sites:
            raise RuntimeError("NetEngine.guard_ranges: records must be [sites, 4]")
        before = set(self.guarded())
        rc = self._lib.fpc_net_guard_ranges(self._h, (ctypes.c_uint32 * len(flat))(*flat), sites, float(lo), float(hi))
        if rc < 0:
            nat.check(rc, "fpc_net_guard_ranges")
        return [i for i in self.guarded() if i not in before]

    def guarded(self):
        return [i for i in range(self._lib.fpc_net_conv_count(self._h)) if self._lib.fpc_net_guarded(self._h, i)]

    def graph_recorded(self):
        return bool(self._lib.fpc_net_graph_recorded(self._h))

    def set_wino_pack(self, on):
        nat.check(self._lib.fpc_net_set_wino_pack(self._h, int(on)), "fpc_net_set_wino_pack")

    def set_wino_orient(self, on):
        nat.check(self._lib.fpc_net_set_wino_orient(self._h, int(on)), "fpc_net_set_wino_orient")

    def wino_blocks(self):
        return int(self._lib.fpc_net_wino_blocks(self._h))

    def force_pointwise(self, on):
        rc = self._lib.fpc_net_force_pointwise(self._h, int(on))
        if rc < 0:
            nat.check(rc, "fpc_net_force_pointwise")
        return rc

    def flops(self):
        buf = (ctypes.c_double * 3)()
        nat.check(self._lib.fpc_net_flops(self._h, buf), "fpc_net_flops")
        return tuple(buf)

    def __del__(self):
        h = getattr(self, "_h", None)
        if h:
            self._lib.fpc_net_destroy(h)
            self._h = None

    def forward(self, x, want_logits=True):
        B, H, W, C, dev = self.B, self.H, self.W, self.classes, self.device
        G = C - 1
        if tuple(x.shape) != (B, 3, H, W) or x.device != dev:
            raise RuntimeError("NetEngine.forward: input shape / device does not match the plan")
        if x.dtype != torch.float32 or not x.is_contiguous():
            x = x.float().contiguous()
        f32 = dict(dtype=torch.float32, device=dev)
        logits = None
        lp = [None] * 5
        if want_logits:
            logits = {'mask': torch.empty((B, C, H, W), **f32), 'quaternion': torch.empty((B, 4 * G, H, W), **f32),
                      'scales': torch.empty((B, 3 * G, H, W), **f32), 'xy': torch.empty((B, 2 * G, H, W), **f32),
                      'z': torch.empty((B, G, H, W), **f32)}
            lp = [logits[k].data_ptr() for k in ('mask', 'quaternion', 'scales', 'xy', 'z')]
        cat = {'mask': torch.empty((B, H, W), dtype=torch.int64, device=dev),
               'quaternion': torch.empty((B, 4, H, W), **f32), 'scales': torch.empty((B, 3, H, W), **f32),
               'xy': torch.empty((B, 2, H, W), **f32), 'z': torch.empty((B, H, W), **f32)}
        bits = None
        if W % 64 == 0 and self._lib.fpc_cc_bits_supported(B, H, W):
            bits = torch.empty((B, self._lib.fpc_mask_bits_words(H, W)), dtype=torch.int64, device=dev)
        with torch.cuda.device(dev):
            nat.check(self._lib.fpc_net_forward_bits(self._h, x.data_ptr(), *lp, cat['mask'].data_ptr(),
                                                     cat['quaternion'].data_ptr(), cat['scales'].data_ptr(),
                                                     cat['xy'].data_ptr(), cat['z'].data_ptr(), nat.ptr(bits), nat.stream()),
                      "fpc_net_forward_bits")
        if bits is not None:
            cat['mask']._fpc_fg_bits = (bits, cat['mask']._version)
        return logits, cat

    def tensor(self, name):
        p = ctypes.c_void_p()
        H, W, C = ctypes.c_int(), ctypes.c_int(), ctypes.c_int()
        nat.check(self._lib.fpc_net_tensor(self._h, name.encode(), ctypes.byref(p), ctypes.byref(H), ctypes.byref(W),
                                           ctypes.byref(C)), "fpc_net_tensor")
        off = p.value - self._ws.data_ptr()
        n = self.B * H.value * W.value * C.value
        return self._ws[off:off + 4 * n].view(torch.float32).view(self.B, H.value, W.value, C.value)
```

include/fpc.h:

```cpp
#ifndef FPC_H_
#define FPC_H_

#include <stddef.h>
#include <stdint.h>

#ifdef __cplusplus
extern "C" {
#endif

#define FPC_ABI_VERSION 11

#define FPC_OK 0
#define FPC_EINVAL (-1)
#define FPC_EWORKSPACE (-2)
#define FPC_ELAUNCH (-3)
#define FPC_EDEVICE (-4)
#define FPC_EFORMAT (-5)

typedef void* fpc_stream_t;

int fpc_abi_version(void);
const char* fpc_error_string(int code);
const char* fpc_last_hip_error(void);

// ... 65 lines not shown
int fpc_aggregate(const int32_t* labels, const int64_t* cat_mask,
                  const float* quat, const float* scales, const float* xy, const float* z,
                  int B, int H, int W, int N, const int32_t* n_dev,
                  int64_t* class_ids, int64_t* sample_ids, float* inst_masks,
                  float* oq, float* os, float* oz, float* oxy, float* out_stats,
                  void* ws, size_t ws_bytes, fpc_stream_t stream);
size_t fpc_mask_bits_words(int H, int W);
int fpc_aggregate_bits(const int32_t* labels, const int64_t* cat_mask,
                       const float* quat, const float* scales, const float* xy, const float* z,
                       int B, int H, int W, int N, const int32_t* n_dev,
                       int64_t* class_ids, int64_t* sample_ids, float* inst_masks,
                       float* oq, float* os, float* oz, float* oxy, float* out_stats, uint64_t* inst_bits,
                       const int32_t* root_pix, void* ws, size_t ws_bytes, fpc_stream_t stream);

int fpc_pose_rt(const float* q, const float* xy, const float* z, const float* kinv, int n,
                float* R, float* T, float* RT, fpc_stream_t stream);

int fpc_pack_pose_records(const int64_t* sample_ids, const int64_t* class_ids, const float* q, const float* scales,
                          const float* xy, const float* z, const float* R, const float* T, const float* RT, int n,
                          int sample_offset, int capacity, float* out, fpc_stream_t stream);

size_t fpc_mask_iou_workspace_bytes(int n1, int n2, int64_t hw);
int fpc_mask_iou(const void* masks1, int n1, const void* masks2, int n2, int64_t hw, int elem_size,
                 float* iou, int32_t* inter, int32_t* uni, void* ws, size_t ws_bytes, fpc_stream_t stream);

size_t fpc_preprocess_workspace_bytes(int B);
int fpc_preprocess_u8(const uint8_t* img_hwc, int B, int H, int W, const double* mean3, const double* std3,
                      int input_range_01, float* out_nchw, void* ws, size_t ws_bytes, fpc_stream_t stream);

int fpc_png_info(const uint8_t* data, size_t nbytes, int32_t* out5);
int fpc_png_decode(const uint8_t* data, size_t nbytes, void* out, size_t out_bytes, int mode);
int fpc_png_decode_batch(const uint8_t* const* datas, const size_t* sizes, int n, uint8_t* out, int H, int W, int threads);

#define FPC_PNG_DESC_WORDS 8
#define FPC_INF_ETRUNCATED 1
#define FPC_INF_EBLOCK_TYPE 2
#define FPC_INF_ESTORED_LEN 3
#define FPC_INF_EOVERSUBSCRIBED 4
#define FPC_INF_EINCOMPLETE 5
#define FPC_INF_EREPEAT_FIRST 6
#define FPC_INF_ELITLEN_SYMBOL 7
#define FPC_INF_EDIST_SYMBOL 8
#define FPC_INF_EDIST_TOO_FAR 9
#define FPC_INF_EOUT_OVERFLOW 10
#define FPC_INF_EOUT_SHORT 11
#define FPC_INF_EADLER 12
#define FPC_INF_EFDICT 13
#define FPC_INF_EMETHOD 14
#define FPC_INF_EFCHECK 15
#define FPC_INF_ELENGTHS_OVERRUN 16
#define FPC_INF_ENO_END_CODE 17
#define FPC_INF_EBAD_CODE 18
#define FPC_PNG_EDESC 20
#define FPC_PNG_EFILTER 21
int fpc_inflate_host(const uint8_t* in, size_t zbytes, uint8_t* out, size_t cap, size_t* out_len);
size_t fpc_png_pack_bytes(int n, int H, int W);
int fpc_png_pack_batch(const uint8_t* const* datas, const size_t* sizes, int n, int H, int W, int mode, uint8_t* staging,
                       size_t staging_bytes, int64_t* desc, size_t* used);
size_t fpc_png_decode_device_workspace_bytes(int n, int H, int W, int max_bpp);
int fpc_png_decode_device(const uint8_t* staging, size_t staging_bytes, const int64_t* desc, int n, int H, int W, int mode,
                          int max_bpp, void* out, size_t frame_bytes, int32_t* status, void* workspace, size_t workspace_bytes,
                          fpc_stream_t stream);

int fpc_gt_build(const uint8_t* ids, int64_t pix_stride, int64_t frame_stride, int B, int H, int W,
                 const int16_t* row_of, const uint8_t* class_of, const int32_t* first_row, int n,
                 int64_t* class_mask, void* inst_masks, int mask_elem, int32_t* pix_count, fpc_stream_t stream);
int fpc_depth_decode(const void* src, int src_kind, int channels, int B, int H, int W, float* depth_f32, fpc_stream_t stream);

int fpc_pose_errors(const float* q0, const float* q1, const int64_t* symmetric_ids, const float* rot, int nrot,
                    const float* RT1, const float* RT2, const float* scales1, const float* scales2,
                    const float* T1, const float* T2, int n, double* out_degree, float* out_iou3d, float* out_offset,
                    fpc_stream_t stream);

size_t fpc_pose_metrics_state_words(int num_classes, int n_deg, int n_iou, int n_off, int n_complex);
int fpc_pose_metrics_update(const int32_t* order, const int32_t* match_pred, const int32_t* count, int n1, int n2,
                            const float* gt_quaternion, const float* gt_RT, const float* gt_scales, const float* gt_T,
                            const int64_t* symmetric_ids, const int64_t* class_ids, const float* quaternion, const float* RT,
                            const float* scales, const float* T, const float* rot, int nrot, const double* thr_degree, int n_deg,
                            const double* thr_iou, int n_iou, const double* thr_offset, int n_off, const double* thr_complex,
                            int n_complex, const double* thr_table, int num_classes, int64_t* state, double* raw_degree,
                            float* raw_iou, float* raw_offset, int32_t* raw_class, int raw_capacity, fpc_stream_t stream);

int fpc_confusion_update(const int64_t* pred, const int64_t* gt, int64_t n, int num_classes, int64_t* state, fpc_stream_t stream);

int fpc_post_network_backward(const int32_t* labels, const float* cat_xy, int B, int H, int W, int N,
                              const int32_t* n_dev, const double* table, float inlier_thresh, int max_num,
                              uint64_t seed, const uint8_t* keep, float* g_q, float* g_s, float* g_xy, float* g_z,
                              fpc_stream_t stream);
int fpc_vote_refine_backward(const float* mask, const float* vertex, int64_t vs_n, int64_t vs_h, int64_t vs_w,
                             int64_t vs_c, int n, int H, int W, const double* table, float inlier_thresh, int max_num,
                             uint64_t seed, const uint8_t* keep, float* g_vertex, fpc_stream_t stream);
int fpc_class_compress_backward(const int64_t* cat_mask, const float* quat, const float* xy, const float* go_q,
                                const float* go_s, const float* go_xy, const float* go_z, int B, int C, int HW,
                                float* g_q, float* g_s, float* g_xy, float* g_z, fpc_stream_t stream);
int fpc_mask_losses(const float* logits, const int64_t* target, int B, int C, int HW, int64_t ignore_ce,
                    int64_t ignore_cce, float alpha, float gamma, double* sums6, const float* w3, float* grad,
                    fpc_stream_t stream);
#define FPC_MATCH_MAX_INSTANCES 1024
int fpc_match_assign(const float* iou, const int64_t* gt_cls, const int64_t* pred_cls, int n1, int n2, int32_t* match_pred,
                     int32_t* order, int32_t* count, fpc_stream_t stream);
#define FPC_LOSS_L2 0
#define FPC_LOSS_L1 1
#define FPC_LOSS_SMOOTH_L1 2
int fpc_matched_losses(const int32_t* order, const int32_t* match_pred, const int32_t* count, int n1, int n2,
                       const float* gt_quaternion, const float* gt_xy, const float* gt_z, const float* gt_scales,
                       const int64_t* symmetric_ids, const float* quaternion, const float* xy, const float* z,
                       const float* scales, const float* rot, int nrot, double eps, int xy_type, int z_type, int scales_type,
                       const double* weights, double* losses, double* task_total, double* matched_total, int32_t* best_rot,
                       fpc_stream_t stream);
int fpc_matched_losses_backward(const int32_t* order, const int32_t* match_pred, const int32_t* count, int n1, int n2,
                                const float* gt_quaternion, const float* gt_xy, const float* gt_z, const float* gt_scales,
                                const int64_t* symmetric_ids, const float* quaternion, const float* xy, const float* z,
                                const float* scales, const float* rot, int nrot, double eps, int xy_type, int z_type,
                                int scales_type, const double* weights, const double* losses, const int32_t* best_rot,
                                const double* g_losses, float* g_quaternion, float* g_xy, float* g_z, float* g_scales,
                                fpc_stream_t stream);
int fpc_grad_sumsq(const float* g, size_t n, double* out2, fpc_stream_t stream);
int fpc_lookahead_radam_step(float* p, const float* g, float* m, float* v, float* slow, size_t n, float lr, float beta1,
                             float beta2, float eps, float weight_decay, int64_t step, int la_k, float la_alpha,
                             const float* ctl, fpc_stream_t stream);

typedef struct fpc_net fpc_net_t;
int fpc_net_create(const char* encoder, int classes, int B, int H, int W, fpc_net_t** out);
int fpc_net_create_encoder(int block, const int* layers4, int classes, int B, int H, int W, fpc_net_t** out);
int fpc_net_create_encoder_ex(int block, const int* layers4, int groups, int width_per_group, int classes, int B, int H, int W,
                              fpc_net_t** out);
int fpc_net_create_encoder_se(const int* layers4, int reduction, int classes, int B, int H, int W, fpc_net_t** out);
void fpc_net_destroy(fpc_net_t* net);
int fpc_net_param_count(const fpc_net_t* net);
const char* fpc_net_param_name(const fpc_net_t* net, int i);
int64_t fpc_net_param_numel(const fpc_net_t* net, int i);
size_t fpc_net_workspace_bytes(const fpc_net_t* net);
int fpc_net_load_params(fpc_net_t* net, const float* const* params, int count, void* ws, size_t ws_bytes,
                        fpc_stream_t stream);
int fpc_net_forward(fpc_net_t* net, const float* x, float* logits_mask, float* logits_quat,
                    float* logits_scales, float* logits_xy, float* logits_z, int64_t* cat_mask,
                    float* cq, float* cs, float* cxy, float* cz, fpc_stream_t stream);
int fpc_net_forward_bits(fpc_net_t* net, const float* x, float* logits_mask, float* logits_quat,
                         float* logits_scales, float* logits_xy, float* logits_z, int64_t* cat_mask,
                         float* cq, float* cs, float* cxy, float* cz, uint64_t* fg_bits, fpc_stream_t stream);

int fpc_net_autotune_next(fpc_net_t* net, int mode );
int fpc_net_set_split_precision(fpc_net_t* net, int on);
int fpc_net_set_graph(fpc_net_t* net, int on);
int fpc_net_graph_recorded(const fpc_net_t* net);
int fpc_net_conv_count(const fpc_net_t* net);
int fpc_net_conv_plan(const fpc_net_t* net, int i, int* out5);
int fpc_net_copy_plans(fpc_net_t* dst, const fpc_net_t* src);
int fpc_net_force_winograd(fpc_net_t* net, int form);
int fpc_net_force_pointwise(fpc_net_t* net, int on);
int fpc_net_force_fold(fpc_net_t* net, int on);
int fpc_net_force_direct_h3(fpc_net_t* net, int on);
int fpc_net_force_stem_pool(fpc_net_t* net, int on);
int fpc_act_range(const float* x, long long n, unsigned* rec4, fpc_stream_t stream);
int fpc_net_survey_next(fpc_net_t* net, unsigned* records_dev, int sites);
int fpc_net_guard_ranges(fpc_net_t* net, const unsigned* records_host, int sites, float lo, float hi);
int fpc_net_guarded(const fpc_net_t* net, int i);
int fpc_stem_pool_tasks(int Ho, int Wo, int64_t* out4);
int fpc_wino_pack_geometry(int H, int W, int B, int Cin, int fold, int64_t* out8);
int fpc_net_set_wino_pack(fpc_net_t* net, int on);
int fpc_net_set_wino_orient(fpc_net_t* net, int on);
int fpc_wino_orient_geometry(int H, int W, int B, int Cin, int fold, int pack, int64_t* out9);
int fpc_wino_recip(uint32_t d, int64_t* out2);
int fpc_wino_decode(int Cout, int groups, int tbx, int tby, int W, int B, int pack, int64_t* out14);
int64_t fpc_net_wino_blocks(const fpc_net_t* net);
int fpc_net_flops(const fpc_net_t* net, double* out3);
int fpc_net_tensor(const fpc_net_t* net, const char* name, const float** ptr, int* H, int* W, int* C);

enum {
    FPC_PLAN_WINO_ORIENT = -11, FPC_PLAN_WINO_PACKED = -10, FPC_PLAN_TWO_LAUNCH = 100, FPC_PLAN_BF3 = 1000, FPC_PLAN_LATERAL = 2000, FPC_PLAN_STEM = 3000,
    FPC_PLAN_STEM_POOL = 3100, FPC_PLAN_POINTWISE = 4000, FPC_PLAN_FOLDED = 5000, FPC_PLAN_H3 = 6000, FPC_PLAN_LATERAL_H3 = 7000,
    FPC_PLAN_GROUPED = 8000
};
size_t fpc_conv2d_workspace_bytes(int B, int Ho, int Wo, int Cin, int Cout, int Kh, int Kw);
size_t fpc_conv2d_workspace_bytes_for(int B, int Ho, int Wo, int Cin, int Cout, int Kh, int Kw, int bm, int bn, int nsplit);
int fpc_conv2d_plan(int B, int Ho, int Wo, int Cin, int Cout, int Kh, int Kw, int bm, int bn, int nsplit,
                    int* out4 );
int fpc_conv2d(const float* in, int64_t sb, int64_t sh, int64_t sw, int64_t sc, const float* w_oihw,
               const float* scale, const float* shift, const float* res, const float* up, float* out,
               float* gn_part, int B, int Hi, int Wi, int Cin, int Cout, int Kh, int Kw, int stride, int pad,
               int relu, int bm, int bn, int nsplit, void* ws, size_t ws_bytes, fpc_stream_t stream);

size_t fpc_conv2d_grouped_workspace_bytes(int C, int groups);
int fpc_conv2d_grouped(const float* in, int64_t sb, int64_t sh, int64_t sw, int64_t sc, const float* w_oihw, const float* scale,
                       const float* shift, float* out, int B, int Hi, int Wi, int C, int groups, int stride, int relu, int form,
                       void* ws, size_t ws_bytes, fpc_stream_t stream);

size_t fpc_conv2d_grouped_dgrad_workspace_bytes(int C, int groups);
int fpc_conv2d_grouped_dgrad(const float* dy, const float* w_oihw, float* dx, int B, int Hi, int Wi, int C, int groups, int stride,
                             void* ws, size_t ws_bytes, fpc_stream_t stream);
size_t fpc_conv2d_grouped_wgrad_workspace_bytes(int B, int Ho, int Wo, int C, int groups);
int fpc_conv2d_grouped_wgrad(const float* x, int64_t sb, int64_t sh, int64_t sw, const float* dy, float* dw, int B, int Hi, int Wi,
                             int C, int groups, int stride, void* ws, size_t ws_bytes, fpc_stream_t stream);

int fpc_image_nhwc4(const float* x, float* out, int B, int H, int W, fpc_stream_t stream);
size_t fpc_stem_wgrad_workspace_bytes(int B, int Hi, int Wi);
int fpc_stem_wgrad_slices(int B, int Hi, int Wi);
int fpc_stem_wgrad(const float* img4, const float* dy, float* dw, int B, int Hi, int Wi, void* ws, size_t ws_bytes,
                   fpc_stream_t stream);
int fpc_maxpool3x3s2_fwd(const float* x, float* y, int B, int Hi, int Wi, int C, fpc_stream_t stream);
int fpc_maxpool3x3s2_bwd(const float* x, const float* dy, float* dx, int B, int Hi, int Wi, int C, fpc_stream_t stream);

int fpc_se_pool_slabs(int H, int W, int C);
size_t fpc_se_scratch_floats(int B, int H, int W, int C);
int fpc_se_gate(const float* x, const float* w1, const float* b1, const float* w2, const float* b2, float* gate, float* scratch, int B,
                int H, int W, int C, int R, fpc_stream_t stream);
int fpc_se_scale_add_relu(const float* x, const float* gate, const float* res, float* y, int B, int H, int W, int C,
                          fpc_stream_t stream);
int fpc_maxpool3x3s2_ceil_fwd(const float* x, float* y, int B, int Hi, int Wi, int C, fpc_stream_t stream);

size_t fpc_conv2d_wgrad_workspace_bytes(int B, int Ho, int Wo, int Cin, int Cout, int Kh, int Kw);
int fpc_conv2d_wgrad(const float* x, int64_t sb, int64_t sh, int64_t sw, const float* dy, float* dw, int B, int Hi,
                     int Wi, int Cin, int Cout, int Kh, int Kw, int stride, int pad, void* ws, size_t ws_bytes,
                     fpc_stream_t stream);
int fpc_conv2d_wgrad_split(const float* x, int64_t sb, int64_t sh, int64_t sw, const float* dy, float* dw, int B, int Hi,
                           int Wi, int Cin, int Cout, int Kh, int Kw, int stride, int pad, void* ws, size_t ws_bytes,
                           fpc_stream_t stream);

int fpc_upsample_bilinear_fwd(const float* in, int64_t sb, int64_t sc, int64_t sh, int64_t sw, float* out, int B, int C, int h,
                              int w, int scale, int out_nhwc, fpc_stream_t stream);
size_t fpc_upsample_bilinear_bwd_scratch_floats(int B, int C, int h, int w, int scale);
int fpc_upsample_bilinear_bwd(const float* dout, int64_t sb, int64_t sc, int64_t sh, int64_t sw, float* din, float* scratch,
                              int B, int C, int h, int w, int scale, int din_nhwc, fpc_stream_t stream);

size_t fpc_groupnorm4_relu_scratch_floats(int B, int HW, int C);
int fpc_groupnorm4_relu_fwd(const float* x, const float* gamma, const float* beta, float* y, float* stats, float* part, int B,
                            int HW, int C, int groups, float eps, fpc_stream_t stream);
int fpc_groupnorm4_relu_bwd(const float* x, const float* dy, const float* gamma, const float* beta, const float* stats, float* dx,
                            float* part, int B, int HW, int C, int groups, fpc_stream_t stream);

size_t fpc_batchnorm_scratch_floats(int P, int C);
int fpc_batchnorm_fwd(const float* x, const float* res, const float* gamma, const float* beta, float* running_mean,
                      float* running_var, float* y, float* stats, float* part, int P, int C, float eps, float momentum, int relu,
                      fpc_stream_t stream);
int fpc_batchnorm_bwd(const float* x, const float* y, const float* dy, const float* gamma, const float* stats, float* dx,
                      float* dres, float* dgamma, float* dbeta, float* part, int P, int C, int relu, fpc_stream_t stream);

#ifdef __cplusplus
}
#endif
#endif
```

tools_dev/frame_timeline.py:

```python
import csv, sys
rows = list(csv.DictReader(open(sys.argv[1])))
rows.sort(key=lambda r: int(r['Start_Timestamp']))
idx = [i for i, r in enumerate(rows) if 'nchw3_to_nhwc4' in r['Kernel_Name']]
s, e = idx[-3], idx[-2]
t0 = int(rows[s]['Start_Timestamp'])
tot = 0; cat = {}
for r in rows[s:e]:
    d = (int(r['End_Timestamp']) - int(r['Start_Timestamp'])) / 1e3
    tot += d
    nm = r['Kernel_Name']
    key = nm.split('(')[0].replace('void ', '').replace('fpc::', '')[:40]
    cat[key] = cat.get(key, 0) + d
    if '--all' in sys.argv:
        print(f"{(int(r['Start_Timestamp'])-t0)/1e3:9.1f} {d:8.2f} grid=({int(r['Grid_Size_X'])//int(r['Workgroup_Size_X'])},{r['Grid_Size_Y']},{r['Grid_Size_Z']}) {nm[:70]}")
print('sum of kernels %.1f us, span %.1f us, %d dispatches' % (tot, (int(rows[e]['Start_Timestamp']) - t0) / 1e3, e - s))
for k, v in sorted(cat.items(), key=lambda kv: -kv[1]):
    print(f"{v:9.1f} us  {k}")
```

Baseline: 2845.

## Read NCHW input directly in fused stem conv+pool, skipping layout conversion

Adds a planar variant of the fused stem 7x7 conv + maxpool kernel that reads the 3-channel NCHW input directly, with a repacked weight image using K=176 instead of 224. This removes the separate nchw3_to_nhwc4 conversion launch and its round trip through memory, and reduces padded MFMA work. The autotuner now times the planar, fused and paired variants, each including the layout cost, and picks one. The packed planar weights are stored in the stem activation buffer, so they are repacked whenever that buffer may have been overwritten, which adds bookkeeping risk.

```diff
diff --git a/fastposecnn_amd/_native.py b/fastposecnn_amd/_native.py
--- a/fastposecnn_amd/_native.py
+++ b/fastposecnn_amd/_native.py
@@ -95,6 +95,7 @@
     "fpc_net_force_fold": (_i, [_vp, _i]),
     "fpc_net_force_direct_h3": (_i, [_vp, _i]),
     "fpc_net_force_stem_pool": (_i, [_vp, _i]),
+    "fpc_net_stem_reads_planar": (_i, [_vp]),
     "fpc_act_range": (_i, [_vp, ctypes.c_longlong, _vp, _vp]),
     "fpc_net_survey_next": (_i, [_vp, _vp, _i]),
     "fpc_net_guard_ranges": (_i, [_vp, ctypes.POINTER(ctypes.c_uint32), _i, _f, _f]),
diff --git a/fastposecnn_amd/csrc/net.hip b/fastposecnn_amd/csrc/net.hip
--- a/fastposecnn_amd/csrc/net.hip
+++ b/fastposecnn_amd/csrc/net.hip
@@ -270,6 +270,9 @@
     bool h3_packed = false;
     hipStream_t load_stream = nullptr;
     size_t stem_h3_off = 0;
+    bool stem_h3p_ok = false;
+    bool stem_planar = true;
+    const float* x_cur = nullptr;
     bool fold_ok = false;
     size_t fold_wc_off[4] = {}, fold_img1_off[4] = {}, fold_img2_off[4] = {}, fold_tab_off[4] = {};
 
@@ -612,6 +615,17 @@
     delete n;
 }
 
+static bool stem_h3p_fits(const fpc_net* n) {
+    return (size_t)n->B * n->a_stem.H * n->a_stem.W * n->a_stem.C >= h3_packed_floats(n->convs[n->c_stem].Npad, kStemPlanarK);
+}
+static int ensure_stem_h3p(fpc_net* n, hipStream_t s) {
+    if (n->stem_h3p_ok) return FPC_OK;
+    const PackedConv& st = n->convs[n->c_stem];
+    const int rc = launch_pack_weight_h3p(n->pptr[st.p_w], n->ws + n->a_stem.off, st.Cout, st.Npad, s);
+    if (!rc) n->stem_h3p_ok = true;
+    return rc;
+}
+
 static int pack_h3_images(fpc_net* n, hipStream_t s) {
     for (const PackedConv& c : n->convs)
         if (c.h3_ok) {
@@ -622,7 +636,8 @@
     int rc = launch_pack_weight_h3(n->pptr[st.p_w], n->ws + n->stem_h3_off, st.Cout, st.Cin, st.Cinp, st.Kh, st.Kw, st.Kwp, st.Npad, st.Kpad, s);
     if (rc) return rc;
     n->h3_packed = true;
-    return FPC_OK;
+    n->stem_h3p_ok = false;
+    return stem_h3p_fits(n) ? ensure_stem_h3p(n, s) : FPC_OK;
 }
 
 extern "C" int fpc_net_set_split_precision(fpc_net_t* n, int on) {
@@ -1024,7 +1039,25 @@
     return launch_stem_pool_h3(t, s);
 }
 
-static int forward_middle(fpc_net* n, hipStream_t s) {
+static int launch_stem_pool_planar(const float* x, long long x_sb, const float* h3p_image, const float* scale, const float* shift, float* pool,
+                                   int B, int Hi, int Wi, int Npad, int relu, hipStream_t s) {
+    if (!x || !h3p_image) return FPC_EINVAL;
+    StemPoolArgs t;
+    memset(&t, 0, sizeof(t));
+    t.in = x; t.wpl = reinterpret_cast<const unsigned short*>(h3p_image); t.out = pool;
+    t.scale = scale; t.shift = shift;
+    t.B = B; t.Hi = Hi; t.Wi = Wi; t.Ho = conv_out(Hi, 7, 2, 3); t.Wo = conv_out(Wi, 7, 2, 3); t.Hp = t.Ho / 2; t.Wp = t.Wo / 2;
+    t.Npad = Npad; t.Kpad = kStemPlanarK; t.relu = relu;
+    t.band = kStemPoolBand; t.grid = 256;
+    t.planar = 1; t.in_sb = x_sb;
+    return launch_stem_pool_h3(t, s);
+}
+
+static bool stem_runs_planar(const fpc_net* n) {
+    return !n->se && n->cplan[n->c_stem].pool && n->stem_planar && n->h3_packed && !(n->W & 1) && stem_h3p_fits(n);
+}
+
+static int forward_middle(fpc_net* n, hipStream_t s, bool stem_done) {
     float* ws = n->ws;
     n->wino_blocks = 0;
     const int B = n->B, H = n->H, W = n->W;
@@ -1032,7 +1065,7 @@
     auto nhwc = [&](const Act& t, long long& sb, long long& sh, long long& sw, long long& sc) {
         sc = 1; sw = t.C; sh = (long long)t.W * t.C; sb = (long long)t.H * sh;
     };
-    {
+    if (!stem_done) {
         const PackedConv& c = n->convs[n->c_stem];
         fill_conv_args(n, a, c, n->cplan[n->c_stem], H, W, n->a_stem.H, n->a_stem.W, (long long)4 * H * W, (long long)4 * W, 4,
                        1, true, 0);
@@ -1044,23 +1077,47 @@
         };
         if (n->se) {
             n->cplan[n->c_stem].pool = 0;
+            n->stem_h3p_ok = false;
             FPC_TRY(run_conv(n, a, 1, n->c_stem, s));
             FPC_TRY(launch_maxpool3x3s2_ceil(ws + n->a_stem.off, ws + n->a_pool.off, B, n->a_stem.H, n->a_stem.W, 64, s));
         } else if (n->cplan[n->c_stem].pool && !n->tuning) {
             if (n->survey) FPC_TRY(survey_site(n, a, n->cplan[n->c_stem], 1, n->c_stem, s));
-            FPC_TRY(launch_stem_pool(a, h3img, ws + n->a_pool.off, n->a_pool.H, n->a_pool.W, s));
+            if (stem_runs_planar(n)) {
+                FPC_TRY(ensure_stem_h3p(n, s));
+                FPC_TRY(launch_stem_pool_planar(n->x_cur, (long long)3 * H * W, ws + n->a_stem.off, a.p[0].scale, a.p[0].shift, ws + n->a_pool.off,
+                                                B, H, W, a.Npad, 1, s));
+            } else {
+                FPC_TRY(launch_stem_pool(a, h3img, ws + n->a_pool.off, n->a_pool.H, n->a_pool.W, s));
+            }
         } else {
             n->cplan[n->c_stem].pool = 0;
+            n->stem_h3p_ok = false;
             FPC_TRY(run_conv(n, a, 1, n->c_stem, s));
             FPC_TRY(pool_launch());
             if (n->tuning && n->split_precision >= 3 && !n->guarded[n->c_stem] && launch_stem_pool(a, h3img, ws + n->a_pool.off, n->a_pool.H, n->a_pool.W, s) == FPC_OK) {
                 const ConvPlan cur = n->cplan[n->c_stem];
-                float ms_pair = 1e30f, ms_fused = 1e30f;
+                const float* x = n->x_cur;
+                const float* h3pimg = ws + n->a_stem.off;
+                auto layout = [&]() { return x ? launch_nchw3_to_nhwc4(x, ws + n->a_img4.off, B, H * W, s) : FPC_OK; };
+                auto planar = [&]() { return launch_stem_pool_planar(x, (long long)3 * H * W, h3pimg, a.p[0].scale, a.p[0].shift, ws + n->a_pool.off, B, H, W, a.Npad, 1, s); };
+                const bool try_planar = x && !(W & 1) && stem_h3p_fits(n);
+                float ms_pair = 1e30f, ms_fused = 1e30f, ms_planar = 1e30f;
                 for (int rep = 0; rep < 3; ++rep) {
-                    ms_pair = std::min(ms_pair, min_ms(s, 1, [&] { int rc = launch_conv_plan(a, cur, 1, s); return rc ? rc : pool_launch(); }));
-                    ms_fused = std::min(ms_fused, min_ms(s, 1, [&] { return launch_stem_pool(a, h3img, ws + n->a_pool.off, n->a_pool.H, n->a_pool.W, s); }));
+                    ms_pair = std::min(ms_pair, min_ms(s, 1, [&] { int rc = layout(); if (!rc) rc = launch_conv_plan(a, cur, 1, s); return rc ? rc : pool_launch(); }));
+                    ms_fused = std::min(ms_fused, min_ms(s, 1, [&] { int rc = layout(); return rc ? rc : launch_stem_pool(a, h3img, ws + n->a_pool.off, n->a_pool.H, n->a_pool.W, s); }));
+                    if (try_planar) {
+                        n->stem_h3p_ok = false;
+                        if (ensure_stem_h3p(n, s) == FPC_OK) ms_planar = std::min(ms_planar, min_ms(s, 1, planar));
+                    }
                 }
-                if (ms_fused < ms_pair) { ConvPlan q; q.stem = 256; q.pool = 1; n->cplan[n->c_stem] = q; }
+                if (std::min(ms_fused, ms_planar) < ms_pair) {
+                    ConvPlan q; q.stem = 256; q.pool = 1; n->cplan[n->c_stem] = q;
+                    n->stem_planar = ms_planar <= ms_fused;
+                } else if (try_planar) {
+                    n->stem_h3p_ok = false;
+                    FPC_TRY(launch_conv_plan(a, cur, 1, s));
+                    FPC_TRY(pool_launch());
+                }
             }
         }
     }
@@ -1292,12 +1349,21 @@
     float* ws = n->ws;
     const int B = n->B, H = n->H, W = n->W;
 
-    FPC_TRY(launch_nchw3_to_nhwc4(x, ws + n->a_img4.off, B, H * W, s));
     const bool plain = n->tuning || n->survey;
+    const bool planar = stem_runs_planar(n) && !n->tuning;
+    const bool stem_done = planar && !plain;
+    n->x_cur = x;
+    if (!planar || plain) FPC_TRY(launch_nchw3_to_nhwc4(x, ws + n->a_img4.off, B, H * W, s));
+    if (stem_done) {
+        const PackedConv& c = n->convs[n->c_stem];
+        FPC_TRY(ensure_stem_h3p(n, s));
+        FPC_TRY(launch_stem_pool_planar(x, (long long)3 * H * W, ws + n->a_stem.off, ws + c.scale_off, ws + c.shift_off, ws + n->a_pool.off, B, H, W,
+                                        c.Npad, 1, s));
+    }
     if (n->use_graph && !plain && s != nullptr && !n->graph_exec) {
         hipGraph_t g = nullptr;
         if (hipStreamBeginCapture(s, hipStreamCaptureModeThreadLocal) == hipSuccess) {
-            int rc = forward_middle(n, s);
+            int rc = forward_middle(n, s, stem_done);
             hipError_t e = hipStreamEndCapture(s, &g);
             if (rc) { if (g) (void)hipGraphDestroy(g); return rc; }
             if (e == hipSuccess && g) e = hipGraphInstantiate(&n->graph_exec, g, nullptr, nullptr, 0);
@@ -1309,7 +1375,7 @@
     if (n->use_graph && !plain && s != nullptr && n->graph_exec) {
         if (hipGraphLaunch(n->graph_exec, s) != hipSuccess) return FPC_ELAUNCH;
     } else {
-        FPC_TRY(forward_middle(n, s));
+        FPC_TRY(forward_middle(n, s, stem_done));
     }
     {
         Up4Args u;
@@ -1472,6 +1538,7 @@
     ConvPlan q;
     q.stem = 256; q.pool = on;
     p = q;
+    n->stem_planar = true;
     n->guarded[n->c_stem] = 0;
     drop_graph(n);
     return 1;
@@ -1501,9 +1568,15 @@
         dst->guarded[i] = dst->guarded[i] || src->guarded[i];
         if (dst->guarded[i] && plan_range_limited(dst->cplan[i])) dst->cplan[i] = range_free_plan(dst, (int)i);
     }
+    dst->stem_planar = src->stem_planar;
     dst->tuned = true;
     drop_graph(dst);
     return FPC_OK;
+}
+
+extern "C" int fpc_net_stem_reads_planar(const fpc_net_t* n) {
+    if (!n || !n->loaded) return FPC_EINVAL;
+    return stem_runs_planar(n) ? 1 : 0;
 }
 
 extern "C" int fpc_net_flops(const fpc_net_t* n, double* out3) {
@@ -1660,6 +1733,12 @@
     c.K = Cin * Kh * Kw; c.Kpad = cdiv(c.K, kConvBK) * kConvBK; c.Npad = cdiv(Cout, kConvNAlign) * kConvNAlign;
     hipStream_t s = (hipStream_t)stream;
     float* packed = (float*)ws;
+    if (rq.stem && rq.pool && Cin == 3) {
+        if (Kh != 7 || stride != 2 || pad != 3 || Cout != 64 || sw != 1 || sh != (int64_t)Wi || sc != (int64_t)Hi * Wi || res || up || gn_part)
+            return FPC_EINVAL;
+        FPC_TRY(launch_pack_weight_h3p(w_oihw, packed, Cout, c.Npad, s));
+        return launch_stem_pool_planar(in, sb, packed, scale, shift, out, B, Hi, Wi, c.Npad, relu, s);
+    }
     if (rq.stem) {
         if (Cin != 4 || Kh != 7 || stride != 2 || pad != 3 || Cout != 64 || sc != 1 || sw != 4 || sh != (int64_t)4 * Wi ||
             sb != (int64_t)4 * Hi * Wi || res || up || gn_part)
diff --git a/fastposecnn_amd/csrc/net_kernels.hpp b/fastposecnn_amd/csrc/net_kernels.hpp
--- a/fastposecnn_amd/csrc/net_kernels.hpp
+++ b/fastposecnn_amd/csrc/net_kernels.hpp
@@ -118,9 +118,13 @@
     int B, Hi, Wi, Ho, Wo, Hp, Wp, Npad, Kpad, relu;
     int band;
     int grid;
+    int planar;
+    long long in_sb;
 };
 constexpr int kStemPoolBand = 10;
+constexpr int kStemPlanarK = 176;
 int launch_stem_pool_h3(const StemPoolArgs& a, hipStream_t s);
+int launch_pack_weight_h3p(const float* w_oihw, float* packed, int Cout, int Npad, hipStream_t s);
 void stem_pool_tasks(int Ho, int Wo, int band, long long out4[4]);
 
 constexpr int kMaxGnSites = 4;
diff --git a/fastposecnn_amd/csrc/stem.hip b/fastposecnn_amd/csrc/stem.hip
--- a/fastposecnn_amd/csrc/stem.hip
+++ b/fastposecnn_amd/csrc/stem.hip
@@ -117,7 +117,6 @@
     }
 }
 
-constexpr int kSpLdsW = kStemKG * 2 * 2 * 1024;
 constexpr int kSpHaloRows = 32;
 
 __device__ __attribute__((noinline)) void stem_pool_halo(const char* img, const unsigned char* s_w, float* halo, int y0, int ox0, int Hi,
@@ -182,12 +181,84 @@
                 __builtin_amdgcn_fence(__ATOMIC_ACQUIRE, "wavefront");
 }
 
+
+constexpr int kStemKGp = kStemPlanarK / 16;
+typedef float f32x2 __attribute__((ext_vector_type(2)));
+typedef f32x2 f32x2u __attribute__((aligned(4)));
+typedef f32x4 f32x4u __attribute__((aligned(4)));
+
+__device__ __attribute__((noinline)) void stem_pool_halo_p(const char* img, const unsigned char* s_w, float* halo, int y0, int ox0, int Hi,
+                                                           unsigned rowB, unsigned planeB, float sc0, float sc1, float sh0, float sh1) {
+    const int lane = threadIdx.x & 63, col = lane & 31, h = lane >> 5;
+    const float sc[2] = {sc0, sc1}, sh[2] = {sh0, sh1};
+    float m1 = -1.f;
+    asm volatile("" : "+s"(m1));
+    auto masked = [](f32x4 v, unsigned m) {
+        f32x4 o;
+#pragma unroll
+        for (int e = 0; e < 4; ++e) { const float x = v[e]; o[e] = __builtin_bit_cast(float, __builtin_bit_cast(unsigned, x) & m); }
+        return o;
+    };
+    const int iyb = 2 * (y0 + col) - 3;
+    const unsigned xb = (unsigned)(2 * (ox0 - 1) - 3) * 4u;
+    f32x16 hacc[2];
+#pragma unroll
+    for (int nt = 0; nt < 2; ++nt)
+#pragma unroll
+        for (int i = 0; i < 16; ++i) hacc[nt][i] = 0.f;
+    constexpr int kPreH = 4;
+    f32x4 hr[kPreH][2];
+    unsigned hk[kPreH];
+    auto hissue = [&](int j, f32x4 (&r)[2], unsigned& m) {
+        const int c0 = 2 * j, c1 = 2 * j + 1 < 21 ? 2 * j + 1 : 20;
+        const int kh = h ? c1 / 3 : c0 / 3, ch = h ? c1 % 3 : c0 % 3, iy = iyb + kh;
+        m = (iy >= 0 && iy < Hi && !(h && 2 * j + 1 >= 21)) ? 0xFFFFFFFFu : 0u;
+        const unsigned off = (unsigned)ch * planeB + (unsigned)min(max(iy, 0), Hi - 1) * rowB + xb;
+        r[0] = *reinterpret_cast<const f32x4u*>(img + off);
+        r[1] = *reinterpret_cast<const f32x4u*>(img + off + 16u);
+    };
+#pragma unroll
+    for (int j = 0; j < kPreH; ++j) hissue(j, hr[j], hk[j]);
+#pragma unroll
+    for (int j = 0; j < kStemKGp; ++j) {
+        u32x2 p1, p2, q1, q2;
+        split_h2(masked(hr[j % kPreH][0], hk[j % kPreH]), m1, p1, p2);
+        f32x4 hi4 = masked(hr[j % kPreH][1], hk[j % kPreH]);
+        hi4[3] = 0.f;
+        split_h2(hi4, m1, q1, q2);
+        const u32x4 A1 = u32x4{p1[0], p1[1], q1[0], q1[1]}, A2 = u32x4{p2[0], p2[1], q2[0], q2[1]};
+        if (j + kPreH < kStemKGp) hissue(j + kPreH, hr[j % kPreH], hk[j % kPreH]);
+        const unsigned char* wb = &s_w[(size_t)(j * 2 * 2) * 1024 + lane * 16];
+#pragma unroll
+        for (int nt = 0; nt < 2; ++nt) {
+            const f16x8 b1 = __builtin_bit_cast(f16x8, *reinterpret_cast<const u32x4*>(wb + (0 * 2 + nt) * 1024));
+            const f16x8 b2 = __builtin_bit_cast(f16x8, *reinterpret_cast<const u32x4*>(wb + (1 * 2 + nt) * 1024));
+            f32x16 c = hacc[nt];
+            c = __builtin_amdgcn_mfma_f32_32x32x16_f16(__builtin_bit_cast(f16x8, A2), b1, c, 0, 0, 0);
+            c = __builtin_amdgcn_mfma_f32_32x32x16_f16(__builtin_bit_cast(f16x8, A1), b2, c, 0, 0, 0);
+            c = __builtin_amdgcn_mfma_f32_32x32x16_f16(__builtin_bit_cast(f16x8, A1), b1, c, 0, 0, 0);
+            hacc[nt] = c;
+        }
+        __builtin_amdgcn_sched_barrier(0);
+    }
+#pragma unroll
+    for (int nt = 0; nt < 2; ++nt)
+#pragma unroll
+        for (int i = 0; i < 16; ++i)
+            halo[(8 * (i >> 2) + (i & 3) + 4 * h) * 64 + 32 * nt + col] = fmaxf(hacc[nt][i] * sc[nt] + sh[nt], 0.f);
+    __builtin_amdgcn_fence(__ATOMIC_RELEASE, "wavefront");
+    __builtin_amdgcn_wave_barrier();
+    __builtin_amdgcn_fence(__ATOMIC_ACQUIRE, "wavefront");
+}
+
+template <bool PL>
 __global__ __launch_bounds__(512, 1) void k_stem_pool_h3(const StemPoolArgs a) {
-    __shared__ __attribute__((aligned(16))) unsigned char s_w[kSpLdsW];
+    constexpr int KG = PL ? kStemKGp : kStemKG;
+    __shared__ __attribute__((aligned(16))) unsigned char s_w[KG * 2 * 2 * 1024];
     __shared__ float s_halo[8][kSpHaloRows][64];
     const int tid = threadIdx.x, lane = tid & 63, col = lane & 31, h = lane >> 5;
     const int wv = __builtin_amdgcn_readfirstlane(tid >> 6);
-    for (int c = tid; c < kStemKG * 2 * 2 * 64; c += 512) {
+    for (int c = tid; c < KG * 2 * 2 * 64; c += 512) {
         const int l = c & 63, nt = (c >> 6) & 1, pk = c >> 7, plane = pk & 1, kg = pk >> 1;
         const unsigned short* src = a.wpl + ((size_t)plane * a.Npad + nt * 32 + (l & 31)) * a.Kpad + 16 * kg + 8 * (l >> 5);
         *reinterpret_cast<u32x4*>(&s_w[(size_t)c * 16]) = *reinterpret_cast<const u32x4*>(src);
@@ -207,7 +278,9 @@
         const int per = (ntask + 7) >> 3, lo = (blockIdx.x & 7) * per;
         t_first = lo + (blockIdx.x >> 3) * 8 + wv; t_end = min(lo + per, ntask); t_step = (gridDim.x >> 3) * 8;
     }
-    const unsigned rowB = (unsigned)a.Wi * 16u;
+    const unsigned rowB = (unsigned)a.Wi * (PL ? 4u : 16u);
+    const unsigned planeB = (unsigned)a.Hi * rowB;
+    const bool hb = h != 0;
     auto masked = [](f32x3 v, unsigned m) {
         f32x4 o;
 #pragma unroll
@@ -222,24 +295,56 @@
         const int r0 = band * a.band, nr = min(a.band, a.Hp - r0);
         const int y0 = 2 * r0 - 1;
         const int ox0 = strip * 64;
-        const char* img = reinterpret_cast<const char*>(a.in + (size_t)b * a.Hi * a.Wi * 4);
-        if (strip > 0) stem_pool_halo(img, s_w, halo, y0, ox0, a.Hi, rowB, sc[0], sc[1], sh[0], sh[1]);
-        else {
+        const char* img = reinterpret_cast<const char*>(a.in + (PL ? (size_t)b * a.in_sb : (size_t)b * a.Hi * a.Wi * 4));
+        if (strip > 0) {
+            if constexpr (PL) stem_pool_halo_p(img, s_w, halo, y0, ox0, a.Hi, rowB, planeB, sc[0], sc[1], sh[0], sh[1]);
+            else stem_pool_halo(img, s_w, halo, y0, ox0, a.Hi, rowB, sc[0], sc[1], sh[0], sh[1]);
+        } else {
 #pragma unroll
             for (int i = 0; i < kSpHaloRows * 64 / 256; ++i) *reinterpret_cast<f32x4*>(&halo[(i * 64 + lane) * 4]) = f32x4{0.f, 0.f, 0.f, 0.f};
         }
         __builtin_amdgcn_fence(__ATOMIC_RELEASE, "wavefront");
         __builtin_amdgcn_wave_barrier();
         __builtin_amdgcn_fence(__ATOMIC_ACQUIRE, "wavefront");
-        unsigned xoff[8], xm[8];
-#pragma unroll
-        for (int k = 0; k < 8; ++k) {
-            const int ix = 2 * (ox0 + col) - 3 + 2 * h + 64 * (k >> 2) + 4 * ((k >> 1) & 1) + (k & 1);
-            xm[k] = (ix >= 0 && ix < a.Wi) ? 0xFFFFFFFFu : 0u;
-            xoff[k] = (unsigned)min(max(ix, 0), a.Wi - 1) * 16u;
+        unsigned xoff[8], xm[PL ? 3 : 8];
+        bool selL3 = false, selL1 = false, selR = false;
+        if constexpr (PL) {
+#pragma unroll
+            for (int s = 0; s < 2; ++s) {
+                const int xs = 2 * (ox0 + 32 * s + col) - 3;
+                xoff[3 * s + 0] = (unsigned)max(xs, 0) * 4u;
+                xoff[3 * s + 1] = (unsigned)min(xs + 4, a.Wi - 2) * 4u;
+                xoff[3 * s + 2] = (unsigned)min(xs + 6, a.Wi - 1) * 4u;
+            }
+            const int xs0 = 2 * (ox0 + col) - 3, xs1 = xs0 + 64;
+            selL3 = xs0 == -3; selL1 = xs0 == -1; selR = xs1 + 6 >= a.Wi;
+            xm[0] = xs0 >= 0 ? 0xFFFFFFFFu : 0u;
+            xm[1] = xs0 + 1 >= 0 ? 0xFFFFFFFFu : 0u;
+            xm[2] = selR ? 0u : 0xFFFFFFFFu;
+        } else {
+#pragma unroll
+            for (int k = 0; k < 8; ++k) {
+                const int ix = 2 * (ox0 + col) - 3 + 2 * h + 64 * (k >> 2) + 4 * ((k >> 1) & 1) + (k & 1);
+                xm[k] = (ix >= 0 && ix < a.Wi) ? 0xFFFFFFFFu : 0u;
+                xoff[k] = (unsigned)min(max(ix, 0), a.Wi - 1) * 16u;
+            }
         }
         constexpr int kPre = 4;
         f32x3 ring[kPre][4];
+        float ringp[kPre][2][7];
+        auto issue_p = [&](int y, int j, float (&r)[2][7]) {
+            const int c0 = 2 * j, c1 = 2 * j + 1 < 21 ? 2 * j + 1 : 20;
+            const unsigned ro0 = (unsigned)(c0 % 3) * planeB + (unsigned)min(max(2 * y - 3 + c0 / 3, 0), a.Hi - 1) * rowB;
+            const unsigned ro1 = (unsigned)(c1 % 3) * planeB + (unsigned)min(max(2 * y - 3 + c1 / 3, 0), a.Hi - 1) * rowB;
+            const unsigned ro = hb ? ro1 : ro0;
+#pragma unroll
+            for (int s = 0; s < 2; ++s) {
+                const f32x4 t0 = *reinterpret_cast<const f32x4u*>(img + (ro + xoff[3 * s + 0]));
+                const f32x2 t1 = *reinterpret_cast<const f32x2u*>(img + (ro + xoff[3 * s + 1]));
+                r[s][0] = t0[0]; r[s][1] = t0[1]; r[s][2] = t0[2]; r[s][3] = t0[3]; r[s][4] = t1[0]; r[s][5] = t1[1];
+                r[s][6] = *reinterpret_cast<const float*>(img + (ro + xoff[3 * s + 2]));
+            }
+        };
         auto issue = [&](int y, int j, f32x3 (&r)[4]) {
             const int kh = j >> 1, g2 = j & 1;
             const unsigned ro = (unsigned)min(max(2 * y - 3 + kh, 0), a.Hi - 1) * rowB;
@@ -252,13 +357,15 @@
         for (int nt = 0; nt < 2; ++nt)
 #pragma unroll
             for (int i = 0; i < 16; ++i) run[nt][i] = 0.f;
-        auto conv_row = [&](auto Mc, int y, int yn, int prow) {
+        auto conv_row = [&](auto Mc, auto Sc, int y, int yn, int prow) {
             constexpr int MODE = decltype(Mc)::value;
-            constexpr int SL = MODE == 1 ? 2 : 0;
+            constexpr int SL = decltype(Sc)::value;
             float hlv[2];
-#pragma unroll
-            for (int nt = 0; nt < 2; ++nt) hlv[nt] = halo[(y - y0) * 64 + 32 * nt + col];
-            __builtin_amdgcn_sched_barrier(0);
+            if constexpr (!PL) {
+#pragma unroll
+                for (int nt = 0; nt < 2; ++nt) hlv[nt] = halo[(y - y0) * 64 + 32 * nt + col];
+                __builtin_amdgcn_sched_barrier(0);
+            }
             f32x16 acc[2][2];
 #pragma unroll
             for (int s = 0; s < 2; ++s)
@@ -267,11 +374,17 @@
 #pragma unroll
                     for (int i = 0; i < 16; ++i) acc[s][nt][i] = 0.f;
 #pragma unroll
-            for (int j = 0; j < kStemKG; ++j) {
+            for (int j = 0; j < KG; ++j) {
                 const int slot = (j + SL) % kPre;
                 const int kh = j >> 1, g2 = j & 1;
                 const int iy = 2 * y - 3 + kh;
-                const unsigned rm = (iy >= 0 && iy < a.Hi) ? 0xFFFFFFFFu : 0u;
+                unsigned rm = (iy >= 0 && iy < a.Hi) ? 0xFFFFFFFFu : 0u;
+                if constexpr (PL) {
+                    const int i0 = 2 * y - 3 + (2 * j) / 3, i1 = 2 * y - 3 + (2 * j + 1) / 3;
+                    const unsigned rm0 = (i0 >= 0 && i0 < a.Hi) ? 0xFFFFFFFFu : 0u;
+                    const unsigned rm1 = (2 * j + 1 < 21 && i1 >= 0 && i1 < a.Hi) ? 0xFFFFFFFFu : 0u;
+                    rm = hb ? rm1 : rm0;
+                }
                 const unsigned char* wb = &s_w[(size_t)(j * 2 * 2) * 1024 + lane * 16];
                 f16x8 bw[2][2];
 #pragma unroll
@@ -282,8 +395,24 @@
 #pragma unroll
                 for (int s = 0; s < 2; ++s) {
                     u32x2 p1, p2, q1, q2;
-                    split_h2(masked(ring[slot][2 * s], xm[4 * s + 2 * g2] & rm), m1, p1, p2);
-                    split_h2(masked(ring[slot][2 * s + 1], xm[4 * s + 2 * g2 + 1] & rm), m1, q1, q2);
+                    if constexpr (PL) {
+                        const float(&r)[7] = ringp[slot][s];
+                        auto keep = [](float x, unsigned m) { return __builtin_bit_cast(float, __builtin_bit_cast(unsigned, x) & m); };
+                        if (s == 0) {
+                            const unsigned k0 = xm[0] & rm, k1 = xm[1] & rm;
+                            const float t1 = selL1 ? r[0] : r[1], t2 = selL1 ? r[1] : r[2], t3 = selL3 ? r[0] : (selL1 ? r[2] : r[3]);
+                            split_h2(f32x4{keep(r[0], k0), keep(t1, k1), keep(t2, k1), keep(t3, rm)}, m1, p1, p2);
+                            split_h2(f32x4{keep(r[4], rm), keep(r[5], rm), keep(r[6], rm), 0.f}, m1, q1, q2);
+                        } else {
+                            const unsigned k2 = xm[2] & rm;
+                            const float t4 = selR ? r[5] : r[4];
+                            split_h2(f32x4{keep(r[0], rm), keep(r[1], rm), keep(r[2], rm), keep(r[3], rm)}, m1, p1, p2);
+                            split_h2(f32x4{keep(t4, rm), keep(r[5], k2), keep(r[6], k2), 0.f}, m1, q1, q2);
+                        }
+                    } else {
+                        split_h2(masked(ring[slot][2 * s], xm[4 * s + 2 * g2] & rm), m1, p1, p2);
+                        split_h2(masked(ring[slot][2 * s + 1], xm[4 * s + 2 * g2 + 1] & rm), m1, q1, q2);
+                    }
                     const u32x4 A1 = u32x4{p1[0], p1[1], q1[0], q1[1]}, A2 = u32x4{p2[0], p2[1], q2[0], q2[1]};
 #pragma unroll
                     for (int nt = 0; nt < 2; ++nt) {
@@ -294,8 +423,18 @@
                         acc[s][nt] = c;
                     }
                 }
-                if (j + kPre < kStemKG) issue(y, j + kPre, ring[slot]);
-                else issue(yn, j + kPre - kStemKG, ring[slot]);
+                if constexpr (PL) {
+                    if (j + kPre < KG) issue_p(y, j + kPre, ringp[slot]);
+                    else issue_p(yn, j + kPre - KG, ringp[slot]);
+                } else {
+                    if (j + kPre < KG) issue(y, j + kPre, ring[slot]);
+                    else issue(yn, j + kPre - KG, ring[slot]);
+                }
+                __builtin_amdgcn_sched_barrier(0);
+            }
+            if constexpr (PL) {
+#pragma unroll
+                for (int nt = 0; nt < 2; ++nt) hlv[nt] = halo[(y - y0) * 64 + 32 * nt + col];
                 __builtin_amdgcn_sched_barrier(0);
             }
 #pragma unroll
@@ -332,12 +471,30 @@
                 }
             }
         };
-#pragma unroll
-        for (int j = 0; j < kPre; ++j) issue(y0, j, ring[j]);
-        conv_row(std::integral_constant<int, 0>{}, y0, y0 + 1, 0);
-        for (int p = 0; p < nr; ++p) {
-            conv_row(std::integral_constant<int, 1>{}, y0 + 2 * p + 1, y0 + 2 * p + 2, 0);
-            conv_row(std::integral_constant<int, 2>{}, y0 + 2 * p + 2, y0 + 2 * p + 3, r0 + p);
+        using std::integral_constant;
+        if constexpr (PL) {
+#pragma unroll
+            for (int j = 0; j < kPre; ++j) issue_p(y0, j, ringp[j]);
+            conv_row(integral_constant<int, 0>{}, integral_constant<int, 0>{}, y0, y0 + 1, 0);
+            int p = 0;
+            for (; p + 1 < nr; p += 2) {
+                conv_row(integral_constant<int, 1>{}, integral_constant<int, 3>{}, y0 + 2 * p + 1, y0 + 2 * p + 2, 0);
+                conv_row(integral_constant<int, 2>{}, integral_constant<int, 2>{}, y0 + 2 * p + 2, y0 + 2 * p + 3, r0 + p);
+                conv_row(integral_constant<int, 1>{}, integral_constant<int, 1>{}, y0 + 2 * p + 3, y0 + 2 * p + 4, 0);
+                conv_row(integral_constant<int, 2>{}, integral_constant<int, 0>{}, y0 + 2 * p + 4, y0 + 2 * p + 5, r0 + p + 1);
+            }
+            if (p < nr) {
+                conv_row(integral_constant<int, 1>{}, integral_constant<int, 3>{}, y0 + 2 * p + 1, y0 + 2 * p + 2, 0);
+                conv_row(integral_constant<int, 2>{}, integral_constant<int, 2>{}, y0 + 2 * p + 2, y0 + 2 * p + 3, r0 + p);
+            }
+        } else {
+#pragma unroll
+            for (int j = 0; j < kPre; ++j) issue(y0, j, ring[j]);
+            conv_row(integral_constant<int, 0>{}, integral_constant<int, 0>{}, y0, y0 + 1, 0);
+            for (int p = 0; p < nr; ++p) {
+                conv_row(integral_constant<int, 1>{}, integral_constant<int, 2>{}, y0 + 2 * p + 1, y0 + 2 * p + 2, 0);
+                conv_row(integral_constant<int, 2>{}, integral_constant<int, 0>{}, y0 + 2 * p + 2, y0 + 2 * p + 3, r0 + p);
+            }
         }
     }
 }
@@ -355,14 +512,49 @@
 }
 
 int launch_stem_pool_h3(const StemPoolArgs& a, hipStream_t s) {
-    if (!a.in || !a.wpl || !a.out || a.B < 1 || !a.relu || a.Npad < 64 || a.Kpad != 224 || (a.Wo & 63) != 0 || a.Ho < 2 || (a.Ho & 1) ||
+    if (!a.in || !a.wpl || !a.out || a.B < 1 || !a.relu || a.Npad < 64 || a.Kpad != (a.planar ? kStemPlanarK : 224) || (a.Wo & 63) != 0 ||
+        a.Ho < 2 || (a.Ho & 1) ||
         a.Ho != (a.Hi + 6 - 7) / 2 + 1 || a.Wo != (a.Wi + 6 - 7) / 2 + 1 || a.Hp != a.Ho / 2 || a.Wp != a.Wo / 2 ||
         a.band < 1 || 2 * a.band + 1 > kSpHaloRows || (long long)a.Hi * a.Wi * 16 >= (1LL << 31))
         return FPC_EINVAL;
+    if (a.planar && ((a.Wi & 1) || a.in_sb < 3LL * a.Hi * a.Wi || ((uintptr_t)a.in & 3))) return FPC_EINVAL;
     const long long tasks = (long long)a.B * ((a.Hp + a.band - 1) / a.band) * (a.Wo >> 6);
     if (tasks >= (1LL << 31) - 8 * 4096) return FPC_EINVAL;
     const int grid = (int)std::min<long long>(a.grid > 0 ? a.grid : 256, (tasks + 7) / 8);
-    hipLaunchKernelGGL(k_stem_pool_h3, dim3(grid), dim3(512), 0, s, a);
+    if (a.planar) hipLaunchKernelGGL(k_stem_pool_h3<true>, dim3(grid), dim3(512), 0, s, a);
+    else hipLaunchKernelGGL(k_stem_pool_h3<false>, dim3(grid), dim3(512), 0, s, a);
+    return check_launch();
+}
+
+__global__ __launch_bounds__(256) void k_pack_weight_h3p(const float* __restrict__ w, unsigned short* __restrict__ out, float* __restrict__ tail,
+                                                         int Cout, int Npad) {
+    const float wmax = __builtin_bit_cast(float, reinterpret_cast<const unsigned*>(tail)[1]);
+    int ex = 0;
+    if (wmax > 0.f && wmax < 3.0e38f) { (void)frexpf(wmax, &ex); ex = 13 - ex; }
+    ex = max(-100, min(100, ex));
+    const float sc = ldexpf(1.0f, ex);
+    if (blockIdx.x == 0 && threadIdx.x == 0) tail[0] = ldexpf(1.0f, -ex);
+    const int total = Npad * kStemPlanarK;
+    for (int g = blockIdx.x * blockDim.x + threadIdx.x; g < total; g += gridDim.x * blockDim.x) {
+        const int n = g / kStemPlanarK, k = g - n * kStemPlanarK, c = k >> 3, tap = k & 7, kh = c / 3, ch = c - 3 * kh;
+        float v = 0.f;
+        if (n < Cout && c < 21 && tap < 7) v = w[((n * 3 + ch) * 7 + kh) * 7 + tap] * sc;
+        const fp16x2 h = __builtin_amdgcn_cvt_pkrtz(v, 0.f);
+        const float r = v - (float)h[0];
+        const fp16x2 h2 = __builtin_amdgcn_cvt_pkrtz(r, 0.f);
+        out[g] = (unsigned short)(__builtin_bit_cast(unsigned, h) & 0xFFFFu);
+        out[total + g] = (unsigned short)(__builtin_bit_cast(unsigned, h2) & 0xFFFFu);
+    }
+}
+
+int launch_pack_weight_h3p(const float* w, float* packed, int Cout, int Npad, hipStream_t s) {
+    if (!w || !packed || Cout < 1 || Cout > Npad || Npad > 4096 || ((uintptr_t)w & 15)) return FPC_EINVAL;
+    float* tail = packed + (size_t)Npad * kStemPlanarK;
+    if (hipMemsetAsync(tail, 0, 2 * sizeof(float), s) != hipSuccess) return FPC_ELAUNCH;
+    const int rc = launch_absmax_bits(w, (long long)Cout * 3 * 7 * 7, reinterpret_cast<unsigned*>(tail) + 1, s);
+    if (rc) return rc;
+    hipLaunchKernelGGL(k_pack_weight_h3p, dim3((Npad * kStemPlanarK + 255) / 256), dim3(256), 0, s, w,
+                       reinterpret_cast<unsigned short*>(packed), tail, Cout, Npad);
     return check_launch();
 }
 
diff --git a/fastposecnn_amd/engine.py b/fastposecnn_amd/engine.py
--- a/fastposecnn_amd/engine.py
+++ b/fastposecnn_amd/engine.py
@@ -115,6 +115,12 @@
             nat.check(rc, "fpc_net_force_stem_pool")
         return rc
 
+    def stem_reads_planar(self):
+        rc = self._lib.fpc_net_stem_reads_planar(self._h)
+        if rc < 0:
+            nat.check(rc, "fpc_net_stem_reads_planar")
+        return bool(rc)
+
     def survey(self, x, want_logits=True):
         if tuple(x.shape) != (self.B, 3, self.H, self.W) or x.device != self.device:
             raise RuntimeError("NetEngine.survey: input shape / device does not match the plan")
diff --git a/include/fpc.h b/include/fpc.h
--- a/include/fpc.h
+++ b/include/fpc.h
@@ -241,6 +241,7 @@
 int fpc_net_force_fold(fpc_net_t* net, int on);
 int fpc_net_force_direct_h3(fpc_net_t* net, int on);
 int fpc_net_force_stem_pool(fpc_net_t* net, int on);
+int fpc_net_stem_reads_planar(const fpc_net_t* net);
 int fpc_act_range(const float* x, long long n, unsigned* rec4, fpc_stream_t stream);
 int fpc_net_survey_next(fpc_net_t* net, unsigned* records_dev, int sites);
 int fpc_net_guard_ranges(fpc_net_t* net, const unsigned* records_host, int sites, float lo, float hi);
diff --git a/tools_dev/frame_timeline.py b/tools_dev/frame_timeline.py
--- a/tools_dev/frame_timeline.py
+++ b/tools_dev/frame_timeline.py
@@ -2,6 +2,9 @@
 rows = list(csv.DictReader(open(sys.argv[1])))
 rows.sort(key=lambda r: int(r['Start_Timestamp']))
 idx = [i for i, r in enumerate(rows) if 'nchw3_to_nhwc4' in r['Kernel_Name']]
+stem = [i for i, r in enumerate(rows) if 'k_stem_pool_h3' in r['Kernel_Name']]
+if len(stem) >= 3 and (len(idx) < 3 or idx[-1] < stem[-3]):
+    idx = stem
 s, e = idx[-3], idx[-2]
 t0 = int(rows[s]['Start_Timestamp'])
 tot = 0; cat = {}
```

Result: no change. 2847, median of 3 (+0.1%).
